# set-soft/ComfyUI-FLOAT_Optimized

Hardware: AMD Instinct MI355X
Metric: 512x512 frames/sec end-to-end audio->video @50 ODE steps (higher is better)
Workload: dtype fp16; 1 GPU; configs[1]: 10 s audio + 512x512 portrait in HBM -> 250 frames in pinned host memory; appearance encoder + wav2vec2 audio encoder + FMT sampling (50 Euler evaluations/window, CFG a=2.0 e=1.0) + decode + D2H, through InferenceAgent.infer_device (the product call); nfe=51, frames_per_clip=250, fmt_dtype=fp16, dec_dtype=fp16, decode_batch=32, hip_graph=True, parallelism=replicas x1 (one clip per GPU), stage_overlap=off

## Files before the change

comfyui-float_optimized_amd/csrc/fmt_api.hip:

```cpp
#include <math.h>
#include <stdlib.h>

#include "fmt_gemm.hpp"
#include "fmt_kernels.hpp"
#include "fmt_rb_kernels.hpp"
#include "fmt_big_kernels.hpp"
#include "fmt_launch.hpp"

namespace {

struct Blk {
  Lin qkv, proj, fc1, fc2;
};

constexpr int kMaxTok = 80;
constexpr int kMaxSteps = 1024;

}

struct float_fmt {
  float_fmt_cfg_t cfg;
  DevicePool pool;
  int D, ntok, Mpad, Kc, Ntot, Kx;
  int Bmax = 1;
  Lin x_embed, t0, t2, c_embed, adaln_all, final_lin;
  std::vector<Blk> blk;
  float* pos = nullptr;
  float* freqs = nullptr;
  u16 *cond16, *sc16, *h16, *hfin16, *qkv16, *att16, *hid16, *xin16, *tsin16, *th16;
  float *ccond, *xres, *xcur, *temb, *vout;
  unsigned long long* sat = nullptr;
  float* slab = nullptr;
  float *wa_c, *we_c, *prev_x, *prev_wa, *prev_we, *x0_c;
  float* wr_c = nullptr;
  int method = 0;
  FmtTune tune;
  int n_cu = 0;
  float* kbuf = nullptr;
  float* modall = nullptr;
  int Mmod = 0;
  size_t mod_zs = 0;
  struct GraphKey {
    int nfe, bc, we_len, method;
    int prio;
    float a, r, e;
    bool operator==(const GraphKey& o) const { return memcmp(this, &o, sizeof(GraphKey)) == 0; }
  };
  struct GraphEntry {
    GraphKey key;
    hipGraphExec_t exec[kFmtMaxClips + 1];
    uint64_t used;
  };
  std::vector<GraphEntry> graphs;
  uint64_t graph_clock = 0;
  hipStream_t cap_stream = nullptr;
  int cap_prio = 0;
  struct {
    const float *wr, *wa, *we, *noise;
    float* r_d;
    int T, we_len, nfe, include_r, next, n_chunks, B;
    int first = 0, total = 0;
    const float *hist_x = nullptr, *hist_wa = nullptr, *hist_we = nullptr;
    float a, r, e;
    std::vector<float> ts;
    bool active = false;
    bool ragged = false;
    FmtClipTab<const float*> rg_wr, rg_wa, rg_we, rg_noise;
    FmtClipTab<float*> rg_rd;
    int rg_win[kFmtMaxClips];
  } job;
};

namespace {

int dev_copy2d(float* dst, size_t dpitch, const float* src, size_t spitch, int width, int rows, hipStream_t s) {
  if (width <= 0 || rows <= 0) return FLOAT_OK;
  hipLaunchKernelGGL(fmt_copy_kernel, dim3((unsigned)(((size_t)rows * width + 255) / 256)), dim3(256), 0, s, dst, dpitch, src, spitch, width, rows);
  FH_CHECK_HIP(hipGetLastError());
  return FLOAT_OK;
}
int dev_copy(float* dst, const float* src, size_t n, hipStream_t s) { return dev_copy2d(dst, n, src, n, (int)n, 1, s); }
int dev_zero(float* dst, size_t n, hipStream_t s) { return dev_copy2d(dst, n, nullptr, n, (int)n, 1, s); }
int copy_or_zero(float* dst, const float* src, size_t n, hipStream_t s) { return src ? dev_copy(dst, src, n, s) : dev_zero(dst, n, s); }

FmtLaunch launch_ctx(const float_fmt* h, hipStream_t s) {
  return FmtLaunch{h->tune, s, h->sat, h->xres, h->slab, h->h16, h->qkv16, h->att16, h->D, h->ntok, h->Ntot, h->Mpad, h->cfg.heads,
                   h->cfg.attn_window};
}


constexpr int kScSteps = 64;

static int stream_priority(hipStream_t s) {
  int prio = 0;
  if (hipStreamGetPriority(s, &prio) != hipSuccess) {
    (void)hipGetLastError();
    prio = 0;
  }
  return prio;
}

template <class T>
int run_mod_all(float_fmt* h, int M, int e0, int n, hipStream_t s) {
  const int D = h->D;
  const FmtTune& tn = h->tune;
  FH_REQUIRE(n >= 1 && n <= kScSteps, "modulation batch of %d evaluations (max %d)", n, kScSteps);
  const int prio = (s == h->cap_stream && s) ? h->cap_prio : stream_priority(s);
  const bool big = !T::is32 && tn.wide && prio == 0 && big_shape_ok(tn, n * M, h->adaln_all.N, h->adaln_all.K, h->n_cu);
  hipLaunchKernelGGL((fmt_silu_c_kernel<T>), dim3((M * D / 8 + 255) / 256, n), dim3(256), 0, s, h->sc16, h->temb + (size_t)e0 * D,
                     h->ccond, M, D, (size_t)h->Mpad * D, big ? M : 0, h->sat);
  h->mod_zs = big ? (size_t)M * h->Ntot : (size_t)h->Mmod * h->Ntot;
  if constexpr (!T::is32) {
    if (big) return launch_big4<T>(h->sc16, h->adaln_all, h->modall, n * M, h->Ntot, h->n_cu, s);
  }
  GemmArgs g = base_args(h->sc16, h->adaln_all, M);
  g.sat = h->sat, g.out_f32 = h->modall, g.ldo = h->Ntot, g.zcount = n;
  const bool dma = (tn.wide_variant == 6 || tn.wide_variant == 7) && (M + 15) / 16 > 4 && dma_shape_ok(g, 320);
  g.zgroup = tn.zgroup > 0 ? tn.zgroup : (dma ? 2 : 4);
  g.a_zstride = (size_t)h->Mpad * D;
  g.o_zstride = (size_t)h->Mmod * h->Ntot;
  if constexpr (!T::is32) {
    if (tn.wide && g.N % 128 == 0 && g.K % 128 == 0) return launch_wide<T>(g, tn.wide_variant, s);
  }
  for (int z = 0; z < n; ++z) {
    GemmArgs gz = g;
    gz.A = g.A + (size_t)z * g.a_zstride * (sizeof(typename T::elem) / sizeof(u16));
    gz.out_f32 = g.out_f32 + (size_t)z * g.o_zstride;
    gz.zcount = 0;
    int rc = run_gemm<T, EPI_F32>(tn, gz, s);
    if (rc) return rc;
  }
  return FLOAT_OK;
}

bool split_ok(int ks, const Lin& L) { return (ks == 1 || ks == 2 || ks == 4) && L.K % (128 * ks) == 0; }

template <class T>
int run_proj(const FmtLaunch& cx, const Blk& B, int M, const float* gate, const RbPlan& rb, PendingRed* pend) {
  const FmtTune& tn = cx.tn;
  const int ks = rb.shape >= 0 ? rb.ksplit : (split_ok(tn.proj_split, B.proj) ? tn.proj_split : 0);
  int rc;
  launch_attn<T>(cx, M, (!ks && (tn.touch & 2)) ? &B.proj : nullptr);
  GemmArgs g = base_args(cx.att16, B.proj, M);
  if (rb.shape >= 0) {
    to_slab(g, cx.slab, cx.Mpad, ks);
    rc = launch_rbs<T, EPI_PARTIAL>(g, rb.shape, cx.s);
  } else if (ks) {
    rc = run_gemm_partial<T>(cx, g, ks);
  } else {
    g.sat = cx.sat, g.out_f32 = cx.xres, g.ldo = cx.D;
    g.gate = gate, g.ldg = cx.Ntot;
    if (tn.touch & 16) g.touch = make_touch(tn, B.fc1, M, 0, gemm_lanes_per_xcd(tn, M, g.N, g.K), 2);
    rc = run_gemm<T, EPI_GATE_RES>(tn, g, cx.s, false, &tn.plan_layer[RB_PROJ]);
  }
  if (!rc && ks) *pend = pending_red(cx.slab, cx.Mpad, cx.D, B.proj.b, gate, ks);
  return rc;
}

template <class T>
int run_fc2(const FmtLaunch& cx, const Blk& B, const u16* hid16, int M, const float* gate, const RbPlan& rb, const Lin& after,
            int after_nt, PendingRed* pend) {
  const FmtTune& tn = cx.tn;
  const int ks = rb.shape >= 0 ? rb.ksplit : (split_ok(tn.fc2_split, B.fc2) ? tn.fc2_split : 0);
  GemmArgs g = base_args(hid16, B.fc2, M);
  int rc;
  if (rb.shape >= 0) {
    to_slab(g, cx.slab, cx.Mpad, ks);
    rc = launch_rbs<T, EPI_PARTIAL>(g, rb.shape, cx.s);
  } else if (ks) {
    g.sat = cx.sat;
    if (tn.touch & 32) g.touch = make_touch(tn, after, M, 0, gemm_lanes_per_xcd(tn, M, g.N * ks, g.K / ks), 2, after_nt);
    rc = run_gemm_partial<T>(cx, g, ks, &tn.plan_layer[RB_FC2]);
  } else {
    g.sat = cx.sat, g.out_f32 = cx.xres, g.ldo = cx.D;
    g.gate = gate, g.ldg = cx.Ntot;
    rc = run_gemm<T, EPI_GATE_RES>(tn, g, cx.s);
  }
  if (!rc && ks) *pend = pending_red(cx.slab, cx.Mpad, cx.D, B.fc2.b, gate, ks);
  return rc;
}

template <class T>
int run_blocks(float_fmt* h, int nclip, int bc, const float* modbuf, bool euler, float dt, float a, float r, float e, hipStream_t s,
               float* vout_to = nullptr) {
  const float_fmt_cfg_t& c = h->cfg;
  const FmtTune& tn = h->tune;
  const FmtLaunch cx = launch_ctx(h, s);
  const int D = h->D, ntok = h->ntok, M = nclip * bc * ntok;
  int rc;
  {
    GemmArgs g = base_args(h->xin16, h->x_embed, nclip * ntok);
    g.sat = h->sat, g.out_f32 = h->xres, g.ldo = D;
    g.pos = h->pos, g.bc = bc, g.ntok = ntok;
    if ((rc = run_gemm<T, EPI_XEMBED>(tn, g, s))) return rc;
  }
  PendingRed pend;
  RbPlan rb_qkv, rb_proj, rb_fc1, rb_fc2;
  if constexpr (!T::is32) {
    rb_qkv = pick_rb(tn, RB_QKV, M), rb_proj = pick_rb(tn, RB_PROJ, M), rb_fc1 = pick_rb(tn, RB_FC1, M), rb_fc2 = pick_rb(tn, RB_FC2, M);
  }
  for (int b = 0; b < c.depth; ++b) {
    const float* mod = modbuf + (size_t)b * 6 * D;
    const Blk& B = h->blk[b];
    const bool last = b + 1 == c.depth;
    if ((rc = launch_lnmod<T>(cx, M, mod, mod + D, &pend, &B.qkv, nullptr, 0, 128, rb_qkv.shape))) return rc;
    {
      GemmArgs g = base_args(h->h16, B.qkv, M);
      g.sat = h->sat, g.out16 = h->qkv16, g.ldo16 = 3 * D;
      if ((tn.touch & 8) && !split_ok(tn.proj_split, B.proj)) g.touch = make_touch(tn, B.proj, M, 0, gemm_lanes_per_xcd(tn, M, g.N, g.K), 2);
      if (rb_qkv.shape >= 0) rc = launch_rbs<T, EPI_T16>(g, rb_qkv.shape, s);
      else rc = run_gemm<T, EPI_T16>(tn, g, s, false, &tn.plan_layer[RB_QKV]);
      if (rc) return rc;
    }
    if ((rc = run_proj<T>(cx, B, M, mod + 2 * D, rb_proj, &pend))) return rc;
    if ((rc = launch_lnmod<T>(cx, M, mod + 3 * D, mod + 4 * D, &pend, &B.fc1, nullptr, 0, 64, rb_fc1.shape))) return rc;
    {
      GemmArgs g = base_args(h->h16, B.fc1, M);
      g.sat = h->sat, g.out16 = h->hid16, g.ldo16 = B.fc2.K / 32;
      if ((tn.touch & 4) && rb_fc2.shape < 0)
        g.touch = make_touch(tn, B.fc2, M, split_ok(tn.fc2_split, B.fc2) ? tn.fc2_split : 0, gemm_lanes_per_xcd(tn, M, g.N, g.K), 2);
      if (rb_fc1.shape >= 0) rc = launch_rbs<T, EPI_GELU_P16>(g, rb_fc1.shape, s);
      else rc = run_gemm<T, EPI_GELU_P16>(tn, g, s, false, &tn.plan_layer[RB_FC1]);
      if (rc) return rc;
    }
    if ((rc = run_fc2<T>(cx, B, h->hid16, M, mod + 5 * D, rb_fc2, last ? h->final_lin : h->blk[b + 1].qkv, last ? 1 : 0, &pend))) return rc;
  }
  {
    const float* mod = modbuf + (size_t)c.depth * 6 * D;
    const bool tokblk = (!tn.no_tokblk || nclip > 1) && (bc == 1 || bc == 3 || bc == 4) && h->final_lin.K % 256 == 0;
    FH_REQUIRE(tokblk || nclip == 1, "batched sampling needs the token-blocked head GEMM");
    const int nblk = (ntok + 15) / 16, seqs = nclip * bc;
    if ((rc = launch_lnmod<T>(cx, M, mod, mod + D, &pend, nullptr, tokblk ? h->hfin16 : nullptr, tokblk ? seqs * 16 : 0))) return rc;
    GemmArgs g = base_args(tokblk ? h->hfin16 : h->h16, h->final_lin, tokblk ? nblk * seqs * 16 : M);
    g.sat = h->sat, g.tokblk = tokblk ? 1 : 0;
    g.nclip = nclip, g.bc = bc, g.ntok = ntok, g.n_prev = c.n_prev;
    g.a_cfg = a, g.r_cfg = r, g.e_cfg = e, g.dt = dt;
    if (euler) g.xcur = h->xcur, g.xin16 = h->xin16, g.ldx = h->Kx / 32;
    else g.vout = vout_to ? vout_to : h->vout;
    if (tokblk) rc = launch_gemm<T, EPI_CFG>(g, bc, 1, 8, s);
    else rc = run_gemm<T, EPI_CFG>(tn, g, s, true);
    if (rc) return rc;
  }
  FH_CHECK_HIP(hipGetLastError());
  return FLOAT_OK;
}

void linspace01(int n, std::vector<float>* ts) {
  ts->resize(n);
  if (n == 1) {
    (*ts)[0] = 0.f;
    return;
  }
  const float step = 1.0f / (float)(n - 1);
  const int half = n / 2;
  for (int i = 0; i < n; ++i) (*ts)[i] = (i < half) ? (0.f + step * (float)i) : (1.0f - step * (float)(n - 1 - i));
}

struct TimeSpec {
  float t;
  int nfe, stages;
  float c[4];
};
template <class T>
int prepare_time(float_fmt* h, const TimeSpec& ts, int n, hipStream_t s) {
  int rc;
  hipLaunchKernelGGL((fmt_tsin_kernel<T>), dim3(n), dim3(256), 0, s, h->tsin16, h->freqs, n, ts.t, ts.nfe, ts.stages, ts.c[0],
                     ts.c[1], ts.c[2], ts.c[3]);
  GemmArgs g = base_args(h->tsin16, h->t0, n);
  g.sat = h->sat, g.out16 = h->th16, g.ldo16 = h->t2.K / 32;
  if ((rc = launch_gemm<T, EPI_SILU_P16>(g, 4, 1, T::is32 ? 4 : pick_nw(g.K, 0), s))) return rc;
  GemmArgs g2 = base_args(h->th16, h->t2, n);
  g2.sat = h->sat, g2.out_f32 = h->temb, g2.ldo = h->D;
  if ((rc = launch_gemm<T, EPI_F32>(g2, 4, 1, T::is32 ? 4 : pick_nw(g2.K, 0), s))) return rc;
  return FLOAT_OK;
}

struct CfgMode {
  int bc;
  unsigned wr_mask, wa_mask, we_mask;
  int nclip = 1;
};

CfgMode cfg_mode(float a, float r, float e, int include_r) {
  if (a == 1.0f && r == 1.0f && e == 1.0f) return {1, 1u, 1u, 1u, 1};
  if (!include_r) return {3, 0b111u, 0b110u, 0b010u, 1};
  return {4, 0b1110u, 0b1100u, 0b0100u, 1};
}

template <class T>
int stage_window(float_fmt* h, const CfgMode& m, const float* x0, const float* wa, const float* wr, const float* we,
                 int we_len, const float* prev_x, const float* prev_wa, const float* prev_we, hipStream_t s) {
  const float_fmt_cfg_t& c = h->cfg;
  const int M = m.nclip * m.bc * h->ntok;
  hipLaunchKernelGGL((fmt_build_cond_kernel<T>), dim3(M), dim3(256), 0, s, h->cond16, h->Kc, m.bc, h->ntok, c.n_prev,
                     c.dim_w, c.dim_a, c.dim_e, wr, wa, prev_wa, we, we_len, prev_we, m.wr_mask, m.wa_mask, m.we_mask, h->sat);
  GemmArgs g = base_args(h->cond16, h->c_embed, M);
  g.sat = h->sat, g.out_f32 = h->ccond, g.ldo = h->D;
  int rc;
  if ((rc = run_gemm<T, EPI_F32>(h->tune, g, s))) return rc;
  const int n = m.nclip * h->ntok * c.dim_w;
  hipLaunchKernelGGL((fmt_init_x_kernel<T>), dim3((n + 255) / 256), dim3(256), 0, s, h->xcur, h->xin16, h->Kx / 32, x0, prev_x,
                     c.n_prev, c.n_cur, c.dim_w, m.nclip, h->sat);
  FH_CHECK_HIP(hipGetLastError());
  return FLOAT_OK;
}

int check_cfg_rows(const float_fmt* h, const CfgMode& m) {
  FH_REQUIRE(!h->tune.no_tokblk || m.bc * h->ntok <= 240,
             "%d-way CFG of %d tokens is %d rows; the all-rows CFG epilogue GEMM holds at most 240 (15 row tiles)", m.bc, h->ntok,
             m.bc * h->ntok);
  return FLOAT_OK;
}

int check_common(float_fmt* h, const void* we, int we_len, const void* prev_we) {
  FH_REQUIRE(h != nullptr, "null FMT handle");
  FH_REQUIRE(we_len == 1 || we_len == h->cfg.n_cur,
             "Dynamic emotion latent `we` time dimension (%d) does not match audio latent `wa` time dimension (%d).",
             we_len, h->cfg.n_cur);
  FH_REQUIRE(!(we_len > 1 && prev_we == nullptr),
             "`we` is dynamic (T>1), but prev_we was not provided with prev_x/prev_wa.");
  (void)we;
  return FLOAT_OK;
}

struct Tableau {
  int s;
  float c[4], a[4][3], b[4];
};
const Tableau& tableau(int method) {
  static const Tableau T[5] = {
      {1, {0.f}, {{0.f}}, {1.f}},
      {2, {0.f, 0.5f}, {{0.f}, {0.5f}}, {0.f, 1.f}},
      {4, {0.f, 1.f / 3, 2.f / 3, 1.f}, {{0.f}, {1.f / 3}, {-1.f / 3, 1.f}, {1.f, -1.f, 1.f}}, {0.125f, 0.375f, 0.375f, 0.125f}},
      {2, {0.f, 1.f}, {{0.f}, {1.f}}, {0.5f, 0.5f}},
      {3, {0.f, 1.f / 3, 2.f / 3}, {{0.f}, {1.f / 3}, {0.f, 2.f / 3}}, {0.25f, 0.f, 0.75f}},
  };
  return T[method];
}

TimeSpec time_spec(int method, int nfe) {
  const Tableau& tb = tableau(method);
  TimeSpec ts{};
  ts.nfe = nfe;
  ts.stages = tb.s;
  for (int j = 0; j < 4; ++j) ts.c[j] = tb.c[j];
  return ts;
}
int n_evals(int method, int nfe) { return (nfe - 1) * tableau(method).s; }

template <class T>
int run_window_steps(float_fmt* h, const CfgMode& m, int nfe, const std::vector<float>& ts, float a, float r, float e,
                     hipStream_t s) {
  const Tableau& tb = tableau(h->method);
  const float_fmt_cfg_t& c = h->cfg;
  const size_t kstride = (size_t)h->Bmax * kMaxTok * c.dim_w;
  const int n = m.nclip * c.n_cur * c.dim_w, rows = m.nclip * m.bc * h->ntok;
  const int nev = n_evals(h->method, nfe), batch = h->tune.hoist ? kScSteps : 1;
  const bool euler = h->method == FLOAT_ODE_EULER;
  int rc;
  for (int ev = 0; ev < nev; ++ev) {
    const int i = ev / tb.s, j = ev - i * tb.s, z = ev % batch;
    const float dt = ts[i + 1] - ts[i];
    if (z == 0 && (rc = run_mod_all<T>(h, rows, ev, std::min(batch, nev - ev), s))) return rc;
    const float* mod = h->modall + (size_t)z * h->mod_zs;
    if (euler) {
      if ((rc = run_blocks<T>(h, m.nclip, m.bc, mod, true, dt, a, r, e, s))) return rc;
      continue;
    }
    if (j > 0) {
      hipLaunchKernelGGL((fmt_rk_combine_kernel<T>), dim3((n + 255) / 256), dim3(256), 0, s, h->xcur, h->kbuf, kstride, j,
                         dt * tb.a[j][0], dt * tb.a[j][1], dt * tb.a[j][2], 0.f, 0, h->xin16, h->Kx / 32, c.n_prev, c.n_cur,
                         c.dim_w, m.nclip, h->sat);
    }
    if ((rc = run_blocks<T>(h, m.nclip, m.bc, mod, false, 0.f, a, r, e, s, h->kbuf + (size_t)j * kstride))) return rc;
    if (j == tb.s - 1) {
      hipLaunchKernelGGL((fmt_rk_combine_kernel<T>), dim3((n + 255) / 256), dim3(256), 0, s, h->xcur, h->kbuf, kstride, tb.s,
                         dt * tb.b[0], dt * tb.b[1], dt * tb.b[2], dt * tb.b[3], 1, h->xin16, h->Kx / 32, c.n_prev, c.n_cur,
                         c.dim_w, m.nclip, h->sat);
    }
  }
  FH_CHECK_HIP(hipGetLastError());
  return FLOAT_OK;
}

constexpr size_t kMaxGraphs = 8;
void destroy_graphs(float_fmt::GraphEntry& g) {
  for (hipGraphExec_t& e : g.exec)
    if (e) {
      (void)hipGraphExecDestroy(e);
      e = nullptr;
    }
}
template <class T>
int run_window_steps_graph(float_fmt* h, const CfgMode& m, int we_len, int nfe, const std::vector<float>& ts, float a,
                           float r, float e, hipStream_t s) {
  float_fmt::GraphKey key;
  memset(&key, 0, sizeof(key));
  key.nfe = nfe;
  key.method = h->method;
  key.bc = m.bc;
  key.we_len = we_len;
  key.a = a;
  key.r = r;
  key.e = e;
  key.prio = stream_priority(s);
  FH_REQUIRE(m.nclip >= 1 && m.nclip <= kFmtMaxClips, "chain of %d clips (max %d)", m.nclip, kFmtMaxClips);
  float_fmt::GraphEntry* hit = nullptr;
  for (auto& g : h->graphs)
    if (g.key == key) hit = &g;
  if (!hit || !hit->exec[m.nclip]) {
    if (!h->cap_stream) FH_CHECK_HIP(hipStreamCreateWithFlags(&h->cap_stream, hipStreamNonBlocking));
    hipGraph_t graph = nullptr;
    h->cap_prio = key.prio;
    FH_CHECK_HIP(hipStreamBeginCapture(h->cap_stream, hipStreamCaptureModeThreadLocal));
    int rc = run_window_steps<T>(h, m, nfe, ts, a, r, e, h->cap_stream);
    hipError_t ce = hipStreamEndCapture(h->cap_stream, &graph);
    if (rc) {
      if (graph) (void)hipGraphDestroy(graph);
      return rc;
    }
    FH_CHECK_HIP(ce);
    hipGraphExec_t exec = nullptr;
    FH_CHECK_HIP(hipGraphInstantiate(&exec, graph, nullptr, nullptr, 0));
    (void)hipGraphDestroy(graph);
    if (!hit) {
      if (h->graphs.size() >= kMaxGraphs) {
        size_t lru = 0;
        for (size_t i = 1; i < h->graphs.size(); ++i)
          if (h->graphs[i].used < h->graphs[lru].used) lru = i;
        hipError_t se = hipDeviceSynchronize();
        if (se != hipSuccess) {
          (void)hipGraphExecDestroy(exec);
          FH_CHECK_HIP(se);
        }
        destroy_graphs(h->graphs[lru]);
        h->graphs.erase(h->graphs.begin() + lru);
      }
      float_fmt::GraphEntry fresh;
      memset(&fresh, 0, sizeof(fresh));
      fresh.key = key;
      h->graphs.push_back(fresh);
      hit = &h->graphs.back();
    }
    hit->exec[m.nclip] = exec;
  }
  hit->used = ++h->graph_clock;
  FH_CHECK_HIP(hipGraphLaunch(hit->exec[m.nclip], s));
  return FLOAT_OK;
}

template <class T>
int window_impl(float_fmt* h, const float* x0, const float* wa, const float* wr, const float* we, int we_len,
                const float* prev_x, const float* prev_wa, const float* prev_we, int nfe, const std::vector<float>& ts,
                float a, float r, float e, int include_r, hipStream_t s, int nclip = 1) {
  CfgMode m = cfg_mode(a, r, e, include_r);
  m.nclip = nclip;
  int rc = check_cfg_rows(h, m);
  if (rc) return rc;
  if ((rc = stage_window<T>(h, m, x0, wa, wr, we, we_len, prev_x, prev_wa, prev_we, s))) return rc;
  if (nfe <= 1) return FLOAT_OK;
  hipStreamCaptureStatus cs = hipStreamCaptureStatusNone;
  if (hipStreamIsCapturing(s, &cs) != hipSuccess) {
    (void)hipGetLastError();
    cs = hipStreamCaptureStatusNone;
  }
  if (h->cfg.use_graph && !g_fh_profiling && cs == hipStreamCaptureStatusNone)
    return run_window_steps_graph<T>(h, m, we_len, nfe, ts, a, r, e, s);
  return run_window_steps<T>(h, m, nfe, ts, a, r, e, s);
}

template <class T>
int eval_impl(float_fmt* h, float t, const float* x, const float* wa, const float* wr, const float* we, int we_len,
              const float* prev_x, const float* prev_wa, const float* prev_we, float a, float r, float e, int include_r,
              float* out, hipStream_t s) {
  TimeSpec tsp{};
  tsp.t = t;
  int rc = prepare_time<T>(h, tsp, 1, s);
  if (rc) return rc;
  const CfgMode m = cfg_mode(a, r, e, include_r);
  if ((rc = check_cfg_rows(h, m))) return rc;
  if ((rc = stage_window<T>(h, m, x, wa, wr, we, we_len, prev_x, prev_wa, prev_we, s))) return rc;
  if ((rc = run_mod_all<T>(h, m.bc * h->ntok, 0, 1, s))) return rc;
  if ((rc = run_blocks<T>(h, 1, m.bc, h->modall, false, 0.f, a, r, e, s))) return rc;
  return dev_copy(out, h->vout, (size_t)h->ntok * h->cfg.dim_w, s);
}

template <class T>
int sample_window(float_fmt* h, int k, hipStream_t s) {
  const float_fmt_cfg_t& c = h->cfg;
  auto& J = h->job;
  const int L = c.n_cur, P = c.n_prev, Tn = J.T, B = J.B;
  const bool dynamic = J.we_len > 1;
  int rc;
  auto blocks = [](int n) { return dim3((n + 255) / 256); };
  if (k == J.first) {
    if ((rc = prepare_time<T>(h, time_spec(h->method, J.nfe), std::max(1, n_evals(h->method, J.nfe)), s))) return rc;
    if ((rc = copy_or_zero(h->prev_x, J.hist_x, (size_t)B * P * c.dim_w, s))) return rc;
    if ((rc = copy_or_zero(h->prev_wa, J.hist_wa, (size_t)B * P * c.dim_a, s))) return rc;
    if ((rc = copy_or_zero(h->prev_we, J.hist_we, (size_t)B * P * c.dim_e, s))) return rc;
  } else if (P > 0) {
    hipLaunchKernelGGL(fmt_tail_kernel, blocks(B * P * c.dim_w), dim3(256), 0, s, h->prev_x, h->xcur, P, L, c.dim_w, B);
    hipLaunchKernelGGL(fmt_tail_kernel, blocks(B * P * c.dim_a), dim3(256), 0, s, h->prev_wa, h->wa_c, P, L, c.dim_a, B);
    if (dynamic) hipLaunchKernelGGL(fmt_tail_kernel, blocks(B * P * c.dim_e), dim3(256), 0, s, h->prev_we, h->we_c, P, L, c.dim_e, B);
  }
  hipLaunchKernelGGL(fmt_slice_pad_kernel, blocks(B * L * c.dim_a), dim3(256), 0, s, h->wa_c, J.wa, k * L, Tn, L, c.dim_a, B);
  if (dynamic) hipLaunchKernelGGL(fmt_slice_pad_kernel, blocks(B * L * c.dim_e), dim3(256), 0, s, h->we_c, J.we, k * L, Tn, L, c.dim_e, B);
  if ((rc = dev_copy(h->x0_c, J.noise + (size_t)k * B * L * c.dim_w, (size_t)B * L * c.dim_w, s))) return rc;
  rc = window_impl<T>(h, h->x0_c, h->wa_c, J.wr, dynamic ? h->we_c : J.we, dynamic ? L : 1, h->prev_x, h->prev_wa,
                      dynamic ? h->prev_we : nullptr, J.nfe, J.ts, J.a, J.r, J.e, J.include_r, s, B);
  if (rc) return rc;
  const int rows = (k == J.total - 1) ? (Tn - k * L) : L;
  return dev_copy2d(J.r_d + (size_t)k * L * c.dim_w, (size_t)Tn * c.dim_w, h->xcur, (size_t)L * c.dim_w, rows * c.dim_w, B, s);
}

template <class T>
int sample_window_ragged(float_fmt* h, int k, hipStream_t s) {
  const float_fmt_cfg_t& c = h->cfg;
  auto& J = h->job;
  const int L = c.n_cur, P = c.n_prev;
  const bool dynamic = J.we_len > 1;
  int nact = 0;
  while (nact < J.B && J.rg_win[nact] > k) ++nact;
  int rc;
  auto blocks = [](int n) { return dim3((n + 255) / 256); };
  auto grid = [nact](int n) { return dim3((n + 255) / 256, nact); };
  if (k == 0) {
    if ((rc = prepare_time<T>(h, time_spec(h->method, J.nfe), std::max(1, n_evals(h->method, J.nfe)), s))) return rc;
    if ((rc = dev_zero(h->prev_x, (size_t)nact * P * c.dim_w, s))) return rc;
    if ((rc = dev_zero(h->prev_wa, (size_t)nact * P * c.dim_a, s))) return rc;
    if ((rc = dev_zero(h->prev_we, (size_t)nact * P * c.dim_e, s))) return rc;
    hipLaunchKernelGGL(fmt_gather_pad_kernel, grid(c.dim_w), dim3(256), 0, s, h->wr_c, J.rg_wr, 0, 1, c.dim_w);
    if (!dynamic) hipLaunchKernelGGL(fmt_gather_pad_kernel, grid(c.dim_e), dim3(256), 0, s, h->we_c, J.rg_we, 0, 1, c.dim_e);
  } else if (P > 0) {
    hipLaunchKernelGGL(fmt_tail_kernel, blocks(nact * P * c.dim_w), dim3(256), 0, s, h->prev_x, h->xcur, P, L, c.dim_w, nact);
    hipLaunchKernelGGL(fmt_tail_kernel, blocks(nact * P * c.dim_a), dim3(256), 0, s, h->prev_wa, h->wa_c, P, L, c.dim_a, nact);
    if (dynamic) hipLaunchKernelGGL(fmt_tail_kernel, blocks(nact * P * c.dim_e), dim3(256), 0, s, h->prev_we, h->we_c, P, L, c.dim_e, nact);
  }
  hipLaunchKernelGGL(fmt_gather_pad_kernel, grid(L * c.dim_a), dim3(256), 0, s, h->wa_c, J.rg_wa, k * L, L, c.dim_a);
  if (dynamic) hipLaunchKernelGGL(fmt_gather_pad_kernel, grid(L * c.dim_e), dim3(256), 0, s, h->we_c, J.rg_we, k * L, L, c.dim_e);
  hipLaunchKernelGGL(fmt_gather_pad_kernel, grid(L * c.dim_w), dim3(256), 0, s, h->x0_c, J.rg_noise, k * L, L, c.dim_w);
  FH_CHECK_HIP(hipGetLastError());
  rc = window_impl<T>(h, h->x0_c, h->wa_c, h->wr_c, h->we_c, dynamic ? L : 1, h->prev_x, h->prev_wa,
                      dynamic ? h->prev_we : nullptr, J.nfe, J.ts, J.a, J.r, J.e, J.include_r, s, nact);
  if (rc) return rc;
  hipLaunchKernelGGL(fmt_scatter_trim_kernel, grid(L * c.dim_w), dim3(256), 0, s, J.rg_rd, h->xcur, k * L, L, c.dim_w);
  FH_CHECK_HIP(hipGetLastError());
  return FLOAT_OK;
}

template <class T>
int create_impl(float_fmt* h, const TensorTable& tt) {
  const float_fmt_cfg_t& c = h->cfg;
  const int D = c.dim_h;
  int rc;
  prime_kernels<T>();
  auto pack = [&](const std::vector<std::string>& names, int N_each, int K, Lin* out) {
    return pack_linear_pool<T>(h->tune, &h->pool, tt, names, N_each, K, out);
  };
  if ((rc = pack({"x_embedder.proj"}, D, c.dim_w, &h->x_embed))) return rc;
  if ((rc = pack({"t_embedder.mlp.0"}, D, 256, &h->t0))) return rc;
  if ((rc = pack({"t_embedder.mlp.2"}, D, D, &h->t2))) return rc;
  if ((rc = pack({"c_embedder"}, D, c.dim_w + c.dim_a + c.dim_e, &h->c_embed))) return rc;
  h->blk.resize(c.depth);
  std::vector<std::string> ada;
  for (int b = 0; b < c.depth; ++b) {
    const std::string p = "blocks." + std::to_string(b) + ".";
    if ((rc = pack({p + "attn.qkv"}, 3 * D, D, &h->blk[b].qkv))) return rc;
    if ((rc = pack({p + "attn.proj"}, D, D, &h->blk[b].proj))) return rc;
    if ((rc = pack({p + "mlp.fc1"}, c.mlp_hidden, D, &h->blk[b].fc1))) return rc;
    if ((rc = pack({p + "mlp.fc2"}, D, c.mlp_hidden, &h->blk[b].fc2))) return rc;
    ada.push_back(p + "adaLN_modulation.1");
  }
  if ((rc = pack(ada, 6 * D, D, &h->adaln_all))) return rc;
  Lin tail;
  if ((rc = pack(std::vector<std::string>{"decoder.adaLN_modulation.1"}, 2 * D, D, &tail))) return rc;
  if ((rc = concat_linear_rows<T>(&h->pool, h->adaln_all, tail, &h->adaln_all))) return rc;
  if ((rc = pack({"decoder.linear"}, c.dim_w, D, &h->final_lin))) return rc;
  return FLOAT_OK;
}

}


int fmt_pack_linear(const FmtTune& tn, DevicePool* pool, int dtype, const TensorTable& tt, const std::vector<std::string>& names,
                    int N_each, int K, FmtLin* out) {
  FH_REQUIRE(dtype == FLOAT_DT_BF16 || dtype == FLOAT_DT_FP16 || dtype == FLOAT_DT_FP32, "the GEMM service: unknown dtype %d", dtype);
  return fmt_by_dtype(dtype, [&](auto t) { return pack_linear_pool<decltype(t)>(tn, pool, tt, names, N_each, K, out); });
}

int fmt_pack_linear_raw(const FmtTune& tn, DevicePool* pool, int dtype, const float* w, const float* b, int N, int K, FmtLin* out) {
  std::vector<float> zeros;
  if (!b) {
    zeros.assign(N, 0.f);
    b = zeros.data();
  }
  float_tensor_t t[2];
  memset(t, 0, sizeof(t));
  t[0].name = "raw.weight";
  t[0].data = w;
  t[0].ndim = 2;
  t[0].shape[0] = N;
  t[0].shape[1] = K;
  t[1].name = "raw.bias";
  t[1].data = b;
  t[1].ndim = 1;
  t[1].shape[0] = N;
  TensorTable tt(t, 2);
  return fmt_pack_linear(tn, pool, dtype, tt, {"raw"}, N, K, out);
}

GemmArgs fmt_gemm_args(const u16* A, const FmtLin& L, int M) { return base_args(A, L, M); }

void fmt_gemm_prime(int dtype) {
  fmt_by_dtype(dtype, [](auto t) { prime_kernels<decltype(t)>(); });
}

template <class T>
static int gemm_run_t(const FmtTune& tn, int epi, const GemmArgs& g, hipStream_t s) {
  switch (epi) {
    case EPI_F32: return run_gemm<T, EPI_F32>(tn, g, s);
    case EPI_T16: return run_gemm<T, EPI_T16>(tn, g, s);
    case EPI_SILU_P16: return run_gemm<T, EPI_SILU_P16>(tn, g, s);
    case EPI_GELU_P16: return run_gemm<T, EPI_GELU_P16>(tn, g, s);
    case EPI_GELUERF_P16: return run_gemm<T, EPI_GELUERF_P16>(tn, g, s);
    default: fh_set_error("fmt_gemm_run: epilogue %d is not exported", epi); return FLOAT_E_INVALID;
  }
}

int fmt_gemm_run(const FmtTune& tn, int dtype, int epi, GemmArgs g, hipStream_t s) {
  return fmt_by_dtype(dtype, [&](auto t) { return gemm_run_t<decltype(t)>(tn, epi, g, s); });
}

template <class T>
static int debug_impl(float_fmt* h, int what, const float* in, float* out, hipStream_t s) {
  const int D = h->D, ntok = h->ntok;
  if (what == 0) {
    return dev_copy(out, h->pos, (size_t)ntok * D, s);
  }
  if (what == 3 || what == 4) {
    FH_REQUIRE(in != nullptr, "float_fmt_debug: request %d needs an input", what);
    constexpr int Mt = 48, Kt = 1024;
    const int Nt = what == 3 ? 64 : 16;
    std::vector<float> host((size_t)(Mt + Nt) * Kt);
    FH_CHECK_HIP(hipStreamSynchronize(s));
    FH_CHECK_HIP(hipMemcpy(host.data(), in, host.size() * sizeof(float), hipMemcpyDeviceToHost));
    struct Scratch : DevicePool {
      ~Scratch() { release(); }
    } pool;
    Lin a, w;
    int rc;
    if ((rc = fmt_pack_linear_raw(h->tune, &pool, h->cfg.dtype, host.data(), nullptr, Mt, Kt, &a))) return rc;
    if ((rc = fmt_pack_linear_raw(h->tune, &pool, h->cfg.dtype, host.data() + (size_t)Mt * Kt, nullptr, Nt, Kt, &w))) return rc;
    GemmArgs g = base_args(a.W, w, Mt);
    g.out_f32 = out, g.ldo = Nt;
    if (what == 3) {
      if ((rc = launch_gemm<T, EPI_F32>(g, 3, 4, T::is32 ? 4 : 8, s))) return rc;
    } else {
      float* ones = nullptr;
      if ((rc = pool.alloc(&ones, (size_t)Mt * Nt, false))) return rc;
      const std::vector<float> one((size_t)Mt * Nt, 1.f);
      FH_CHECK_HIP(hipMemcpy(ones, one.data(), one.size() * sizeof(float), hipMemcpyHostToDevice));
      FH_CHECK_HIP(hipMemsetAsync(out, 0, (size_t)Mt * Nt * sizeof(float), s));
      g.gate = ones, g.ldg = Nt;
      if ((rc = launch_gemm<T, EPI_GATE_RES>(g, 3, 1, T::is32 ? 4 : 8, s))) return rc;
    }
    FH_CHECK_HIP(hipStreamSynchronize(s));
    return FLOAT_OK;
  }
  if (what == 5) {
    FH_REQUIRE(in != nullptr, "float_fmt_debug: request %d needs an input", what);
    hipLaunchKernelGGL(fmt_xlane_probe_kernel, dim3(kXlaneProbeVecs), dim3(64), 0, s, in, out);
    FH_CHECK_HIP(hipGetLastError());
    return FLOAT_OK;
  }
  FH_REQUIRE(what == 1 && in != nullptr, "float_fmt_debug: unknown request %d (or null input)", what);
  const int n = ntok * 3 * D;
  hipLaunchKernelGGL((fmt_dbg_to16_kernel<T>), dim3((n + 255) / 256), dim3(256), 0, s, h->qkv16, in, n);
  launch_attn<T>(launch_ctx(h, s), ntok, nullptr);
  hipLaunchKernelGGL((fmt_dbg_unpack_kernel<T>), dim3((ntok * D + 255) / 256), dim3(256), 0, s, out, h->att16, ntok, D);
  FH_CHECK_HIP(hipGetLastError());
  return FLOAT_OK;
}

static int drain_job(float_fmt_t* h, void* stream) {
  int32_t left = 1;
  while (left > 0)
    if (int rc = float_fmt_sample_next(h, stream, nullptr, &left)) return rc;
  return FLOAT_OK;
}

extern "C" {

int float_fmt_create(const float_fmt_cfg_t* cfg, const float_tensor_t* tensors, int32_t n_tensors, float_fmt_t** out) {
  FH_REQUIRE(cfg && tensors && out, "null argument to float_fmt_create");
  FH_REQUIRE(cfg->dim_h % 256 == 0 && cfg->dim_h / 256 <= 8 && ((cfg->dim_h / 256) & (cfg->dim_h / 256 - 1)) == 0,
             "dim_h=%d unsupported", cfg->dim_h);
  FH_REQUIRE(cfg->dim_h / cfg->heads == 128, "head_dim must be 128 (dim_h=%d heads=%d)", cfg->dim_h, cfg->heads);
  FH_REQUIRE(cfg->dim_w % 128 == 0 && cfg->mlp_hidden % 128 == 0, "dim_w / mlp_hidden must be multiples of 128");
  FH_REQUIRE(cfg->n_prev + cfg->n_cur <= kMaxTok, "at most %d tokens per window (got %d)", kMaxTok, cfg->n_prev + cfg->n_cur);
  FH_REQUIRE(cfg->n_prev >= 0 && cfg->n_prev <= cfg->n_cur, "n_prev must be in [0, n_cur]");
  FH_REQUIRE(cfg->dtype == FLOAT_DT_BF16 || cfg->dtype == FLOAT_DT_FP16 || cfg->dtype == FLOAT_DT_FP32, "unknown dtype %d", cfg->dtype);
  FH_REQUIRE(cfg->max_batch >= 0 && cfg->max_batch <= 16, "max_batch must be in [0, 16] (got %d)", cfg->max_batch);
  float_fmt* h = new float_fmt();
  h->tune = FmtTune::from_env();
  h->cfg = *cfg;
  h->D = cfg->dim_h;
  h->ntok = cfg->n_prev + cfg->n_cur;
  h->Bmax = cfg->max_batch > 0 ? cfg->max_batch : 1;
  h->Mpad = 16 * ((h->Bmax * 4 * h->ntok + 15) / 16 + 12);
  h->Kc = round_up(cfg->dim_w + cfg->dim_a + cfg->dim_e, 128);
  h->Kx = round_up(cfg->dim_w, 128);
  {
    int dev = 0, ncu = 0;
    if (hipGetDevice(&dev) == hipSuccess && hipDeviceGetAttribute(&ncu, hipDeviceAttributeMultiprocessorCount, dev) == hipSuccess) h->n_cu = ncu;
    else (void)hipGetLastError();
  }
  h->Ntot = cfg->depth * 6 * h->D + 2 * h->D;
  TensorTable tt(tensors, n_tensors);
  int rc = fmt_by_dtype(cfg->dtype, [&](auto t) { return create_impl<decltype(t)>(h, tt); });
  const int D = h->D, Mp = h->Mpad;
  const size_t esz = cfg->dtype == FLOAT_DT_FP32 ? 2 : 1;
  auto A = [&](auto** p, size_t n) {
    if (!rc) rc = h->pool.alloc(p, std::is_same<std::remove_reference_t<decltype(**p)>, u16>::value ? n * esz : n, true);
  };
  A(&h->pos, (size_t)kMaxTok * D);
  A(&h->freqs, 128);
  A(&h->cond16, (size_t)Mp * h->Kc);
  A(&h->sc16, (size_t)kScSteps * Mp * D + (size_t)12 * 16 * D);
  A(&h->h16, (size_t)Mp * D);
  A(&h->hfin16, (size_t)h->Bmax * 64 * ((kMaxTok + 15) / 16) * D);
  A(&h->qkv16, (size_t)Mp * 3 * D);
  A(&h->att16, (size_t)Mp * D);
  A(&h->hid16, (size_t)Mp * cfg->mlp_hidden);
  A(&h->xin16, (size_t)(h->Bmax * kMaxTok + 6 * 16) * h->Kx);
  A(&h->tsin16, (size_t)kMaxSteps * 256);
  A(&h->th16, (size_t)kMaxSteps * D);
  A(&h->ccond, (size_t)Mp * D);
  h->Mmod = 16 * ((h->Bmax * 4 * h->ntok + 15) / 16);
  if (!rc) rc = h->pool.alloc(&h->modall, (size_t)kScSteps * h->Mmod * h->Ntot, false);
  A(&h->kbuf, (size_t)4 * h->Bmax * kMaxTok * cfg->dim_w);
  A(&h->xres, (size_t)Mp * D);
  A(&h->slab, (size_t)8 * Mp * D);
  A(&h->sat, 1);
  A(&h->xcur, (size_t)h->Bmax * cfg->n_cur * cfg->dim_w);
  A(&h->temb, (size_t)kMaxSteps * D);
  A(&h->vout, (size_t)h->Bmax * kMaxTok * cfg->dim_w);
  A(&h->wa_c, (size_t)h->Bmax * cfg->n_cur * cfg->dim_a);
  A(&h->we_c, (size_t)h->Bmax * cfg->n_cur * cfg->dim_e);
  A(&h->x0_c, (size_t)h->Bmax * cfg->n_cur * cfg->dim_w);
  A(&h->wr_c, (size_t)h->Bmax * cfg->dim_w);
  A(&h->prev_x, (size_t)h->Bmax * cfg->n_cur * cfg->dim_w);
  A(&h->prev_wa, (size_t)h->Bmax * cfg->n_cur * cfg->dim_a);
  A(&h->prev_we, (size_t)h->Bmax * cfg->n_cur * cfg->dim_e);
  if (!rc) {
    std::vector<float> pos((size_t)h->ntok * D);
    const float_tensor_t* pe = tt.find("pos_embed");
    if (pe && TensorTable::numel(pe) == (int64_t)h->ntok * D) {
      memcpy(pos.data(), pe->data, pos.size() * sizeof(float));
    } else {
      for (int p = 0; p < h->ntok; ++p)
        for (int j = 0; j < D; ++j) {
          const float ang = (float)((double)p / pow(10000.0, 2.0 * (double)(j / 2) / (double)D));
          pos[(size_t)p * D + j] = (j & 1) ? cosf(ang) : sinf(ang);
        }
    }
    std::vector<float> fr(128);
    for (int k = 0; k < 128; ++k) fr[k] = expf(-logf(10000.0f) * (float)k / 128.0f);
    if (hipMemcpy(h->pos, pos.data(), pos.size() * sizeof(float), hipMemcpyHostToDevice) != hipSuccess ||
        hipMemcpy(h->freqs, fr.data(), fr.size() * sizeof(float), hipMemcpyHostToDevice) != hipSuccess) {
      fh_set_error("hipMemcpy of FMT tables failed");
      rc = FLOAT_E_HIP;
    }
  }
  if (rc) {
    float_fmt_destroy(h);
    return rc;
  }
  *out = h;
  return FLOAT_OK;
}

void float_fmt_destroy(float_fmt_t* h) {
  if (!h) return;
  for (auto& g : h->graphs) destroy_graphs(g);
  if (h->cap_stream) (void)hipStreamDestroy(h->cap_stream);
  h->pool.release();
  delete h;
}

int float_fmt_eval(float_fmt_t* h, float t, const float* x, const float* wa, const float* wr, const float* we,
                   int32_t we_len, const float* prev_x, const float* prev_wa, const float* prev_we, float a_cfg,
                   float r_cfg, float e_cfg, int32_t include_r_cfg, float* out, void* stream) {
  int rc = check_common(h, we, we_len, prev_we);
  if (rc) return rc;
  FH_REQUIRE(x && wa && wr && we && prev_x && prev_wa && out, "null tensor argument to float_fmt_eval");
  hipStream_t s = (hipStream_t)stream;
  return fmt_by_dtype(h->cfg.dtype, [&](auto tag) {
    return eval_impl<decltype(tag)>(h, t, x, wa, wr, we, we_len, prev_x, prev_wa, prev_we, a_cfg, r_cfg, e_cfg, include_r_cfg, out, s);
  });
}

int float_fmt_sample_chunk(float_fmt_t* h, const float* x0, const float* wa, const float* wr, const float* we,
                           int32_t we_len, const float* prev_x, const float* prev_wa, const float* prev_we, int32_t nfe,
                           float a_cfg, float r_cfg, float e_cfg, int32_t include_r_cfg, float* out, void* stream) {
  int rc = check_common(h, we, we_len, prev_we);
  if (rc) return rc;
  FH_REQUIRE(x0 && wa && wr && we && prev_x && prev_wa && out, "null tensor argument to float_fmt_sample_chunk");
  FH_REQUIRE(nfe >= 1 && n_evals(h->method, nfe) < kMaxSteps, "nfe=%d: too many evaluations (max %d)", nfe, kMaxSteps);
  hipStream_t s = (hipStream_t)stream;
  std::vector<float> ts;
  linspace01(nfe, &ts);
  const float_fmt_cfg_t& c = h->cfg;
  if ((rc = dev_copy(h->x0_c, x0, (size_t)c.n_cur * c.dim_w, s))) return rc;
  if ((rc = dev_copy(h->wa_c, wa, (size_t)c.n_cur * c.dim_a, s))) return rc;
  if ((rc = dev_copy(h->prev_x, prev_x, (size_t)c.n_prev * c.dim_w, s))) return rc;
  if ((rc = dev_copy(h->prev_wa, prev_wa, (size_t)c.n_prev * c.dim_a, s))) return rc;
  if (we_len > 1) {
    if ((rc = dev_copy(h->we_c, we, (size_t)c.n_cur * c.dim_e, s))) return rc;
    if ((rc = dev_copy(h->prev_we, prev_we, (size_t)c.n_prev * c.dim_e, s))) return rc;
  }
  const float* we_p = we_len > 1 ? h->we_c : we;
  const float* pwe_p = we_len > 1 ? h->prev_we : nullptr;
  const TimeSpec tsp = time_spec(h->method, nfe);
  const int nev = std::max(1, n_evals(h->method, nfe));
  rc = fmt_by_dtype(c.dtype, [&](auto t) {
    typedef decltype(t) T;
    if (int prc = prepare_time<T>(h, tsp, nev, s)) return prc;
    return window_impl<T>(h, h->x0_c, h->wa_c, wr, we_p, we_len, h->prev_x, h->prev_wa, pwe_p, nfe, ts, a_cfg, r_cfg, e_cfg,
                          include_r_cfg, s);
  });
  if (rc) return rc;
  return dev_copy(out, h->xcur, (size_t)c.n_cur * c.dim_w, s);
}

int float_fmt_debug(float_fmt_t* h, int32_t what, const float* in, float* out, void* stream) {
  FH_REQUIRE(h != nullptr && out != nullptr, "null argument to float_fmt_debug");
  return fmt_by_dtype(h->cfg.dtype, [&](auto t) { return debug_impl<decltype(t)>(h, what, in, out, (hipStream_t)stream); });
}

int float_fmt_saturation(float_fmt_t* h, uint64_t* total, int32_t reset, void* stream) {
  FH_REQUIRE(h && total, "null argument to float_fmt_saturation");
  FH_CHECK_HIP(hipStreamSynchronize((hipStream_t)stream));
  unsigned long long v = 0;
  FH_CHECK_HIP(hipMemcpy(&v, h->sat, sizeof(v), hipMemcpyDeviceToHost));
  *total = v;
  if (reset) {
    FH_CHECK_HIP(hipMemsetAsync(h->sat, 0, sizeof(v), (hipStream_t)stream));
    FH_CHECK_HIP(hipStreamSynchronize((hipStream_t)stream));
  }
  return FLOAT_OK;
}

int float_fmt_set_method(float_fmt_t* h, int32_t method) {
  FH_REQUIRE(h != nullptr, "null FMT handle");
  FH_REQUIRE(method >= FLOAT_ODE_EULER && method <= FLOAT_ODE_HEUN3, "unknown ODE method %d", method);
  h->method = method;
  return FLOAT_OK;
}

int float_fmt_sample_begin(float_fmt_t* h, const float* wr, const float* wa, int32_t T, const float* we, int32_t we_len,
                           const float* noise, int32_t nfe, float a_cfg, float r_cfg, float e_cfg, int32_t include_r_cfg,
                           float* r_d) {
  FH_REQUIRE(h != nullptr, "null FMT handle");
  FH_REQUIRE(wr && wa && we && noise && r_d, "null tensor argument to float_fmt_sample");
  FH_REQUIRE(T >= 1, "T must be >= 1 (got %d)", T);
  FH_REQUIRE(we_len == 1 || we_len == T,
             "Dynamic emotion latent `we` time dimension (%d) does not match audio latent `wa` time dimension (%d).",
             we_len, T);
  FH_REQUIRE(nfe >= 1 && n_evals(h->method, nfe) < kMaxSteps, "nfe=%d: too many evaluations (max %d)", nfe, kMaxSteps);
  auto& J = h->job;
  J.wr = wr;
  J.wa = wa;
  J.we = we;
  J.noise = noise;
  J.r_d = r_d;
  J.T = T;
  J.we_len = we_len;
  J.nfe = nfe;
  J.include_r = include_r_cfg;
  J.a = a_cfg;
  J.r = r_cfg;
  J.e = e_cfg;
  J.B = 1;
  J.ragged = false;
  J.next = 0;
  J.n_chunks = (T + h->cfg.n_cur - 1) / h->cfg.n_cur;
  J.first = 0;
  J.total = J.n_chunks;
  J.hist_x = J.hist_wa = J.hist_we = nullptr;
  linspace01(nfe, &J.ts);
  J.active = true;
  return FLOAT_OK;
}

int float_fmt_sample_begin_range(float_fmt_t* h, const float* wr, const float* wa, int32_t T, const float* we, int32_t we_len,
                                 const float* noise, int32_t nfe, float a_cfg, float r_cfg, float e_cfg, int32_t include_r_cfg,
                                 float* r_d, int32_t first_window, int32_t end_window, const float* hist_x, const float* hist_wa,
                                 const float* hist_we) {
  int rc = float_fmt_sample_begin(h, wr, wa, T, we, we_len, noise, nfe, a_cfg, r_cfg, e_cfg, include_r_cfg, r_d);
  if (rc) return rc;
  auto& J = h->job;
  J.active = false;
  FH_REQUIRE(first_window >= 0 && first_window < end_window && end_window <= J.total,
             "window range [%d, %d) outside the clip's %d windows", first_window, end_window, J.total);
  FH_REQUIRE(we_len == 1 || hist_we != nullptr || hist_x == nullptr,
             "a dynamic-emotion job that starts from a history needs hist_we too");
  J.first = J.next = first_window;
  J.n_chunks = end_window;
  J.hist_x = hist_x;
  J.hist_wa = hist_wa;
  J.hist_we = we_len > 1 ? hist_we : nullptr;
  J.active = true;
  return FLOAT_OK;
}

int float_fmt_sample_next(float_fmt_t* h, void* stream, int32_t* window_done, int32_t* windows_left) {
  FH_REQUIRE(h != nullptr && h->job.active, "float_fmt_sample_next without float_fmt_sample_begin");
  auto& J = h->job;
  hipStream_t s = (hipStream_t)stream;
  const int k = J.next;
  int rc = fmt_by_dtype(h->cfg.dtype, [&](auto t) {
    return J.ragged ? sample_window_ragged<decltype(t)>(h, k, s) : sample_window<decltype(t)>(h, k, s);
  });
  if (rc) {
    J.active = false;
    return rc;
  }
  J.next = k + 1;
  if (window_done) *window_done = k;
  if (windows_left) *windows_left = J.n_chunks - J.next;
  if (J.next >= J.n_chunks) J.active = false;
  return FLOAT_OK;
}

int float_fmt_sample_batch(float_fmt_t* h, int32_t n_clips, const float* wr, const float* wa, int32_t T, const float* we,
                           int32_t we_len, const float* noise, int32_t nfe, float a_cfg, float r_cfg, float e_cfg,
                           int32_t include_r_cfg, float* r_d, void* stream) {
  FH_REQUIRE(h != nullptr, "null FMT handle");
  FH_REQUIRE(n_clips >= 1 && n_clips <= h->Bmax, "batch of %d clips, the handle was created with max_batch = %d", n_clips, h->Bmax);
  int rc = float_fmt_sample_begin(h, wr, wa, T, we, we_len, noise, nfe, a_cfg, r_cfg, e_cfg, include_r_cfg, r_d);
  if (rc) return rc;
  h->job.B = n_clips;
  return drain_job(h, stream);
}

int float_fmt_sample_begin_ragged(float_fmt_t* h, int32_t n_clips, const int32_t* T, const float* const* wr,
                                  const float* const* wa, const float* const* we, int32_t we_dynamic,
                                  const float* const* noise, int32_t nfe, float a_cfg, float r_cfg, float e_cfg,
                                  int32_t include_r_cfg, float* const* r_d) {
  FH_REQUIRE(h != nullptr, "null FMT handle");
  FH_REQUIRE(T && wr && wa && we && noise && r_d, "null array argument to float_fmt_sample_begin_ragged");
  FH_REQUIRE(n_clips >= 1 && n_clips <= h->Bmax, "batch of %d clips, the handle was created with max_batch = %d", n_clips, h->Bmax);
  for (int i = 0; i < n_clips; ++i) {
    FH_REQUIRE(wr[i] && wa[i] && we[i] && noise[i] && r_d[i], "null tensor argument to float_fmt_sample_begin_ragged (clip %d)", i);
    FH_REQUIRE(T[i] >= 1, "T must be >= 1 (got %d for clip %d)", T[i], i);
  }
  FH_REQUIRE(nfe >= 1 && n_evals(h->method, nfe) < kMaxSteps, "nfe=%d: too many evaluations (max %d)", nfe, kMaxSteps);
  auto& J = h->job;
  J.active = false;
  const int L = h->cfg.n_cur;
  int order[kFmtMaxClips];
  for (int i = 0; i < n_clips; ++i) order[i] = i;
  std::stable_sort(order, order + n_clips, [&](int x, int y) { return (T[x] + L - 1) / L > (T[y] + L - 1) / L; });
  memset(&J.rg_wr, 0, sizeof(J.rg_wr));
  memset(&J.rg_wa, 0, sizeof(J.rg_wa));
  memset(&J.rg_we, 0, sizeof(J.rg_we));
  memset(&J.rg_noise, 0, sizeof(J.rg_noise));
  memset(&J.rg_rd, 0, sizeof(J.rg_rd));
  for (int q = 0; q < n_clips; ++q) {
    const int i = order[q], Ti = T[i], win = (Ti + L - 1) / L;
    J.rg_win[q] = win;
    J.rg_wr.p[q] = wr[i], J.rg_wr.T[q] = 1;
    J.rg_wa.p[q] = wa[i], J.rg_wa.T[q] = Ti;
    J.rg_we.p[q] = we[i], J.rg_we.T[q] = we_dynamic ? Ti : 1;
// ... 41 lines not shown
```

comfyui-float_optimized_amd/csrc/fmt_decode.hpp:

```cpp
#pragma once

#if defined(__HIPCC__)
#define FMT_HD __host__ __device__ __forceinline__
#else
#define FMT_HD inline
#endif

struct FmtDiv {
  unsigned mul, sh;
};
inline FmtDiv fmt_make_div(unsigned d) {
  unsigned l = 0;
  while ((1u << l) < d) ++l;
  FmtDiv v;
  v.sh = 28u + l;
  v.mul = (unsigned)((1ull << v.sh) / d + 1ull);
  return v;
}
FMT_HD unsigned fmt_div(unsigned n, unsigned mul, unsigned sh) { return (unsigned)(((unsigned long long)n * mul) >> sh); }
FMT_HD unsigned fmt_div(unsigned n, const FmtDiv& d) { return fmt_div(n, d.mul, d.sh); }
constexpr unsigned kFmtDivMax = 1u << 28;

struct GemmDecode {
  unsigned mblk_mul;
  unsigned nbx, nbx_mul;
  unsigned nbn, nbn_mul;
  unsigned bits;
};
enum { kDecAffine = 1u << 20, kDecKsXcd = 1u << 21 };

inline GemmDecode fmt_make_decode(int nbn, int mblk, int ksplit, bool partial) {
  GemmDecode d;
  const unsigned nbx = (unsigned)(partial ? nbn * ksplit : nbn);
  const FmtDiv dm = fmt_make_div((unsigned)mblk), dx = fmt_make_div(nbx), dn = fmt_make_div((unsigned)nbn);
  d.mblk_mul = dm.mul, d.nbx = nbx, d.nbx_mul = dx.mul, d.nbn = (unsigned)nbn, d.nbn_mul = dn.mul;
  d.bits = dm.sh | (dx.sh << 6) | (dn.sh << 12);
  if ((nbx & 7u) == 0u) {
    d.bits |= kDecAffine;
    if (partial && (8 % ksplit) == 0) {
      unsigned p = 0;
      while ((8u >> p) != (unsigned)ksplit) ++p;
      d.bits |= kDecKsXcd | (p << 18);
    }
  }
  return d;
}

struct GemmBlock {
  int bx, by, ks;
};
FMT_HD GemmBlock fmt_block_decode(const GemmDecode& d, unsigned mblk, unsigned id, bool partial) {
  unsigned bx, by, ks = 0u;
  if (d.bits & kDecAffine) {
    const unsigned slot = id >> 3, q = fmt_div(slot, d.mblk_mul, d.bits & 63u);
    by = slot - q * mblk;
    bx = q * 8u + (id & 7u);
  } else {
    by = fmt_div(id, d.nbx_mul, (d.bits >> 6) & 63u);
    bx = id - by * d.nbx;
  }
  if (partial) {
    if (d.bits & kDecKsXcd) {
      const unsigned p = (d.bits >> 18) & 3u, x = bx & 7u;
      ks = x >> p;
      bx = ((bx >> 3) << p) + (x & ((1u << p) - 1u));
    } else {
      ks = fmt_div(bx, d.nbn_mul, (d.bits >> 12) & 63u);
      bx -= ks * d.nbn;
    }
  }
  return GemmBlock{(int)bx, (int)by, (int)ks};
}
```

comfyui-float_optimized_amd/csrc/fmt_kernels.hpp:

```cpp
#pragma once
#include "common.hpp"
#include "fmt_pack.hpp"

template <class T, int MTW, int NT>
constexpr int fmt_gemm_pf() {
  return T::is32 ? 1 : ((MTW + NT <= 7) ? 4 : ((MTW + NT <= 8) ? 3 : 2));
}
template <class T, int MTW, int NT, int NW, int EPI>
constexpr bool fmt_gemm_has_flat() {
  if (T::is32) return false;
  if (EPI == EPI_XEMBED) return MTW == 4 && NT == 1 && NW == 4;
  return NW == 8 && MTW == 3 && (NT == 4 || EPI == EPI_GATE_RES || EPI == EPI_CFG);
}

template <class T, int MTW, int NT, int NW, int EPI, bool FLAT = false>
__device__ __forceinline__ void fmt_gemm_body(const GemmArgs& g) {
  const unsigned bid = blockIdx.x, nblk = gridDim.x;
  constexpr int BN = NT * 16;
  constexpr int ROWS = MTW * 16;
  constexpr bool WT = NW >= 8;
  constexpr int NTHR = NW * 64;
  constexpr int PF = fmt_gemm_pf<T, MTW, NT>();
  typedef typename T::elem E;
  typedef typename T::pack8 P8;
  extern __shared__ __attribute__((aligned(16))) float red[];
  const int lane = threadIdx.x & 63;
  const int w = threadIdx.x >> 6;
  const int r16 = lane & 15, q = lane >> 4;
  const GemmBlock blk = fmt_block_decode(g.dec, (unsigned)g.mblk, bid, EPI == EPI_PARTIAL);
  const int bx = blk.bx, by = blk.by, ks = blk.ks;
  const int nb0 = bx * NT;
  const int mt0 = by * MTW;
  const int n0 = nb0 * 16, m0 = mt0 * 16;

  f32x4 acc[MTW][NT];
#pragma unroll
  for (int i = 0; i < MTW; ++i)
#pragma unroll
    for (int j = 0; j < NT; ++j) acc[i][j] = f32x4{0.f, 0.f, 0.f, 0.f};

  const int KB = g.K >> 5;
  const int KBs = (EPI == EPI_PARTIAL) ? g.kbs : KB;
  const int KBw = FLAT ? PF : (int)((unsigned)KBs / NW);
  const E* Ap = reinterpret_cast<const E*>(g.A) + ((size_t)mt0 * KB + ks * KBs + w * KBw) * 512 + lane * 8;
  const E* Wp = reinterpret_cast<const E*>(g.W) + ((size_t)nb0 * KB + ks * KBs + w * KBw) * 512 + lane * 8;
  const size_t tstride = (size_t)KB * 512;

  P8 a[PF][MTW], b[PF][NT];
#pragma unroll
  for (int p = 0; p < PF; ++p) {
    if (FLAT || p < KBw) {
#pragma unroll
      for (int j = 0; j < NT; ++j) b[p][j] = T::load8_nt(Wp + j * tstride + (size_t)p * 512);
#pragma unroll
      for (int i = 0; i < MTW; ++i) a[p][i] = T::load8(Ap + i * tstride + (size_t)p * 512);
    }
  }
  constexpr bool kEarlyRes = (EPI == EPI_GATE_RES) && (MTW * 16 * (NT * 2) <= NW * 64);
  float4 res_pf[2], gate_pf[2];
  if constexpr (kEarlyRes) {
    const int r = threadIdx.x / (NT * 2), cg = threadIdx.x % (NT * 2);
    int row = m0 + r;
    const int nb = n0 + cg * 8;
    if constexpr (FLAT) row = min(m0 + min(r, ROWS - 1), g.M - 1);
    if (FLAT || (r < ROWS && row < g.M)) {
      const float* o = g.out_f32 + (size_t)row * g.ldo + nb;
      const float* gt = g.gate + (size_t)row * g.ldg + nb;
      res_pf[0] = fh_load_f4(o);
      res_pf[1] = fh_load_f4(o + 4);
      gate_pf[0] = fh_load_f4_stream(gt);
      gate_pf[1] = fh_load_f4_stream(gt + 4);
    }
  }
  constexpr bool kTouch = (EPI == EPI_GELU_P16 || EPI == EPI_T16 || EPI == EPI_GATE_RES || EPI == EPI_PARTIAL);
  unsigned touched[2] = {0u, 0u};
  if constexpr (kTouch && FLAT) {
    __builtin_amdgcn_sched_barrier(0);
    fmt_touch_always(g.touch, Wp, bid & 7, (bid >> 3) * NTHR + threadIdx.x, (nblk >> 3) * NTHR, touched);
  } else if constexpr (kTouch) {
    if (g.touch.W) fmt_touch(g.touch, bid & 7, (bid >> 3) * NTHR + threadIdx.x, (nblk >> 3) * NTHR, touched);
  }
  if constexpr (FLAT) {
#pragma unroll
    for (int p = 0; p < PF; ++p) {
      __builtin_amdgcn_sched_barrier(0);
#pragma unroll
      for (int i = 0; i < MTW; ++i)
#pragma unroll
        for (int j = 0; j < NT; ++j) acc[i][j] = T::mfma(a[p][i], b[p][j], acc[i][j]);
    }
    __builtin_amdgcn_sched_barrier(0);
  } else
  for (int kb0 = 0; kb0 < KBw; kb0 += PF) {
#pragma unroll
    for (int p = 0; p < PF; ++p) {
      const int kb = kb0 + p;
      if (kb < KBw) {
#pragma unroll
        for (int i = 0; i < MTW; ++i)
#pragma unroll
          for (int j = 0; j < NT; ++j) acc[i][j] = T::mfma(a[p][i], b[p][j], acc[i][j]);
        if (kb + PF < KBw) {
#pragma unroll
          for (int j = 0; j < NT; ++j)
            b[p][j] = T::load8_nt(Wp + j * tstride + (size_t)(kb + PF) * 512);
#pragma unroll
          for (int i = 0; i < MTW; ++i) a[p][i] = T::load8(Ap + i * tstride + (size_t)(kb + PF) * 512);
        }
      }
    }
  }

  if constexpr (kTouch && !FLAT) {
    if (g.touch.W) fmt_touch_retire(touched);
  }
  float* my = red + w * (ROWS * BN);
#pragma unroll
  for (int i = 0; i < MTW; ++i)
#pragma unroll
    for (int j = 0; j < NT; ++j)
#pragma unroll
      for (int r = 0; r < 4; ++r) my[(i * 16 + q * 4 + r) * BN + j * 16 + r16] = acc[i][j][r];
  __syncthreads();

  constexpr int S = ROWS * BN;
  constexpr int CG = BN / 8;
  unsigned rm = 0u;
  auto slab_sum = [&](int o) {
    float a = red[o];
#pragma unroll
    for (int ww = 1; ww < NW; ++ww) a += red[ww * S + o];
    return a;
  };
  if constexpr (EPI == EPI_CFG) {
    const int nclip = g.nclip > 1 ? g.nclip : 1;
    const int tb = g.tokblk ? by / nclip : 0, q = g.tokblk ? by - tb * nclip : 0;
    const int ni = g.tokblk ? 16 : g.ntok, i0 = tb * 16, rstride = g.tokblk ? 16 : g.ntok;
    float* const vout_q = g.vout ? g.vout + (size_t)q * g.ntok * g.N : nullptr;
    float* const xcur_q = g.xcur ? g.xcur + (size_t)q * (g.ntok - g.n_prev) * g.N : nullptr;
    for (int idx = threadIdx.x; idx < ni * BN; idx += NTHR) {
      const int il = idx / BN, i = i0 + il, c = idx % BN, n = n0 + c;
      if (i >= g.ntok) break;
      const float bias = g.bias[n];
      float v[4];
#pragma unroll
      for (int b2 = 0; b2 < 4; ++b2) {
        if (b2 < g.bc) {
          const int o = (b2 * rstride + il) * BN + c;
          v[b2] = slab_sum(o) + bias;
        } else {
          v[b2] = 0.f;
        }
      }
      float out;
      if (g.bc == 1) {
        out = v[0];
      } else if (g.bc == 3) {
        out = v[0] + g.a_cfg * (v[2] - v[0]) + g.e_cfg * (v[1] - v[2]);
      } else {
        out = v[0] + g.r_cfg * (v[1] - v[0]) + g.a_cfg * (v[3] - v[1]) + g.e_cfg * (v[2] - v[3]);
      }
      if (vout_q) vout_q[(size_t)i * g.N + n] = out;
      if (xcur_q && i >= g.n_prev) {
        const size_t xo = (size_t)(i - g.n_prev) * g.N + n;
        const float xn = xcur_q[xo] + g.dt * out;
        xcur_q[xo] = xn;
        reinterpret_cast<E*>(g.xin16)[fmt_pack_off(q * g.ntok + i, n, g.ldx)] = fh_cvt<T>(xn, rm);
      }
    }
  } else {
    for (int idx = threadIdx.x; idx < ROWS * CG; idx += NTHR) {
      const int r = idx / CG, cg = idx % CG;
      const int row = m0 + r, nb = n0 + cg * 8;
      if (row >= g.M) continue;
      float v[8];
      {
        const float* p0 = red + r * BN + cg * 8;
#pragma unroll
        for (int e = 0; e < 8; e += 4) {
          float4 a4 = *reinterpret_cast<const float4*>(p0 + e);
#pragma unroll
          for (int ww = 1; ww < NW; ++ww) {
            const float4 t4 = *reinterpret_cast<const float4*>(p0 + ww * S + e);
            a4.x += t4.x;
            a4.y += t4.y;
            a4.z += t4.z;
            a4.w += t4.w;
          }
          float4 bb = float4{0.f, 0.f, 0.f, 0.f};
          if constexpr (EPI != EPI_PARTIAL) bb = *reinterpret_cast<const float4*>(g.bias + nb + e);
          v[e + 0] = a4.x + bb.x;
          v[e + 1] = a4.y + bb.y;
          v[e + 2] = a4.z + bb.z;
          v[e + 3] = a4.w + bb.w;
        }
      }
      if constexpr (EPI == EPI_F32 || EPI == EPI_PARTIAL) {
        float* o = g.out_f32 + (size_t)ks * g.slab_stride + (size_t)row * g.ldo + nb;
        fh_store_f4_wt<4, WT>(o, float4{v[0], v[1], v[2], v[3]});
        fh_store_f4_wt<4, WT>(o + 4, float4{v[4], v[5], v[6], v[7]});
      } else if constexpr (EPI == EPI_T16 || EPI == EPI_SILU_P16 || EPI == EPI_GELU_P16 || EPI == EPI_GELUERF_P16) {
        P8 u;
#pragma unroll
        for (int i = 0; i < 8; ++i) {
          float x = v[i];
          if constexpr (EPI == EPI_SILU_P16) x = fh_silu(x);
          if constexpr (EPI == EPI_GELU_P16) x = fh_gelu_tanh(x);
          if constexpr (EPI == EPI_GELUERF_P16) x = fh_gelu_erf(x);
          T::set(u, i, x);
        }
        fh_track_pack<T>(rm, u);
        E* const o16 = reinterpret_cast<E*>(g.out16);
        if constexpr (EPI == EPI_T16) T::template store8_wt<8, WT>(o16 + (size_t)row * g.ldo16 + nb, u);
        else T::template store8_wt<8, WT>(o16 + fmt_pack_off(row, nb, g.ldo16), u);
      } else if constexpr (EPI == EPI_GATE_RES) {
        float* o = g.out_f32 + (size_t)row * g.ldo + nb;
        const float* gt = g.gate + (size_t)row * g.ldg + nb;
#pragma unroll
        for (int e = 0; e < 8; e += 4) {
          float4 x, gg;
          if constexpr (kEarlyRes) {
            x = res_pf[e / 4];
            gg = gate_pf[e / 4];
          } else {
            x = fh_load_f4(o + e);
            gg = fh_load_f4_stream(gt + e);
          }
          x.x += gg.x * v[e + 0];
          x.y += gg.y * v[e + 1];
          x.z += gg.z * v[e + 2];
          x.w += gg.w * v[e + 3];
          fh_store_f4_wt<16, WT>(o + e, x);
        }
      } else if constexpr (EPI == EPI_XEMBED) {
        const int q = row / g.ntok, tok = row - q * g.ntok;
        const float* ps = g.pos + (size_t)tok * g.N + nb;
#pragma unroll
        for (int i = 0; i < 8; ++i) v[i] += ps[i];
        for (int b2 = 0; b2 < g.bc; ++b2) {
          float* o = g.out_f32 + (size_t)((q * g.bc + b2) * g.ntok + tok) * g.ldo + nb;
          fh_store_f4_wt<32, WT>(o, float4{v[0], v[1], v[2], v[3]});
          fh_store_f4_wt<32, WT>(o + 4, float4{v[4], v[5], v[6], v[7]});
        }
      }
    }
  }
  if constexpr (EPI == EPI_CFG || EPI == EPI_T16 || EPI == EPI_SILU_P16 || EPI == EPI_GELU_P16 || EPI == EPI_GELUERF_P16) fh_range_flush<T>(g.sat, rm);
  if constexpr (kTouch && FLAT) fmt_touch_retire_last(touched);
}

template <class T, int MTW, int NT, int NW, int EPI>
__global__ __launch_bounds__(NW * 64) void fmt_gemm_kernel(const u16* A, const u16* W, int K, int kbs, int ksplit, int mblk,
                                                           unsigned mblk_mul, unsigned nbx, unsigned nbx_mul, unsigned nbn,
                                                           unsigned nbn_mul, unsigned bits, GemmTail t) {
  GemmArgs g;
  static_cast<GemmHead&>(g) = GemmHead{A, W, K, kbs, ksplit, mblk, GemmDecode{mblk_mul, nbx, nbx_mul, nbn, nbn_mul, bits}};
  static_cast<GemmTail&>(g) = t;
  if constexpr (fmt_gemm_has_flat<T, MTW, NT, NW, EPI>()) {
    if ((EPI == EPI_PARTIAL ? kbs : (K >> 5)) == NW * fmt_gemm_pf<T, MTW, NT>()) {
      fmt_gemm_body<T, MTW, NT, NW, EPI, true>(g);
      return;
    }
  }
  fmt_gemm_body<T, MTW, NT, NW, EPI>(g);
}
template <class K>
void fmt_gemm_launch(int prof, K kern, dim3 grid, dim3 block, size_t smem, hipStream_t s, const GemmArgs& g) {
  const GemmTail& t = g;
  fh_launch_prof(prof, kern, grid, block, smem, s, g.A, g.W, g.K, g.kbs, g.ksplit, g.mblk, g.dec.mblk_mul, g.dec.nbx, g.dec.nbx_mul,
                 g.dec.nbn, g.dec.nbn_mul, g.dec.bits, t);
}

template <class T, int MTW, int KCH , int NWV = 4>
__global__ __launch_bounds__(NWV * 64) void fmt_gemm_wide_kernel(GemmArgs g) {
  constexpr int EPI = EPI_F32;
  constexpr int NF = MTW * KCH;
  constexpr int NFW = (NF + NWV - 1) / NWV;
  constexpr int WR = NWV / 4, MTR = MTW / WR;
  static_assert(MTW % WR == 0, "row tiles must split evenly over the wave rows");
  extern __shared__ __attribute__((aligned(16))) unsigned char sA[];
  const int lane = threadIdx.x & 63, w = threadIdx.x >> 6, wc = w & 3, wr = w >> 2;
  const int r16 = lane & 15, q = lane >> 4;
  const int nbn = g.N >> 7;
  const int nbx = (EPI == EPI_PARTIAL) ? nbn * g.ksplit : nbn;
  int bx, by, bz = 0, ks = 0;
  {
    const int id = blockIdx.x;
    const int nz = g.zcount > 1 ? g.zcount : 1;
    if (nz > 1 && (nbx & 7) == 0 && g.zgroup > 1) {
      const int slot = id >> 3, G = g.zgroup, ncx = nbx >> 3, rows = g.mblk * nz;
      const int full = ncx / G, per_grp = G * rows;
      int grp = slot / per_grp, rem = slot - grp * per_grp, gw = G;
      if (grp >= full) {
        grp = full;
        rem = slot - full * per_grp;
        gw = ncx - full * G;
      }
      const int zy = rem / gw;
      bz = zy / g.mblk;
      by = zy - bz * g.mblk;
// ... 245 lines not shown
      _Pragma("unroll") for (int j = 0; j < 5; ++j) acc[i][j] = T::mfma(BC[j], AC[i], acc[i][j]); \
    __builtin_amdgcn_sched_barrier(0);                                                         \
  } while (0)

  const bool g1 = wr == 1;
#ifdef DMA_CLK
  const unsigned long long c0 = clock64(), w0 = wall_clock64();
#endif
#pragma unroll
  for (int s = 0; s < NS; ++s) issue(s);
  if constexpr (STG) DMA_WAIT(NS - 2);
  else DMA_WAIT(NS - 1);
  __builtin_amdgcn_s_barrier();
  DMA_READ(0, a0, b0);
  asm volatile("s_waitcnt lgkmcnt(0)" ::: "memory");
  __builtin_amdgcn_sched_barrier(0);
  if constexpr (STG) {
    if (g1) __builtin_amdgcn_s_barrier();
    for (int s = 0; s < KB; s += 2) {
      DMA_STEP_STG(s, a0, b0, a1, b1);
      DMA_STEP_STG(s + 1, a1, b1, a0, b0);
    }
    if (!g1) __builtin_amdgcn_s_barrier();
  } else {
    for (int s = 0; s < KB; s += 2) {
      DMA_STEP(s, a0, b0, a1, b1);
      DMA_STEP(s + 1, a1, b1, a0, b0);
    }
  }
#ifdef DMA_CLK
  if ((blockIdx.x == 3000 || blockIdx.x == 6001) && threadIdx.x == 0) {
    const unsigned long long c1 = clock64(), w1 = wall_clock64();
    printf("tile loop: %llu core clocks, %llu wall ticks\n", c1 - c0, w1 - w0);
  }
#endif
#undef DMA_STEP_STG
#undef DMA_WAIT_UPTO
#undef DMA_STEP
#undef DMA_READ
#undef DMA_WAIT
  float* const outz = g.out_f32 + (size_t)bz * g.o_zstride;
  constexpr int OW = CT * 16, OSTR = OW + 4, C4 = OW / 4, NTHR = NW * 64;
  static_assert(96 * OSTR * 4 <= NS * STAGE, "output staging does not fit the ring");
  float* const so = reinterpret_cast<float*>(ring);
  float4 bb[5];
#pragma unroll
  for (int j = 0; j < 5; ++j) bb[j] = *reinterpret_cast<const float4*>(g.bias + (bx * CT + wc * 5 + j) * 16 + q * 4);
#pragma unroll
  for (int p = 0; p < 2; ++p) {
    if (wr == p) {
#pragma unroll
      for (int i = 0; i < 6; ++i)
#pragma unroll
        for (int j = 0; j < 5; ++j)
          *reinterpret_cast<float4*>(so + (i * 16 + r16) * OSTR + (wc * 5 + j) * 16 + q * 4) =
              float4{acc[i][j][0] + bb[j].x, acc[i][j][1] + bb[j].y, acc[i][j][2] + bb[j].z, acc[i][j][3] + bb[j].w};
    }
    __syncthreads();
    {
#pragma unroll
      for (int k = 0; k < (96 * C4) / NTHR; ++k) {
        const int idx = k * NTHR + threadIdx.x, rl = idx / C4, c4 = idx - rl * C4;
        const int row = by * (RT * 16) + p * 96 + rl;
        if (row < g.M)
          *reinterpret_cast<float4*>(outz + (size_t)row * g.ldo + bx * OW + c4 * 4) = *reinterpret_cast<const float4*>(so + rl * OSTR + c4 * 4);
      }
    }
    if (p == 0) __syncthreads();
  }
}

struct LnRed {
  const float* slab;
  size_t slab_stride;
  const float* bias;
  const float* gate;
};

constexpr int kLnTouch = 6;

template <class T, int NV, int KS, bool TOUCH, bool WT>
__device__ __forceinline__ void fmt_lnmod_body(float* __restrict__ x, int M, const float* __restrict__ shift,
                                               const float* __restrict__ scale, int ldm, u16* __restrict__ out, const LnRed& red,
                                               const TouchSpec& pf, int ntok, int perm, unsigned long long* sat, const int wpb) {
  constexpr int D = NV * 256;
  const unsigned bid = blockIdx.x, nblk = gridDim.x;
  const int lane = threadIdx.x & 63;
  int row = bid * wpb + (threadIdx.x >> 6);
  unsigned touched[kLnTouch] = {};
  const bool touch = TOUCH && wpb == 1;
  auto touch_lines = [&]() { fmt_touch(pf, bid & 7, (bid >> 3) * 64 + lane, (nblk >> 3) * 64, touched); };
  if (wpb == 1) {
    const int x = bid & 7, j = bid >> 3;
    row = (((j >> 3) * 8 + x) << 3) + (j & 7);
  }
  if (row >= M) {
    if (touch) {
      touch_lines();
      fmt_touch_retire(touched);
    }
    return;
  }
  float* xr = x + (size_t)row * D;
#ifdef FMT_DIAG_HOTMOD
  const size_t mrow = 0;
#else
  const size_t mrow = (size_t)row;
#endif
  const float* sh = shift + mrow * ldm;
  const float* sc = scale + mrow * ldm;
  float4 v[NV], a[NV], b[NV];
  float s = 0.f;
#pragma unroll
  for (int i = 0; i < NV; ++i) {
    const int c = i * 256 + lane * 4;
    v[i] = fh_load_f4(xr + c);
    a[i] = fh_load_f4_stream(sh + c);
    b[i] = fh_load_f4_stream(sc + c);
  }
  if (KS == 0 && touch) touch_lines();
  if constexpr (KS > 0) {
    float4 p[KS][NV], gt[NV], bi[NV];
#pragma unroll
    for (int i = 0; i < NV; ++i) {
      const int c = i * 256 + lane * 4;
#pragma unroll
      for (int k = 0; k < KS; ++k) {
        const float* ps = red.slab + k * red.slab_stride + (size_t)row * D + c;
        p[k][i] = fh_load_f4_stream(ps);
      }
      gt[i] = fh_load_f4_stream(red.gate + mrow * ldm + c);
    }
#pragma unroll
    for (int i = 0; i < NV; ++i) bi[i] = *reinterpret_cast<const float4*>(red.bias + i * 256 + lane * 4);
    if (touch) touch_lines();
#pragma unroll
    for (int i = 0; i < NV; ++i) {
      float4 t = p[0][i];
#pragma unroll
      for (int k = 1; k < KS; ++k) {
        t.x += p[k][i].x;
        t.y += p[k][i].y;
        t.z += p[k][i].z;
        t.w += p[k][i].w;
      }
      v[i].x += gt[i].x * (t.x + bi[i].x);
      v[i].y += gt[i].y * (t.y + bi[i].y);
      v[i].z += gt[i].z * (t.z + bi[i].z);
      v[i].w += gt[i].w * (t.w + bi[i].w);
      fh_store_f4_wt<1, WT>(xr + i * 256 + lane * 4, v[i]);
    }
  }
#pragma unroll
  for (int i = 0; i < NV; ++i) s += (v[i].x + v[i].y) + (v[i].z + v[i].w);
  const float mu = wave_sum(s) * (1.f / D);
  float s2 = 0.f;
#pragma unroll
  for (int i = 0; i < NV; ++i) {
    const float d0 = v[i].x - mu, d1 = v[i].y - mu, d2 = v[i].z - mu, d3 = v[i].w - mu;
    s2 += (d0 * d0 + d1 * d1) + (d2 * d2 + d3 * d3);
  }
  const float rstd = rsqrtf(wave_sum(s2) * (1.f / D) + 1e-6f);
  unsigned rm = 0u;
  int orow = row;
  if (perm) {
    const int b = row / ntok, i = row - b * ntok;
    orow = (i >> 4) * perm + b * 16 + (i & 15);
  }
#pragma unroll
  for (int i = 0; i < NV; ++i) {
    const int c = i * 256 + lane * 4;
    fh_store4_wt<T, 1, WT>(reinterpret_cast<typename T::elem*>(out) + fmt_pack_off(orow, c, D / 32),
              (v[i].x - mu) * rstd * (1.f + b[i].x) + a[i].x, (v[i].y - mu) * rstd * (1.f + b[i].y) + a[i].y,
              (v[i].z - mu) * rstd * (1.f + b[i].z) + a[i].z, (v[i].w - mu) * rstd * (1.f + b[i].w) + a[i].w, rm);
  }
  fh_range_flush<T>(sat, rm);
  if (touch) fmt_touch_retire(touched);
}

template <class T, int NV, int KS, bool TOUCH, bool WT>
__global__ __launch_bounds__(256) void fmt_lnmod_kernel(float* __restrict__ x, const float* __restrict__ shift,
                                                        const float* __restrict__ scale, const float* __restrict__ slab,
                                                        const float* __restrict__ gate, int M, int ldm, int wpb, unsigned slab_stride,
                                                        u16* __restrict__ out, const float* __restrict__ red_bias, TouchSpec pf,
                                                        int ntok, int perm, unsigned long long* sat) {
  const LnRed red{slab, (size_t)slab_stride, red_bias, gate};
  fmt_lnmod_body<T, NV, KS, TOUCH, WT>(x, M, shift, scale, ldm, out, red, pf, ntok, perm, sat, wpb);
}

template <class T, int LPQ, bool TOUCH, bool WT>
__device__ __forceinline__ void fmt_attn_body(const u16* __restrict__ qkv, int ld, u16* __restrict__ out, int ntok, int M, int D,
                                              int window, const FmtDiv ntok_div, const TouchSpec& pf, unsigned long long* sat,
                                              const int h, const int run, const int nthr, const unsigned lin, const unsigned nwg) {
  constexpr int HD = 128, PD = HD / LPQ, NU = PD / 8;
  const int row_ = run * (nthr / LPQ) + threadIdx.x / LPQ, part = threadIdx.x % LPQ;
  unsigned touched[2] = {0u, 0u};
  auto touch = [&]() {
    if constexpr (TOUCH) {
      fmt_touch(pf, lin & 7, (lin >> 3) * nthr + threadIdx.x, (nwg >> 3) * nthr, touched);
    }
  };
  if (row_ >= M) {
    touch();
    if constexpr (TOUCH) fmt_touch_retire(touched);
    return;
  }
  const int b = (int)fmt_div((unsigned)row_, ntok_div), qi = row_ - b * ntok;
  const int d0 = h * HD + part * PD;
  const float scale = rsqrtf((float)HD);
  typedef typename T::elem E;
  typedef typename T::pack8 P8;
  const E* base = reinterpret_cast<const E*>(qkv) + (size_t)(b * ntok) * ld + d0;
  float qf[PD], o[PD];
  P8 qq[NU];
#pragma unroll
  for (int u = 0; u < NU; ++u) qq[u] = T::load8(base + (size_t)qi * ld + u * 8);
  auto scale_q = [&]() {
#pragma unroll
    for (int u = 0; u < NU; ++u) {
#pragma unroll
      for (int j = 0; j < 8; ++j) qf[u * 8 + j] = T::get(qq[u], j) * scale;
    }
  };
#pragma unroll
  for (int i = 0; i < PD; ++i) o[i] = 0.f;
  float m = -INFINITY, l = 0.f;
  auto score = [&](const P8* k) {
    float dot = 0.f;
#pragma unroll
    for (int u = 0; u < NU; ++u) {
#pragma unroll
      for (int j = 0; j < 8; ++j) dot += qf[u * 8 + j] * T::get(k[u], j);
    }
    return group_sum<LPQ>(dot);
  };
  auto fold = [&](float dot, const P8* v) {
    const float mn = fmaxf(m, dot);
    const float alpha = __expf(m - mn), p = __expf(dot - mn);
    l = l * alpha + p;
    m = mn;
#pragma unroll
    for (int u = 0; u < NU; ++u) {
#pragma unroll
      for (int j = 0; j < 8; ++j) o[u * 8 + j] = o[u * 8 + j] * alpha + p * T::get(v[u], j);
    }
  };
  if (window <= 2) {
    P8 kk[5][NU], vv[5][NU];
#pragma unroll
    for (int t = 0; t < 5; ++t) {
      const int kj = min(max(qi + t - 2, 0), ntok - 1);
      const E* kp = base + (size_t)kj * ld + D;
#pragma unroll
      for (int u = 0; u < NU; ++u) {
        kk[t][u] = T::load8(kp + u * 8);
        vv[t][u] = T::load8(kp + D + u * 8);
      }
    }
    touch();
    scale_q();
#pragma unroll
    for (int t = 0; t < 5; ++t) {
      const int kj = qi + t - 2;
      const float dot = score(kk[t]);
      if (kj >= 0 && kj < ntok && (t - 2 >= -window) && (t - 2 <= window)) fold(dot, vv[t]);
    }
  } else {
    touch();
    scale_q();
    for (int kj = qi - window; kj <= qi + window; ++kj) {
// ... 27 lines not shown
template <class T, int LPQ, bool TOUCH, bool WT>
__global__ __launch_bounds__(512) void fmt_attn_kernel(const u16* __restrict__ qkv, u16* __restrict__ out, int ld, int ntok, int M,
                                                       int D, int window, int nthr, unsigned ntok_mul, unsigned ntok_sh, int heads,
                                                       int nrun, unsigned long long* sat, TouchSpec pf) {
  fmt_attn_body<T, LPQ, TOUCH, WT>(qkv, ld, out, ntok, M, D, window, FmtDiv{ntok_mul, ntok_sh}, pf, sat, blockIdx.x, blockIdx.y,
                                   nthr, blockIdx.x + (unsigned)heads * blockIdx.y, (unsigned)(heads * nrun));
}

constexpr int kXlaneProbeVecs = 64, kXlaneProbeSums = 5;
__global__ __launch_bounds__(64) void fmt_xlane_probe_kernel(const float* __restrict__ in, float* __restrict__ out) {
  const int lane = threadIdx.x;
  const float v = in[blockIdx.x * 64 + lane];
  float* o = out + (size_t)blockIdx.x * kXlaneProbeSums * 2 * 64 + lane;
  o[0 * 64] = wave_sum(v), o[1 * 64] = wave_sum_shfl(v);
  o[2 * 64] = wave_max(v), o[3 * 64] = wave_max_shfl(v);
  o[4 * 64] = group_sum<16>(v), o[5 * 64] = group_sum_shfl<16>(v);
  o[6 * 64] = group_sum<8>(v), o[7 * 64] = group_sum_shfl<8>(v);
  o[8 * 64] = group_sum<4>(v), o[9 * 64] = group_sum_shfl<4>(v);
}

template <class T>
__global__ void fmt_build_cond_kernel(u16* __restrict__ out, int ld, int bc, int ntok, int n_prev, int dim_w, int dim_a,
                                      int dim_e, const float* __restrict__ wr, const float* __restrict__ wa,
                                      const float* __restrict__ prev_wa, const float* __restrict__ we, int we_len,
                                      const float* __restrict__ prev_we, unsigned wr_mask, unsigned wa_mask,
                                      unsigned we_mask, unsigned long long* sat) {
  const int row = blockIdx.x;
  const int s = row / ntok, i = row % ntok, q = s / bc, b = s - q * bc, n_cur = ntok - n_prev;
  const bool on_r = (wr_mask >> b) & 1, on_a = (wa_mask >> b) & 1, on_e = (we_mask >> b) & 1;
  wr += (size_t)q * dim_w;
  wa += (size_t)q * n_cur * dim_a;
  prev_wa += (size_t)q * n_prev * dim_a;
  we += (size_t)q * we_len * dim_e;
  if (prev_we) prev_we += (size_t)q * n_prev * dim_e;
  unsigned rm = 0u;
  for (int c = threadIdx.x; c < ld; c += blockDim.x) {
    float v = 0.f;
    if (c < dim_w) {
      v = on_r ? wr[c] : 0.f;
    } else if (c < dim_w + dim_a) {
      const int k = c - dim_w;
      if (i < n_prev) v = prev_wa[i * dim_a + k];
      else if (on_a) v = wa[(i - n_prev) * dim_a + k];
    } else if (c < dim_w + dim_a + dim_e) {
      const int k = c - dim_w - dim_a;
      if (on_e) {
        if (we_len == 1) v = we[k];
        else v = (i < n_prev) ? prev_we[i * dim_e + k] : we[(i - n_prev) * dim_e + k];
      }
    }
    reinterpret_cast<typename T::elem*>(out)[fmt_pack_off(row, c, ld / 32)] = fh_cvt<T>(v, rm);
  }
  fh_range_flush<T>(sat, rm);
}

__device__ __forceinline__ float fmt_linspace01(int i, int n) {
  if (n <= 1) return 0.f;
  const float step = __fdiv_rn(1.0f, (float)(n - 1));
  return (i < n / 2) ? __fmul_rn(step, (float)i) : __fsub_rn(1.0f, __fmul_rn(step, (float)(n - 1 - i)));
}
template <class T>
__global__ void fmt_tsin_kernel(u16* __restrict__ out, const float* __restrict__ freqs, int n_steps, float t0, int nfe,
                                int stages, float c0, float c1, float c2, float c3) {
  const int s = blockIdx.x;
  if (s >= n_steps) return;
  float t = t0;
  if (nfe > 0) {
    const int i = s / stages, j = s - i * stages;
    const float gi = fmt_linspace01(i, nfe);
    t = gi;
    if (j > 0) {
      const float cj = j == 1 ? c1 : (j == 2 ? c2 : c3);
      t = __fadd_rn(gi, __fmul_rn(__fsub_rn(fmt_linspace01(i + 1, nfe), gi), cj));
    }
  }
  (void)c0;
  const int k = threadIdx.x;
  const float arg = t * freqs[k & 127];
  reinterpret_cast<typename T::elem*>(out)[fmt_pack_off(s, k, 8)] = T::from_float(k < 128 ? cosf(arg) : sinf(arg));
}

template <class T>
__global__ void fmt_silu_c_kernel(u16* __restrict__ out, const float* __restrict__ temb, const float* __restrict__ ccond,
                                  int M, int D, size_t step_stride, int dense_rows, unsigned long long* sat) {
  const int idx = (blockIdx.x * blockDim.x + threadIdx.x) * 8;
  if (idx >= M * D) return;
  const int c = idx % D, row = idx / D + (int)blockIdx.y * dense_rows;
  typename T::elem* const o = reinterpret_cast<typename T::elem*>(out) + (dense_rows ? (size_t)0 : (size_t)blockIdx.y * step_stride);
  temb += (size_t)blockIdx.y * D;
  typename T::pack8 u;
#pragma unroll
  for (int h = 0; h < 2; ++h) {
    const float4 a = *reinterpret_cast<const float4*>(ccond + idx + 4 * h);
    const float4 t = *reinterpret_cast<const float4*>(temb + c + 4 * h);
    T::set(u, 4 * h + 0, fh_silu(a.x + t.x));
    T::set(u, 4 * h + 1, fh_silu(a.y + t.y));
    T::set(u, 4 * h + 2, fh_silu(a.z + t.z));
    T::set(u, 4 * h + 3, fh_silu(a.w + t.w));
  }
  unsigned rm = 0u;
  fh_track_pack<T>(rm, u);
  fh_range_flush<T>(sat, rm);
  T::store8(o + fmt_pack_off(row, c, D / 32), u);
}

template <class T>
__global__ void fmt_init_x_kernel(float* __restrict__ xcur, u16* __restrict__ xin16, int ldx, const float* __restrict__ x0,
                                  const float* __restrict__ prev_x, int n_prev, int n_cur, int dim_w, int nclip,
                                  unsigned long long* sat) {
  const int idx = blockIdx.x * blockDim.x + threadIdx.x;
  const int ntok = n_prev + n_cur;
  if (idx >= nclip * ntok * dim_w) return;
  const int q = idx / (ntok * dim_w), r = idx - q * ntok * dim_w;
  const int i = r / dim_w, c = r % dim_w;
  float v;
  if (i < n_prev) {
    v = prev_x[((size_t)q * n_prev + i) * dim_w + c];
  } else {
    v = x0[((size_t)q * n_cur + (i - n_prev)) * dim_w + c];
    xcur[((size_t)q * n_cur + (i - n_prev)) * dim_w + c] = v;
  }
  unsigned rm = 0u;
  reinterpret_cast<typename T::elem*>(xin16)[fmt_pack_off(q * ntok + i, c, ldx)] = fh_cvt<T>(v, rm);
  fh_range_flush<T>(sat, rm);
}

template <class T>
__global__ void fmt_rk_combine_kernel(float* __restrict__ xcur, const float* __restrict__ kbuf, size_t kstride, int nk, float c0,
                                      float c1, float c2, float c3, int final, u16* __restrict__ xin16, int ldx, int n_prev,
                                      int n_cur, int W, int nclip, unsigned long long* sat) {
  const int idx = blockIdx.x * blockDim.x + threadIdx.x;
  if (idx >= nclip * n_cur * W) return;
  const int q = idx / (n_cur * W), r = idx - q * n_cur * W;
  const int i = r / W, c = r % W, ntok = n_prev + n_cur;
  const float cf[4] = {c0, c1, c2, c3};
  float y = xcur[idx];
  for (int m = 0; m < nk; ++m) y += cf[m] * kbuf[(size_t)m * kstride + ((size_t)q * ntok + n_prev + i) * W + c];
  if (final) xcur[idx] = y;
  unsigned rm = 0u;
  reinterpret_cast<typename T::elem*>(xin16)[fmt_pack_off(q * ntok + n_prev + i, c, ldx)] = fh_cvt<T>(y, rm);
  fh_range_flush<T>(sat, rm);
}

__global__ void fmt_slice_pad_kernel(float* __restrict__ dst, const float* __restrict__ src, int t0, int T, int n, int dim,
                                     int nclip) {
  const int idx = blockIdx.x * blockDim.x + threadIdx.x;
  if (idx >= nclip * n * dim) return;
  const int q = idx / (n * dim), r = idx - q * n * dim;
  const int i = r / dim, c = r % dim;
  const int t = min(t0 + i, T - 1);
  dst[idx] = src[((size_t)q * T + t) * dim + c];
}

__global__ void fmt_tail_kernel(float* __restrict__ dst, const float* __restrict__ src, int n_prev, int n_cur, int dim, int nclip) {
  const int idx = blockIdx.x * blockDim.x + threadIdx.x;
  if (idx >= nclip * n_prev * dim) return;
  const int q = idx / (n_prev * dim), r = idx - q * n_prev * dim;
  dst[idx] = src[((size_t)q * n_cur + (n_cur - n_prev)) * dim + r];
}

constexpr int kFmtMaxClips = 16;
template <class P>
struct FmtClipTab {
  P p[kFmtMaxClips];
  int T[kFmtMaxClips];
};

__global__ void fmt_gather_pad_kernel(float* __restrict__ dst, const FmtClipTab<const float*> src, int t0, int n, int dim) {
  const int r = blockIdx.x * blockDim.x + threadIdx.x, q = blockIdx.y;
  if (r >= n * dim) return;
// ... 21 lines not shown
```

comfyui-float_optimized_amd/csrc/fmt_launch.hpp:

```cpp
#pragma once
#include <type_traits>

#include "fmt_weights.hpp"

namespace {

constexpr int kLdsMax = 160 * 1024;
constexpr int kWtRows = 256;

typedef void (*GemmKernel)(GemmArgs);
typedef void (*GemmHeadKernel)(const u16*, const u16*, int, int, int, int, unsigned, unsigned, unsigned, unsigned, unsigned, unsigned, GemmTail);

template <class K>
void raise_lds(K kern, int bytes) {
  if (hipFuncSetAttribute(reinterpret_cast<const void*>(kern), hipFuncAttributeMaxDynamicSharedMemorySize, bytes) != hipSuccess)
    (void)hipGetLastError();
}

template <int... Vs, class F>
bool with_const(int v, F&& f) {
  return ((v == Vs && (f(std::integral_constant<int, Vs>{}), true)) || ...);
}

struct FmtLaunch {
  const FmtTune& tn;
  hipStream_t s;
  unsigned long long* sat;
  float *xres, *slab;
  u16 *h16, *qkv16, *att16;
  int D, ntok, Ntot, Mpad, heads, attn_window;
};


template <int MTW, int NT>
struct Tile {};
template <class T, int EPI, int NW, class F, int... MTW, int... NT>
void gemm_tiles(F& f, Tile<MTW, NT>...) {
  (f(fmt_gemm_kernel<T, MTW, NT, NW, EPI>, MTW, NT, NW, NW * MTW * 16 * NT * 16 * (int)sizeof(float)), ...);
}
template <class T, int EPI, int NW, class F>
void gemm_split_tiles(F& f) {
  gemm_tiles<T, EPI, NW>(f, Tile<3, 1>{}, Tile<3, 2>{}, Tile<3, 4>{}, Tile<5, 1>{}, Tile<5, 2>{}, Tile<5, 4>{}, Tile<4, 1>{},
                         Tile<4, 2>{}, Tile<6, 2>{}, Tile<2, 1>{}, Tile<1, 1>{});
}
template <class T, int EPI, class F>
void for_each_gemm(F&& f) {
  if constexpr (T::is32) {
    gemm_tiles<T, EPI, 4>(f, Tile<1, 1>{}, Tile<2, 1>{}, Tile<3, 1>{}, Tile<4, 1>{}, Tile<5, 1>{});
    if constexpr (EPI == EPI_CFG) gemm_tiles<T, EPI, 8>(f, Tile<1, 1>{}, Tile<3, 1>{}, Tile<4, 1>{});
  } else {
    gemm_split_tiles<T, EPI, 4>(f);
    gemm_split_tiles<T, EPI, 8>(f);
    gemm_split_tiles<T, EPI, 16>(f);
    if constexpr (EPI == EPI_F32 || EPI == EPI_CFG) {
      gemm_tiles<T, EPI, 4>(f, Tile<12, 2>{}, Tile<15, 2>{}, Tile<12, 1>{}, Tile<15, 1>{});
      gemm_tiles<T, EPI, 8>(f, Tile<12, 1>{}, Tile<15, 1>{});
    }
  }
}
template <int MTW, int KCH, int NWV>
struct WideTile {};
template <class T, class F, int... MTW, int... KCH, int... NWV>
void wide_tiles(F& f, WideTile<MTW, KCH, NWV>...) {
  (f(fmt_gemm_wide_kernel<T, MTW, KCH, NWV>, MTW, KCH, NWV, 2 * MTW * KCH * 1024), ...);
}
template <class T, class F>
void for_each_wide(F&& f) {
  wide_tiles<T>(f, WideTile<4, 4, 4>{}, WideTile<5, 4, 4>{}, WideTile<6, 4, 4>{}, WideTile<6, 2, 4>{}, WideTile<12, 2, 4>{},
                WideTile<12, 4, 4>{}, WideTile<12, 2, 8>{}, WideTile<12, 4, 8>{});
}
template <class T, int NWC, int NS, int STG, class F>
void dma_tile(F& f) {
  f(fmt_gemm_dma_kernel<T, NWC, NS, STG>, NWC, NS, STG, NS * (12 + 5 * NWC) * 1024);
}
template <class T, class F>
void for_each_dma(F&& f) {
  dma_tile<T, 4, 4, 0>(f);
  dma_tile<T, 4, 4, 1>(f);
}
template <class T, int EPI, int MI, int NJ, int KPS, int NS, class F>
void rbs_tile(F& f, int shape) {
  f(fmt_gemm_rbs_kernel<T, MI, NJ, KPS, NS, EPI>, shape, 32 * MI, 32 * NJ, KPS, fmt_rb_smem(MI, NJ, KPS, NS));
}
template <class T, int EPI, class F>
void for_each_rbs(F&& f) {
  rbs_tile<T, EPI, 3, 2, 2, 4>(f, 0);
  rbs_tile<T, EPI, 3, 4, 2, 4>(f, 1);
  rbs_tile<T, EPI, 6, 4, 2, 3>(f, 2);
}

constexpr int kBigSmem = 4 * 28 * 1024 + 4 * 4096;

template <class T>
void prime_kernels() {
  auto raise = [](auto kern, int, int, int, int smem) {
    if (smem <= kLdsMax) raise_lds(kern, smem);
  };
  for_each_gemm<T, EPI_F32>(raise);
  for_each_gemm<T, EPI_T16>(raise);
  for_each_gemm<T, EPI_SILU_P16>(raise);
  for_each_gemm<T, EPI_GELU_P16>(raise);
  for_each_gemm<T, EPI_GATE_RES>(raise);
  for_each_gemm<T, EPI_XEMBED>(raise);
  for_each_gemm<T, EPI_CFG>(raise);
  for_each_gemm<T, EPI_PARTIAL>(raise);
  for_each_gemm<T, EPI_GELUERF_P16>(raise);
  if constexpr (!T::is32) {
    auto raise_rb = [](GemmKernel kern, int, int, int, int, int smem) { raise_lds(kern, smem); };
    raise_lds(fmt_gemm_big4_kernel<T, 4>, kBigSmem);
    for_each_dma<T>(raise);
    for_each_wide<T>(raise);
    for_each_rbs<T, EPI_T16>(raise_rb);
    for_each_rbs<T, EPI_GELU_P16>(raise_rb);
// ... 100 lines not shown
    for_each_rbs<T, EPI>([&](GemmKernel k, int sh, int r, int c, int kp, int bytes) {
      if (sh == want) kern = k, rows = r, bn = c, kps = kp, smem = bytes;
    });
    if (EPI != EPI_PARTIAL || g.ksplit < 1) g.ksplit = 1;
    FH_REQUIRE(g.N % bn == 0 && (g.K / 32) % (g.ksplit * kps) == 0 && g.K / 32 / g.ksplit / kps >= 1,
               "row-blocked GEMM: N=%d K=%d not tileable by %d columns / %d K slices of %d-k-block stages", g.N, g.K, bn, g.ksplit, kps);
    g.mblk = (g.M + rows - 1) / rows;
    g.touch.W = nullptr;
    const dim3 grid((unsigned)((g.N / bn) * g.mblk * g.ksplit));
    fh_launch_prof(3, kern, grid, dim3(512), smem, s, g);
    FH_CHECK_HIP(hipGetLastError());
    return FLOAT_OK;
  }
}
constexpr int kRbMinRows = 300;
struct RbPlan {
  int shape = -1, ksplit = 1;
};
RbPlan pick_rb(const FmtTune& tn, int layer, int M) {
  RbPlan p;
  if (!tn.rb || M < kRbMinRows) return p;
  const int tier = M < 540 ? 0 : (M < 1100 ? 1 : (M < 2200 ? 2 : 3));
  static const int shapes[4][4] = { {0, 1, 0, 2},  {-1, 0, 0, 2},  {0, 1, 2, 2},  {0, 1, 2, 2}};
  p.shape = shapes[layer][tier];
  p.ksplit = layer == RB_PROJ ? 2 : (layer == RB_FC2 ? (tier == 3 ? 2 : 4) : 1);
  const FmtTune::Rb& o = tn.rb_layer[layer];
  if (o.n >= 1) {
    p.shape = o.shape;
    const int ks = o.ksplit;
    if (o.n >= 2 && (layer == RB_PROJ || layer == RB_FC2) && (ks == 1 || ks == 2 || ks == 4 || ks == 8)) p.ksplit = ks;
  }
  return p;
}

struct Tiling {
  int mtw, nt, nw;
};
int pick_nw(int K, int forced) {
  const int KB = K / 32;
  if (forced && KB % forced == 0) return forced;
  if (KB >= 128 && KB % 16 == 0) return 16;
  if (KB >= 32 && KB % 8 == 0) return 8;
  return 4;
}
Tiling pick_tiling(const FmtTune& tn, int M, int N, int K, bool need_full_rows) {
  const int mt = (M + 15) / 16;
  if (need_full_rows) {
    if (mt <= 4) return {4, 1, pick_nw(K, 0)};
    return {mt <= 12 ? 12 : 15, 1, (tn.full_nw == 8 && (K / 32) % 8 == 0) ? 8 : 4};
  }
  int split = mt <= 4 ? 4 : (mt <= 12 ? 3 : 5);
  if (mt <= 2) split = mt;
  const int blocks = (mt + split - 1) / split;
  const bool wide = N >= 16384;
  if (mt >= 12) {
    const int* o = tn.plan + (wide ? 3 : 0);
    if (o[0]) {
      int nw = o[0] >= 12 ? 4 : pick_nw(K, o[2]);
      while (nw > 4 && nw * o[0] * 16 * o[1] * 16 * 4 > kLdsMax) nw >>= 1;
      return {o[0], o[1], nw};
    }
  }
  if (wide) return {mt <= 4 ? 4 : 6, 2, std::min(8, pick_nw(K, 0))};
  if (mt > 15 && N % 64 == 0) return {3, 4, 4};
  int nt = 1;
  if (mt >= 5) {
    if ((N / 64) * blocks >= 192 && N % 64 == 0) nt = 4;
    else if ((N / 32) * blocks >= 192 && N % 32 == 0) nt = 2;
  } else if ((N / 16) * blocks > 512) {
    nt = 2;
  }
  return {split, nt, pick_nw(K, 0)};
}
Tiling pick_tiling32(int M) {
  const int mt = (M + 15) / 16;
  return {mt <= 5 ? mt : (mt <= 12 ? 3 : 5), 1, 4};
}

GemmArgs base_args(const u16* A, const Lin& L, int M) {
  GemmArgs g;
  memset(&g, 0, sizeof(g));
  g.A = A, g.W = L.W, g.bias = L.b;
  g.K = L.K, g.N = L.N, g.M = M;
  return g;
}

template <class T, int EPI>
int run_gemm(const FmtTune& tn, GemmArgs g, hipStream_t s, bool need_full_rows = false, const LayerPlan* plan = nullptr) {
  if constexpr (T::is32) {
    FH_REQUIRE(!need_full_rows, "the fp32 mode has no all-rows CFG epilogue tiling (token-blocked head only)");
    const Tiling t = pick_tiling32(g.M);
    g.touch.W = nullptr;
    return launch_gemm<T, EPI>(g, t.mtw, t.nt, t.nw, s);
  }
  if (plan && plan->on() && (g.M + 15) / 16 <= 15) {
    g.touch.W = nullptr;
    return launch_gemm<T, EPI>(g, plan->v[0], plan->v[1], plan->v[2], s);
  }
  const Tiling t = pick_tiling(tn, g.M, g.N, g.K, need_full_rows);
  return launch_gemm<T, EPI>(g, t.mtw, t.nt, t.nw, s);
}

struct PendingRed {
  int ks = 0;
  LnRed red{};
};
void to_slab(GemmArgs& g, float* slab, int Mpad, int ks) {
  g.ksplit = ks, g.out_f32 = slab, g.ldo = g.N, g.slab_stride = (size_t)Mpad * g.N;
}
PendingRed pending_red(float* slab, int Mpad, int D, const float* bias, const float* gate, int ks) {
  return PendingRed{ks, LnRed{slab, (size_t)Mpad * D, bias, gate}};
}
template <class T>
int run_gemm_partial(const FmtLaunch& cx, GemmArgs g, int ksplit, const LayerPlan* plan = nullptr) {
  to_slab(g, cx.slab, cx.Mpad, ksplit);
  if (plan && plan->on() && !T::is32 && (g.M + 15) / 16 <= 15) {
    g.touch.W = nullptr;
    return launch_gemm<T, EPI_PARTIAL>(g, plan->v[0], plan->v[1], plan->v[2], cx.s);
  }
  Tiling t = T::is32 ? pick_tiling32(g.M) : pick_tiling(cx.tn, g.M, g.N * ksplit, g.K / ksplit, false);
  while (t.nt > 1 && g.N % (t.nt * 16)) t.nt >>= 1;
  if (T::is32) g.touch.W = nullptr;
  return launch_gemm<T, EPI_PARTIAL>(g, t.mtw, t.nt, t.nw, cx.s);
}

int log2_exact(unsigned v) {
  int n = 0;
  while ((1u << n) < v) ++n;
  return (1u << n) == v ? n : -1;
}

TouchSpec make_touch(const FmtTune& tn, const Lin& L, int M, int ksplit, unsigned lanes, unsigned per_lane, int force_nt = 0) {
  TouchSpec t{};
  Tiling tl = ksplit ? pick_tiling(tn, M, L.N * ksplit, L.K / ksplit, false) : pick_tiling(tn, M, L.N, L.K, false);
  if (force_nt) tl.nt = force_nt;
  if (ksplit)
    while (tl.nt > 1 && L.N % (tl.nt * 16)) tl.nt >>= 1;
  const int ks = ksplit ? ksplit : 1;
  if (L.N % (tl.nt * 16) || L.K % (32 * ks) || 8 % ks) return t;
  const int nbn = L.N / (tl.nt * 16);
  if ((nbn * ks) % 8) return t;
  const unsigned P = 8 / ks, run_lines = (unsigned)(L.K / 32 / ks) * 8u;
  if (log2_exact(run_lines) < 0 || log2_exact((unsigned)tl.nt) < 0) return t;
  t.run_shift = (unsigned)log2_exact(run_lines);
  t.nt_shift = (unsigned)log2_exact((unsigned)tl.nt);
  t.p_shift = (unsigned)log2_exact(P);
  t.tile_bytes = (unsigned)(L.K / 32) * 1024u;
  t.total = ((unsigned)nbn / P) * (unsigned)tl.nt * run_lines;
  if ((size_t)t.total > (size_t)lanes * per_lane) return t;
  t.W = reinterpret_cast<const char*>(L.W);
  return t;
}

TouchSpec make_touch_rb(const Lin& L, int shape, int kb, unsigned lanes, unsigned per_lane) {
  TouchSpec t{};
  const int ct = shape == 0 ? 4 : 8;
  if (kb <= 0 || (kb & (kb - 1)) || L.N % (ct * 16) || (L.N / (ct * 16)) % 8 || L.K / 32 < kb) return t;
  const unsigned run_lines = (unsigned)kb * 8u;
  t.run_shift = (unsigned)log2_exact(run_lines);
  t.nt_shift = (unsigned)log2_exact((unsigned)ct);
  t.p_shift = 3;
  t.tile_bytes = (unsigned)(L.K / 32) * 1024u;
  t.total = (unsigned)(L.N / (ct * 16) / 8) * (unsigned)ct * run_lines;
  if ((size_t)t.total > (size_t)lanes * per_lane) return t;
  t.W = reinterpret_cast<const char*>(L.W);
  return t;
}

unsigned gemm_lanes_per_xcd(const FmtTune& tn, int M, int N, int K) {
  const Tiling t = pick_tiling(tn, M, N, K, false);
  const int mblk = ((M + 15) / 16 + t.mtw - 1) / t.mtw;
  return (unsigned)((N / (t.nt * 16)) * mblk / 8) * (unsigned)(t.nw * 64);
}


template <class T>
int launch_lnmod(const FmtLaunch& cx, int M, const float* shift, const float* scale, PendingRed* pend = nullptr,
                 const Lin* next = nullptr, u16* out = nullptr, int perm = 0, int touch_bit = 1, int rb_shape = -1) {
  const int rpw = cx.tn.ln_rows;
  dim3 grid(rpw == 1 ? ((M + 63) / 64) * 64 : (M + rpw - 1) / rpw), block(64 * rpw);
  const int ks = pend ? pend->ks : 0;
  const bool wt = M <= kWtRows;
  LnRed red{};
  if (ks) red = pend->red;
  TouchSpec pf{};
  if (next && (cx.tn.touch & (1 | touch_bit)) && rpw == 1 && !T::is32)
    pf = rb_shape >= 0 ? make_touch_rb(*next, rb_shape, cx.tn.rb_touch, (grid.x / 8) * 64, 6)
                       : make_touch(cx.tn, *next, M, 0, (grid.x / 8) * 64, 6);
  decltype(&fmt_lnmod_kernel<T, 1, 0, false, false>) kern = nullptr;
  with_const<1, 2, 4, 8>(cx.D / 256, [&](auto NV) {
    with_const<0, 1, 2, 4, 8>((ks == 0 || ks == 1 || ks == 2 || ks == 4) ? ks : 8, [&](auto KS) {
      with_const<0, 1>(pf.W != nullptr, [&](auto TOUCH) {
        with_const<0, 1>(wt, [&](auto WT) {
          kern = fmt_lnmod_kernel<T, decltype(NV)::value, decltype(KS)::value, decltype(TOUCH)::value != 0, decltype(WT)::value != 0>;
        });
      });
    });
  });
  FH_REQUIRE(kern, "dim_h %d unsupported (must be 256*{1,2,4,8})", cx.D);
  FH_REQUIRE(red.slab_stride <= 0xffffffffull, "split-K slab of %zu elements is beyond the LayerNorm kernel's 32-bit stride", red.slab_stride);
  hipLaunchKernelGGL(kern, grid, block, 0, cx.s, cx.xres, shift, scale, red.slab, red.gate, M, cx.Ntot, rpw, (unsigned)red.slab_stride,
                     out ? out : cx.h16, red.bias, pf, cx.ntok, perm, cx.sat);
  if (pend) pend->ks = 0;
  FH_CHECK_HIP(hipGetLastError());
  return FLOAT_OK;
}

template <class T>
void launch_attn(const FmtLaunch& cx, int M, const Lin* pull) {
  const int qpw = cx.tn.attn_qpw, lpq = cx.tn.attn_lpq;
  dim3 grid(cx.heads, (M + qpw - 1) / qpw), block(qpw * lpq);
  TouchSpec pf{};
  if (pull && !T::is32) pf = make_touch(cx.tn, *pull, M, 0, (grid.x * grid.y / 8) * block.x, 2);
  decltype(&fmt_attn_kernel<T, 8, false, false>) kern = nullptr;
  with_const<16, 8>(lpq == 16 ? 16 : 8, [&](auto LPQ) {
    with_const<0, 1>(pf.W != nullptr, [&](auto TOUCH) {
      with_const<0, 1>(M <= kWtRows, [&](auto WT) {
        kern = fmt_attn_kernel<T, decltype(LPQ)::value, decltype(TOUCH)::value != 0, decltype(WT)::value != 0>;
      });
    });
  });
  const FmtDiv nd = fmt_make_div((unsigned)cx.ntok);
  hipLaunchKernelGGL(kern, grid, block, 0, cx.s, cx.qkv16, cx.att16, 3 * cx.D, cx.ntok, M, cx.D, cx.attn_window, (int)block.x, nd.mul, nd.sh,
                     (int)grid.x, (int)grid.y, cx.sat, pf);
}

}
```

comfyui-float_optimized_amd/csrc/fmt_pack.hpp:

```cpp
#pragma once
#include "common.hpp"
#include "fmt_decode.hpp"

enum {
  EPI_F32 = 0,
  EPI_T16 = 1,
  EPI_SILU_P16 = 2,
  EPI_GELU_P16 = 3,
  EPI_GATE_RES = 4,
  EPI_XEMBED = 5,
  EPI_CFG = 6,
  EPI_PARTIAL = 7,
  EPI_GELUERF_P16 = 8
};

__host__ __device__ __forceinline__ size_t fmt_pack_off(int row, int k, int KB) {
  return ((size_t)((row >> 4) * KB + (k >> 5)) * 64 + (row & 15) + 16 * ((k >> 3) & 3)) * 8 + (k & 7);
}

template <class T>
__global__ void fmt_dbg_to16_kernel(u16* __restrict__ dst, const float* __restrict__ src, int n) {
  const int i = blockIdx.x * blockDim.x + threadIdx.x;
  if (i < n) reinterpret_cast<typename T::elem*>(dst)[i] = T::from_float(src[i]);
}
template <class T>
__global__ void fmt_dbg_unpack_kernel(float* __restrict__ dst, const u16* __restrict__ src, int rows, int D) {
  const int i = blockIdx.x * blockDim.x + threadIdx.x;
  if (i >= rows * D) return;
  const int r = i / D, c = i - r * D;
  dst[i] = T::to_float(reinterpret_cast<const typename T::elem*>(src)[fmt_pack_off(r, c, D / 32)]);
}

struct TouchSpec {
  const char* W;
  unsigned run_shift;
  unsigned nt_shift;
  unsigned p_shift;
  unsigned tile_bytes;
  unsigned total;
};

__device__ __forceinline__ unsigned fmt_touch_line(const TouchSpec& t, unsigned xcd, unsigned l) {
  if (l >= t.total) return 0u;
  const unsigned r = l >> t.run_shift, off = l & ((1u << t.run_shift) - 1u);
  const unsigned cb = r >> t.nt_shift, jn = r & ((1u << t.nt_shift) - 1u);
  const unsigned ks = xcd >> t.p_shift, bx = (cb << t.p_shift) + (xcd & ((1u << t.p_shift) - 1u));
  return *reinterpret_cast<const unsigned*>(t.W + (size_t)((bx << t.nt_shift) + jn) * t.tile_bytes +
                                            ((size_t)((ks << t.run_shift) + off) << 7));
}
template <int N>
__device__ __forceinline__ void fmt_touch(const TouchSpec& t, unsigned xcd, unsigned first, unsigned stride, unsigned (&v)[N]) {
#pragma unroll
  for (int i = 0; i < N; ++i) v[i] = fmt_touch_line(t, xcd, first + (unsigned)i * stride);
}
template <int N>
__device__ __forceinline__ void fmt_touch_always(const TouchSpec& t, const void* idle, unsigned xcd, unsigned first, unsigned stride,
                                                 unsigned (&v)[N]) {
#pragma unroll
  for (int i = 0; i < N; ++i) {
    unsigned l = first + (unsigned)i * stride;
    const bool on = t.W != nullptr && l < t.total;
    l = on ? l : 0u;
    const unsigned r = l >> t.run_shift, off = l & ((1u << t.run_shift) - 1u);
    const unsigned cb = r >> t.nt_shift, jn = r & ((1u << t.nt_shift) - 1u);
    const unsigned ks = xcd >> t.p_shift, bx = (cb << t.p_shift) + (xcd & ((1u << t.p_shift) - 1u));
    const char* p = t.W + (size_t)((bx << t.nt_shift) + jn) * t.tile_bytes + ((size_t)((ks << t.run_shift) + off) << 7);
    v[i] = *reinterpret_cast<const unsigned*>(on ? p : reinterpret_cast<const char*>(idle));
  }
}
template <int N>
__device__ __forceinline__ void fmt_touch_retire(const unsigned (&v)[N]) {
  unsigned o = 0u;
#pragma unroll
  for (int i = 0; i < N; ++i) o |= v[i];
  asm volatile("" ::"v"(o));
}
template <int N>
__device__ __forceinline__ void fmt_touch_retire_last(const unsigned (&v)[N]) {
  unsigned o = 0u;
#pragma unroll
  for (int i = 0; i < N; ++i) o |= v[i];
  asm volatile("" ::"v"(o) : "memory");
}

struct GemmHead {
  const u16* A;
  const u16* W;
  int K;
  int kbs;
  int ksplit;
  int mblk;
  GemmDecode dec;
};
struct GemmTail {
  const float* bias;
  int M, N;
  float* out_f32;
  int ldo;
  u16* out16;
  int ldo16;
  const float* gate;
  int ldg;
  const float* pos;
  int bc, ntok, n_prev;
  int nclip;
  float a_cfg, r_cfg, e_cfg, dt;
  float* vout;
  float* xcur;
  u16* xin16;
  int ldx;
  size_t slab_stride;
  TouchSpec touch;
  int zcount, zgroup;
  size_t a_zstride, o_zstride;
  int tokblk;
  unsigned long long* sat;
};
struct GemmArgs : GemmHead, GemmTail {};
static_assert(sizeof(GemmHead) == 14 * 4, "the head is what the dispatch can preload: 14 dwords");

inline void fmt_gemm_head(GemmArgs& g, int bn, bool partial) {
  g.kbs = (g.K >> 5) / (partial ? g.ksplit : 1);
  g.dec = fmt_make_decode(g.N / bn, g.mblk, g.ksplit, partial);
}
```

comfyui-float_optimized_amd/csrc/tuning.hpp:

```cpp
#pragma once
#include <stdio.h>
#include <stdlib.h>
#include <string.h>

#include <algorithm>
#include <string>

inline int env_int(const char* name, int dflt, int lo, int hi) {
  const char* v = getenv(name);
  if (!v || !*v) return dflt;
  char* end = nullptr;
  const long x = strtol(v, &end, 10);
  return (end && *end == 0 && x >= lo && x <= hi) ? (int)x : dflt;
}
inline int env_atoi(const char* name, int dflt) {
  const char* v = getenv(name);
  return v ? atoi(v) : dflt;
}
inline bool env_set(const char* name) { return getenv(name) != nullptr; }
inline int env_scan(const char* s, int* v) { int n = 0; return sscanf(s, "%d%n", v, &n) == 1 ? n : 0; }
inline int env_scan(const char* s, double* v) { int n = 0; return sscanf(s, "%lf%n", v, &n) == 1 ? n : 0; }
template <class V>
int env_list(const char* name, V* v, int n, char sep = ',') {
  const char* s = getenv(name);
  int got = 0;
  while (s && got < n) {
    const int used = env_scan(s, v + got);
    if (!used) break;
    ++got;
    s += used;
    if (sep == ',' && *s++ != ',') break;
  }
  return got;
}

struct LayerPlan {
  int v[3] = {0, 0, 0};
  bool on() const { return v[0] > 0; }
};

enum { RB_QKV = 0, RB_PROJ, RB_FC1, RB_FC2 };

struct FmtTune {
  bool wide = true;
  int wide_variant = 7;
  bool big = true;
  bool rb = true;
  int rb_touch = 16;
  struct Rb {
    int n = 0, shape = -1, ksplit = 1;
  } rb_layer[4];
  int full_nw = 8;
  int plan[6] = {0, 0, 0, 0, 0, 0};
  LayerPlan plan_layer[4];
  int fc2_split = 4;
  int proj_split = 0;
  int touch = 230;
  bool hoist = true;
  int zgroup = 0;
  int ln_rows = 1;
  int attn_qpw = 8, attn_lpq = 16;
  bool no_tokblk = false;
  bool pack_host = false;

  static FmtTune from_env() {
    FmtTune t;
    t.wide = env_atoi("FLOAT_FMT_WIDE", 1) != 0;
    t.wide_variant = env_atoi("FLOAT_FMT_WIDE_VARIANT", t.wide_variant);
    t.big = env_atoi("FLOAT_FMT_BIG", 1) != 0;
    t.rb = env_atoi("FLOAT_FMT_RB", 1) != 0;
    t.rb_touch = env_atoi("FLOAT_FMT_RB_TOUCH", t.rb_touch);
    static const char* const layers[4] = {"QKV", "PROJ", "FC1", "FC2"};
    for (int l = 0; l < 4; ++l) {
      const std::string s = layers[l];
      int rb[2] = {-1, 1};
      t.rb_layer[l].n = env_list(("FLOAT_FMT_RB_" + s).c_str(), rb, 2);
      t.rb_layer[l].shape = rb[0];
      t.rb_layer[l].ksplit = rb[1];
      env_list(("FLOAT_FMT_PLAN_" + s).c_str(), t.plan_layer[l].v, 3);
    }
    t.full_nw = env_atoi("FLOAT_FMT_FULL_NW", t.full_nw);
    env_list("FLOAT_FMT_PLAN", t.plan, 6);
    t.fc2_split = env_atoi("FLOAT_FMT_FC2_SPLIT", t.fc2_split);
    t.proj_split = env_atoi("FLOAT_FMT_PROJ_SPLIT", t.proj_split);
    t.touch = env_atoi("FLOAT_FMT_TOUCH", t.touch);
    t.hoist = env_atoi("FLOAT_FMT_HOIST", 1) != 0;
    t.zgroup = std::max(0, env_atoi("FLOAT_FMT_ZGROUP", 0));
    t.ln_rows = std::max(1, std::min(4, env_atoi("FLOAT_FMT_LN_ROWS", 1)));
    int attn[2] = {t.attn_qpw, t.attn_lpq};
    env_list("FLOAT_FMT_ATTN", attn, 2);
    t.attn_lpq = attn[1] == 16 ? 16 : 8;
    t.attn_qpw = std::max(1, std::min(512 / t.attn_lpq, attn[0]));
    t.no_tokblk = env_set("FLOAT_FMT_NO_TOKBLK");
    t.pack_host = env_atoi("FLOAT_PACK_HOST", 0) != 0;
    return t;
  }
};

struct DecTune {
  int lds_pad = 0;
  unsigned ride_wgs = 16;
  int ride_min_res = 64;
  unsigned ride_pace = 3;
  double ride_w[4][3] = {{170, 140, 50}, {170, 155, 100}, {220, 200, 180}, {300, 250, 120}};
  bool cb_order = true;
  int conv_bn = 64, conv_bn_lo = 32;
  int tpw = 0;
  bool no_zfuse = false;
  int zblur_min = 64;
  int flow_pix = 0;
  int flow_wgs = 2048;
  bool flow_epi = true;
  bool yuv_fused = true;
  bool write_pyr = false;
  bool copy_memcpy = false;
  bool style_norm = true;

  static DecTune from_env() {
    DecTune t;
    t.lds_pad = env_int("FLOAT_DEC_LDS_PAD", 0, 0, 160 * 1024);
    t.ride_wgs = (unsigned)env_int("FLOAT_DEC_RIDE_WGS", 16, 0, 64) / 8 * 8;
    t.ride_min_res = env_int("FLOAT_DEC_RIDE_MIN_RES", 64, 64, 512);
    t.ride_pace = (unsigned)env_int("FLOAT_DEC_RIDE_PACE", 3, 0, 64);
    double w[12];
    if (env_list("FLOAT_DEC_RIDE_W", w, 12, ' ') == 12)
      for (int i = 0; i < 12; ++i)
        if (w[i] > 0.0 && w[i] < 1e6) t.ride_w[i / 3][i % 3] = w[i];
    t.cb_order = env_atoi("FLOAT_DEC_CB_ORDER", 1) != 0;
    t.conv_bn = env_int("FLOAT_DEC_CONV_BN", 64, 32, 64);
    t.conv_bn_lo = env_int("FLOAT_DEC_CONV_BN_LO", 32, 32, 64);
    t.tpw = env_int("FLOAT_DEC_TPW", 0, 0, 4096);
    t.no_zfuse = env_set("FLOAT_DEC_NO_ZFUSE");
    t.zblur_min = env_int("FLOAT_DEC_ZBLUR_MIN", 64, 16, 4096);
    t.flow_pix = env_int("FLOAT_DEC_FLOW_PIX", 0, 0, 4);
    t.flow_wgs = env_int("FLOAT_DEC_FLOW_WGS", 2048, 8, 1 << 20);
    t.flow_epi = env_int("FLOAT_DEC_FLOW_EPI", 1, 0, 1) != 0;
    t.yuv_fused = env_int("FLOAT_DEC_YUV_FUSED", 1, 0, 1) != 0;
    t.write_pyr = env_set("FLOAT_DEC_WRITE_PYR");
    const char* copy = getenv("FLOAT_DEC_COPY");
    t.copy_memcpy = copy && !strcmp(copy, "memcpy");
    t.style_norm = env_int("FLOAT_DEC_STYLE_NORM", 1, 0, 1) != 0;
    return t;
  }
};

struct EncTune {
  bool no_tiles = false;
  static EncTune from_env() { return EncTune{env_set("FLOAT_ENC_NO_TILES")}; }
};

struct AudTune {
  bool attn_mfma = true;
  static AudTune from_env() { return AudTune{env_atoi("FLOAT_AUD_ATTN_MFMA", 1) != 0}; }
};
```

comfyui-float_optimized_amd/fmt.py:

```python
import ctypes as C
import math

import torch

from . import native
from .config import FmtConfig


@native.rebuildable
class FlowMatchingTransformerHIP:

    def __init__(self, state_dict, cfg: FmtConfig = None, device="cuda:0", dtype="fp16", use_graph=2, max_batch=1):
        self.cfg = cfg or FmtConfig()
        self.device = torch.device(device)
        self.dtype = dtype = native.canon_dtype(dtype)
        self.max_batch = max(1, int(max_batch))
        L = native.lib()
        c = self.cfg
        ncfg = native.FmtCfg(c.dim_w, c.dim_a, c.dim_e, c.dim_h, c.fmt_depth, c.num_heads,
                             int(c.dim_h * c.mlp_ratio), c.num_prev_frames, c.num_frames_for_clip,
                             c.attention_window, native.DTYPES[dtype], int(use_graph), self.max_batch)
        sd = {k[4:] if k.startswith("fmt.") else k: v for k, v in state_dict.items()
              if k not in ("alignment_mask", "fmt.alignment_mask")}
        arr, keep = native.tensor_table(sd)
        h = C.c_void_p()
        with torch.cuda.device(self.device):
            native.check(L.float_fmt_create(C.byref(ncfg), arr, len(sd), C.byref(h)))
        self._h = h
        del keep

    def set_method(self, name):
        if name not in native.ODE_METHODS:
            raise ValueError("unknown fixed-step ODE method %r (known: %s)" % (name, ", ".join(native.ODE_METHODS)))
        native.check(native.lib().float_fmt_set_method(self._h, native.ODE_METHODS[name]))
        self.method = name

    @torch.no_grad()
    def pos_embed_in_use(self):
        out = torch.empty(self.cfg.n_tokens, self.cfg.dim_h, device=self.device, dtype=torch.float32)
        with torch.cuda.device(self.device):
            native.check(native.lib().float_fmt_debug(self._h, 0, None, native.dev_ptr(out), native.stream_ptr(self.device)))
        return out

    @torch.no_grad()
    def attention_probe(self, qkv):
        qkv = self._f(qkv)
        if qkv.shape != (self.cfg.n_tokens, 3 * self.cfg.dim_h):
            raise ValueError("qkv must be (%d,%d)" % (self.cfg.n_tokens, 3 * self.cfg.dim_h))
        out = torch.empty(self.cfg.n_tokens, self.cfg.dim_h, device=self.device, dtype=torch.float32)
        with torch.cuda.device(self.device):
            native.check(native.lib().float_fmt_debug(self._h, 1, native.dev_ptr(qkv), native.dev_ptr(out),
                                                      native.stream_ptr(self.device)))
        return out

    @torch.no_grad()
    def gemm_tile_probe(self, a, w):
        a, w = self._f(a), self._f(w)
        if a.shape != (48, 1024) or w.shape not in ((64, 1024), (16, 1024)):
            raise ValueError("a must be (48,1024) and w (64,1024) or (16,1024)")
        buf = torch.cat([a, w]).contiguous()
        out = torch.empty(48, w.shape[0], device=self.device, dtype=torch.float32)
        with torch.cuda.device(self.device):
            native.check(native.lib().float_fmt_debug(self._h, 3 if w.shape[0] == 64 else 4, native.dev_ptr(buf), native.dev_ptr(out),
                                                      native.stream_ptr(self.device)))
        return out

    @torch.no_grad()
    def xlane_probe(self, v):
        v = self._f(v)
        if v.dim() != 2 or v.shape[1] != 64:
            raise ValueError("v must be (n,64)")
        n, per = v.shape[0], native.XLANE_PROBE_VECS
        buf = torch.zeros(-(-n // per) * per, 64, device=self.device, dtype=torch.float32)
        buf[:n] = v
        out = torch.empty(buf.shape[0], 5, 2, 64, device=self.device, dtype=torch.float32)
        with torch.cuda.device(self.device):
            for i in range(0, buf.shape[0], per):
                native.check(native.lib().float_fmt_debug(self._h, 5, native.dev_ptr(buf[i:i + per]), native.dev_ptr(out[i:i + per]),
                                                          native.stream_ptr(self.device)))
        return out[:n]

    def saturation(self, reset=False):
        with torch.cuda.device(self.device):
            return native.saturation("float_fmt_saturation", self._h, self.device, reset)

    def close(self):
        if getattr(self, "_h", None) and native is not None:
            native.lib().float_fmt_destroy(self._h)
            self._h = None

    __del__ = close

    def _f(self, t):
        return None if t is None else t.to(self.device, torch.float32).contiguous()

    def _check_shapes(self, x, wa, wr, we, prev_x, prev_wa, prev_we):
        c = self.cfg
        B = x.shape[0]
        if x.shape != (B, c.num_frames_for_clip, c.dim_w):
            raise ValueError("x must be (B,%d,%d), got %s" % (c.num_frames_for_clip, c.dim_w, tuple(x.shape)))
        if wa.shape != (B, c.num_frames_for_clip, c.dim_a):
            raise ValueError("wa must be (B,%d,%d), got %s" % (c.num_frames_for_clip, c.dim_a, tuple(wa.shape)))
        if wr.shape != (B, c.dim_w):
            raise ValueError("wr must be (B,%d), got %s" % (c.dim_w, tuple(wr.shape)))
        if prev_x is None or prev_wa is None:
            raise ValueError("prev_x was provided, but prev_wa was not." if prev_x is not None
                             else "prev_x / prev_wa are required")
        if we.dim() != 3 or we.shape[2] != c.dim_e:
            raise ValueError("we must be (B,1|%d,%d)" % (c.num_frames_for_clip, c.dim_e))
        if we.shape[1] > 1 and prev_we is None:
            raise ValueError("`we` is dynamic (T>1), but prev_we was not provided with prev_x/prev_wa.")
        if we.shape[1] not in (1, c.num_frames_for_clip):
            raise ValueError("Dynamic emotion latent `we` time dimension (%d) does not match audio latent `wa` "
                             "time dimension (%d)." % (we.shape[1] + c.num_prev_frames,
                                                       c.num_frames_for_clip + c.num_prev_frames))

    @torch.no_grad()
    def forward_with_cfv(self, t, x, wa, wr, we, prev_x, prev_wa, prev_we=None, a_cfg_scale=1.0, r_cfg_scale=1.0,
                         e_cfg_scale=1.0, include_r_cfg=False, **kwargs):
        x, wa, wr, we, prev_x, prev_wa, prev_we = map(self._f, (x, wa, wr, we, prev_x, prev_wa, prev_we))
        self._check_shapes(x, wa, wr, we, prev_x, prev_wa, prev_we)
        c, L = self.cfg, native.lib()
        tval = float(torch.as_tensor(t).reshape(-1)[0])
        B = x.shape[0]
        out = torch.empty(B, c.n_tokens, c.dim_w, device=self.device, dtype=torch.float32)
        dynamic = we.shape[1] > 1
        with torch.cuda.device(self.device):
            s = native.stream_ptr(self.device)
            for b in range(B):
                native.check(L.float_fmt_eval(
                    self._h, tval, native.dev_ptr(x[b]), native.dev_ptr(wa[b]), native.dev_ptr(wr[b]),
                    native.dev_ptr(we[b]), we.shape[1], native.dev_ptr(prev_x[b]), native.dev_ptr(prev_wa[b]),
                    native.dev_ptr(prev_we[b]) if dynamic else None, a_cfg_scale, r_cfg_scale, e_cfg_scale,
                    1 if include_r_cfg else 0, native.dev_ptr(out[b]), s))
        return out

    @torch.no_grad()
    def sample_chunk(self, x0, wa, wr, we, prev_x, prev_wa, prev_we=None, nfe=10, a_cfg_scale=1.0, r_cfg_scale=1.0,
                     e_cfg_scale=1.0, include_r_cfg=False):
        x0, wa, wr, we, prev_x, prev_wa, prev_we = map(self._f, (x0, wa, wr, we, prev_x, prev_wa, prev_we))
        self._check_shapes(x0, wa, wr, we, prev_x, prev_wa, prev_we)
        c, L = self.cfg, native.lib()
        B = x0.shape[0]
        out = torch.empty(B, c.num_frames_for_clip, c.dim_w, device=self.device, dtype=torch.float32)
        dynamic = we.shape[1] > 1
        with torch.cuda.device(self.device):
            s = native.stream_ptr(self.device)
            for b in range(B):
                native.check(L.float_fmt_sample_chunk(
                    self._h, native.dev_ptr(x0[b]), native.dev_ptr(wa[b]), native.dev_ptr(wr[b]),
                    native.dev_ptr(we[b]), we.shape[1], native.dev_ptr(prev_x[b]), native.dev_ptr(prev_wa[b]),
                    native.dev_ptr(prev_we[b]) if dynamic else None, int(nfe), a_cfg_scale, r_cfg_scale, e_cfg_scale,
                    1 if include_r_cfg else 0, native.dev_ptr(out[b]), s))
        return out

    @torch.no_grad()
    def sample(self, r_s, wa, we, noise, nfe=10, a_cfg_scale=2.0, r_cfg_scale=1.0, e_cfg_scale=1.0,
               include_r_cfg=False):
        r_s, wa, we, noise = map(self._f, (r_s, wa, we, noise))
        c, L = self.cfg, native.lib()
        B, T = wa.shape[0], wa.shape[1]
        n_chunks = int(math.ceil(T / c.num_frames_for_clip))
        if noise.shape != (n_chunks, B, c.num_frames_for_clip, c.dim_w):
# ... 112 lines not shown
```

comfyui-float_optimized_amd/native.py:

```python
import ctypes as C
import os

import torch

_HERE = os.path.dirname(os.path.abspath(__file__))
LIB_PATH = os.path.join(_HERE, "csrc", "libfloat_hip.so")

FLOAT_DT_BF16, FLOAT_DT_FP16, FLOAT_DT_FP32 = 0, 1, 2
AUD_FRONT_NORMALIZE = 1
AUD_SEG_NORMALIZE = 1
IMG_RGBA_MODES = {"discard_alpha": 0, "blend_with_color": 1, "replace_with_color": 2}
IMG_OUT_NCHW_PM1, IMG_OUT_HWC_U8 = 0, 1
MATRIX_BT601_LIMITED = 0
IMG_MATRIX_BT601_LIMITED = 0
MATRIX_BT709_LIMITED, MATRIX_BT601_FULL, MATRIX_BT709_FULL = 2, 4, 6
IMG_FILTER_BICUBIC, IMG_FILTER_LANCZOS = 0, 1
ODE_METHODS = {"euler": 0, "midpoint": 1, "rk4": 2, "heun2": 3, "heun3": 4}
DTYPES = {"bf16": FLOAT_DT_BF16, "bfloat16": FLOAT_DT_BF16, "fp16": FLOAT_DT_FP16, "float16": FLOAT_DT_FP16,
          "fp32": FLOAT_DT_FP32, "float32": FLOAT_DT_FP32}
DTYPE_NAMES = {FLOAT_DT_BF16: "bf16", FLOAT_DT_FP16: "fp16", FLOAT_DT_FP32: "fp32"}
DEC_SAT_SITES = 40
XLANE_PROBE_VECS = 64
ABI_VERSION = 6

# ... 31 lines not shown
    _fields_ = [(n, C.c_int32) for n in ("size", "dim", "dim_motion", "dtype")]


class SfdCfg(C.Structure):
    _fields_ = [(n, C.c_int32) for n in ("dtype", "max_h", "max_w", "max_candidates", "max_boxes")]


class AudCfg(C.Structure):
    _fields_ = [("n_conv", C.c_int32), ("conv_dim", C.c_int32 * 8), ("conv_kernel", C.c_int32 * 8), ("conv_stride", C.c_int32 * 8)] + \
               [(n, C.c_int32) for n in ("hidden", "layers", "heads", "intermediate", "pos_k", "pos_groups", "dim_w", "only_last",
                                         "dtype")] + [("ln_eps", C.c_float)] + \
               [(n, C.c_int32) for n in ("feat_norm_layer", "stable_ln", "conv_bias", "num_labels")]


_F = C.POINTER(C.c_float)
_SIGNATURES = {
    "float_hip_abi_version": (C.c_int, []),
    "float_last_error": (C.c_char_p, []),
    "float_yuv_matrix": (C.c_int, [C.c_int32, C.POINTER(C.c_int32)]),
    "float_set_profiling": (C.c_int, [C.c_int32]),
    "float_probe_peaks": (C.c_int, [C.POINTER(C.c_float)] * 4 + [C.POINTER(C.c_int32)]),
    "float_profile_ms": (C.c_double, [C.c_int32, C.POINTER(C.c_int64)]),
    "float_stream_create_cu_range": (C.c_int, [C.c_int32, C.c_int32, C.POINTER(C.c_void_p)]),
    "float_stream_destroy": (C.c_int, [C.c_void_p]),
    "float_fmt_create": (C.c_int, [C.POINTER(FmtCfg), C.POINTER(FloatTensor), C.c_int32, C.POINTER(C.c_void_p)]),
    "float_fmt_destroy": (None, [C.c_void_p]),
    "float_fmt_set_method": (C.c_int, [C.c_void_p, C.c_int32]),
    "float_fmt_debug": (C.c_int, [C.c_void_p, C.c_int32, C.c_void_p, C.c_void_p, C.c_void_p]),
    "float_fmt_eval": (C.c_int, [C.c_void_p, C.c_float] + [C.c_void_p] * 4 + [C.c_int32] + [C.c_void_p] * 3 +
                       [C.c_float] * 3 + [C.c_int32, C.c_void_p, C.c_void_p]),
    "float_fmt_sample_chunk": (C.c_int, [C.c_void_p] + [C.c_void_p] * 4 + [C.c_int32] + [C.c_void_p] * 3 +
                               [C.c_int32] + [C.c_float] * 3 + [C.c_int32, C.c_void_p, C.c_void_p]),
    "float_fmt_sample": (C.c_int, [C.c_void_p, C.c_void_p, C.c_void_p, C.c_int32, C.c_void_p, C.c_int32, C.c_void_p,
                                   C.c_int32] + [C.c_float] * 3 + [C.c_int32, C.c_void_p, C.c_void_p]),
    "float_fmt_sample_batch": (C.c_int, [C.c_void_p, C.c_int32, C.c_void_p, C.c_void_p, C.c_int32, C.c_void_p, C.c_int32,
                                         C.c_void_p, C.c_int32] + [C.c_float] * 3 + [C.c_int32, C.c_void_p, C.c_void_p]),
    "float_fmt_sample_begin_ragged": (C.c_int, [C.c_void_p, C.c_int32, C.POINTER(C.c_int32)] + [C.POINTER(C.c_void_p)] * 3 +
                                      [C.c_int32, C.POINTER(C.c_void_p), C.c_int32] + [C.c_float] * 3 +
                                      [C.c_int32, C.POINTER(C.c_void_p)]),
    "float_fmt_sample_batch_ragged": (C.c_int, [C.c_void_p, C.c_int32, C.POINTER(C.c_int32)] + [C.POINTER(C.c_void_p)] * 3 +
                                      [C.c_int32, C.POINTER(C.c_void_p), C.c_int32] + [C.c_float] * 3 +
                                      [C.c_int32, C.POINTER(C.c_void_p), C.c_void_p]),
    "float_fmt_sample_begin": (C.c_int, [C.c_void_p, C.c_void_p, C.c_void_p, C.c_int32, C.c_void_p, C.c_int32, C.c_void_p,
                                         C.c_int32] + [C.c_float] * 3 + [C.c_int32, C.c_void_p]),
    "float_fmt_sample_next": (C.c_int, [C.c_void_p, C.c_void_p, C.POINTER(C.c_int32), C.POINTER(C.c_int32)]),
    "float_fmt_sample_begin_range": (C.c_int, [C.c_void_p, C.c_void_p, C.c_void_p, C.c_int32, C.c_void_p, C.c_int32, C.c_void_p,
                                               C.c_int32] + [C.c_float] * 3 + [C.c_int32, C.c_void_p, C.c_int32, C.c_int32] +
                                     [C.c_void_p] * 3),
    "float_dec_create": (C.c_int, [C.POINTER(DecCfg), C.POINTER(FloatTensor), C.c_int32, C.POINTER(C.c_void_p)]),
    "float_dec_destroy": (None, [C.c_void_p]),
    "float_dec_set_feats": (C.c_int, [C.c_void_p, C.POINTER(C.c_void_p), C.c_int32, C.c_void_p]),
    "float_dec_frames": (C.c_int, [C.c_void_p, C.c_void_p, C.c_void_p, C.c_int32, C.c_void_p, C.c_void_p]),
    "float_dec_frames_host": (C.c_int, [C.c_void_p, C.c_void_p, C.c_void_p, C.c_int32, C.c_void_p, C.c_void_p, C.c_void_p,
                                        C.c_void_p]),
    "float_dec_frames_u8": (C.c_int, [C.c_void_p, C.c_void_p, C.c_void_p, C.c_int32, C.c_void_p, C.c_void_p]),
    "float_dec_frames_host_u8": (C.c_int, [C.c_void_p, C.c_void_p, C.c_void_p, C.c_int32, C.c_void_p, C.c_void_p, C.c_void_p,
                                           C.c_void_p]),
    "float_dec_frames_i420": (C.c_int, [C.c_void_p, C.c_void_p, C.c_void_p, C.c_int32, C.c_int32, C.c_void_p, C.c_void_p]),
    "float_dec_frames_host_i420": (C.c_int, [C.c_void_p, C.c_void_p, C.c_void_p, C.c_int32, C.c_int32, C.c_void_p, C.c_void_p,
                                             C.c_void_p, C.c_void_p]),
    "float_dec_feat_shape": (C.c_int, [C.c_void_p, C.c_int32, C.POINTER(C.c_int32), C.POINTER(C.c_int32)]),
    "float_dec_frames_raw": (C.c_int, [C.c_void_p, C.c_void_p, C.c_void_p, C.c_int32, C.c_void_p, C.c_void_p]),
    "float_dec_direction": (C.c_int, [C.c_void_p, C.c_void_p, C.c_void_p, C.c_void_p]),
    "float_dec_saturation": (C.c_int, [C.c_void_p, C.POINTER(C.c_uint64), C.POINTER(C.c_uint64), C.c_int32, C.c_void_p]),
    "float_dec_debug_styled_conv": (C.c_int, [C.POINTER(DecUnit), C.POINTER(FloatTensor), C.c_int32, C.c_void_p, C.c_void_p,
                                              C.c_void_p, C.POINTER(C.c_uint64), C.c_void_p]),
    "float_dec_debug_flow_level": (C.c_int, [C.POINTER(DecUnit), C.POINTER(FloatTensor), C.c_int32] + [C.c_void_p] * 9),
    "float_dec_set_feats16": (C.c_int, [C.c_void_p, C.POINTER(C.c_void_p), C.c_int32, C.c_int32, C.c_void_p]),
    "float_enc_create": (C.c_int, [C.POINTER(EncCfg), C.POINTER(FloatTensor), C.c_int32, C.POINTER(C.c_void_p)]),
    "float_enc_destroy": (None, [C.c_void_p]),
    "float_enc_forward": (C.c_int, [C.c_void_p] * 5 + [C.POINTER(C.c_void_p), C.c_int32, C.c_void_p]),
    "float_aud_create": (C.c_int, [C.POINTER(AudCfg), C.POINTER(FloatTensor), C.c_int32, C.POINTER(C.c_void_p)]),
    "float_aud_destroy": (None, [C.c_void_p]),
    "float_aud_reserve": (C.c_int, [C.c_void_p, C.c_int32, C.c_int32, C.c_void_p]),
    "float_aud_classify": (C.c_int, [C.c_void_p, C.c_void_p, C.c_int32, C.c_void_p, C.c_void_p]),
    "float_aud_inference": (C.c_int, [C.c_void_p, C.c_void_p, C.c_int32, C.c_int32, C.c_void_p, C.c_void_p]),
    "float_aud_debug": (C.c_int, [C.c_void_p, C.c_int32, C.c_void_p, C.c_int32, C.c_void_p, C.c_void_p]),
    "float_aud_reserve_segments": (C.c_int, [C.c_void_p, C.c_int32, C.c_int32, C.c_void_p]),
    "float_aud_classify_segments": (C.c_int, [C.c_void_p, C.c_void_p, C.c_int32, C.c_int32, C.c_int64, C.c_int32, C.c_void_p, C.c_void_p,
                                              C.c_int32, C.c_float, C.c_void_p]),
    "float_aud_expand_rows": (C.c_int, [C.c_void_p, C.c_int32, C.c_int32, C.c_void_p, C.c_int32, C.c_float, C.c_void_p]),
    "float_enc_feats16": (C.c_int, [C.c_void_p, C.POINTER(C.c_void_p), C.POINTER(C.c_int32), C.c_int32, C.POINTER(C.c_int32)]),
    "float_enc_export_feats16": (C.c_int, [C.c_void_p, C.POINTER(C.c_void_p), C.c_int32, C.c_void_p]),
    "float_fmt_saturation": (C.c_int, [C.c_void_p, C.POINTER(C.c_uint64), C.c_int32, C.c_void_p]),
    "float_enc_saturation": (C.c_int, [C.c_void_p, C.POINTER(C.c_uint64), C.c_int32, C.c_void_p]),
    "float_aud_saturation": (C.c_int, [C.c_void_p, C.POINTER(C.c_uint64), C.c_int32, C.c_void_p]),
    "float_cmp_segments": (C.c_int, [C.c_void_p, C.c_void_p, C.c_int32, C.c_int64, C.c_float, C.c_void_p, C.c_void_p, C.c_size_t,
                                     C.c_void_p]),
    "float_cmp_work_bytes": (C.c_size_t, [C.c_int32, C.c_int64]),
    "float_aud_front_len": (C.c_int64, [C.c_int64, C.c_int32, C.c_int32]),
    "float_aud_front_work_bytes": (C.c_size_t, [C.c_int64, C.c_int32, C.c_int32]),
    "float_aud_front": (C.c_int, [C.c_void_p, C.c_int32, C.c_int64, C.c_int64, C.c_int32, C.c_int32, C.c_int32, C.c_float, C.c_int32,
                                  C.c_void_p, C.c_int64, C.c_void_p, C.c_size_t, C.c_void_p]),
    "float_img_front_work_bytes": (C.c_size_t, [C.c_int32] * 4),
    "float_img_front": (C.c_int, [C.c_void_p] + [C.c_int32] * 14 + [C.c_void_p, C.c_int32, C.c_int32, C.c_void_p, C.c_size_t, C.c_void_p]),
    "float_img_paste": (C.c_int, [C.c_void_p, C.c_int32, C.c_int32, C.c_void_p] + [C.c_int32] * 8 + [C.c_void_p, C.c_void_p]),
    "float_img_paste_i420": (C.c_int, [C.c_void_p, C.c_int32, C.c_int32, C.c_void_p] + [C.c_int32] * 9 + [C.c_void_p, C.c_void_p]),
    "float_img_resample_plan_ints": (C.c_size_t, [C.c_int32] * 4),
    "float_img_resample_plan": (C.c_int, [C.c_int32] * 5 + [C.POINTER(C.c_int32), C.c_size_t]),
    "float_img_resample_work_bytes": (C.c_size_t, [C.c_int32] * 10),
    "float_img_resample": (C.c_int, [C.c_void_p] + [C.c_int32] * 10 + [C.c_void_p, C.c_void_p, C.c_void_p, C.c_size_t, C.c_void_p, C.c_void_p]),
    "float_jpg_work_bytes": (C.c_size_t, [C.c_int32] * 4),
    "float_jpg_encode": (C.c_int, [C.c_void_p] + [C.c_int32] * 5 + [C.c_void_p, C.c_size_t, C.c_void_p, C.c_void_p, C.c_size_t, C.c_void_p]),
    "float_jpg_work_bytes_padded": (C.c_size_t, [C.c_int32] * 4),
    "float_jpg_encode_padded": (C.c_int, [C.c_void_p] + [C.c_int32] * 5 + [C.c_void_p, C.c_size_t, C.c_void_p, C.c_void_p, C.c_size_t, C.c_void_p]),
    "float_png_work_bytes": (C.c_size_t, [C.c_int32] * 4),
    "float_png_encode": (C.c_int, [C.c_void_p] + [C.c_int32] * 4 + [C.c_void_p, C.c_size_t, C.c_void_p, C.c_void_p, C.c_void_p, C.c_size_t,
                                   C.c_void_p]),
    "float_png_tables": (C.c_int, [C.POINTER(C.c_int32)]),
    "float_sfd_create": (C.c_int, [C.POINTER(SfdCfg), C.POINTER(FloatTensor), C.c_int32, C.POINTER(C.c_void_p)]),
    "float_sfd_destroy": (None, [C.c_void_p]),
    "float_sfd_detect": (C.c_int, [C.c_void_p, C.c_void_p, C.c_int32, C.c_int32, C.c_float, C.c_float, C.c_void_p, C.c_void_p, C.c_void_p]),
    "float_sfd_maps": (C.c_int, [C.c_void_p, C.c_void_p, C.c_int32, C.c_int32, C.c_void_p, C.c_void_p]),
    "float_sfd_post": (C.c_int, [C.c_void_p, C.c_void_p, C.c_int32, C.c_int32, C.c_float, C.c_float, C.c_void_p, C.c_void_p, C.c_void_p]),
    "float_sfd_dense": (C.c_int, [C.c_void_p, C.c_void_p, C.c_void_p]),
    "float_sfd_saturation": (C.c_int, [C.c_void_p, C.POINTER(C.c_uint64), C.c_int32, C.c_void_p]),
    "float_sfd_reserve_batch": (C.c_int, [C.c_void_p, C.c_int32, C.c_int32, C.c_int32]),
    "float_sfd_maps_batch": (C.c_int, [C.c_void_p, C.c_void_p, C.c_int32, C.c_int32, C.c_int32, C.c_void_p, C.c_void_p]),
    "float_sfd_post_batch": (C.c_int, [C.c_void_p, C.c_void_p, C.c_int32, C.c_int32, C.c_int32, C.c_float, C.c_float, C.c_void_p, C.c_void_p,
                                       C.c_void_p]),
    "float_sfd_detect_batch": (C.c_int, [C.c_void_p, C.c_void_p, C.c_int32, C.c_int32, C.c_int32, C.c_float, C.c_float, C.c_void_p, C.c_void_p,
                                         C.c_void_p]),
    "float_sfd_dense_batch": (C.c_int, [C.c_void_p, C.c_void_p, C.c_void_p]),
}
EXPORTS = tuple(_SIGNATURES)

_lib = None


def lib():
    global _lib
    if _lib is not None:
        return _lib
    if not os.path.exists(LIB_PATH):
        raise NativeLibraryError(
            "libfloat_hip.so not built: run `python -c 'import __graft_entry__ as g; g.build()'` or "
            "`make -C comfyui-float_optimized_amd/csrc` (there is no CPU fallback)")
    try:
        L = C.CDLL(LIB_PATH)
    except OSError as e:
        raise NativeLibraryError("cannot load %s: %s" % (LIB_PATH, e)) from e
    for name, (res, args) in _SIGNATURES.items():
        try:
            fn = getattr(L, name)
        except AttributeError as e:
            raise NativeLibraryError("libfloat_hip.so does not export %s" % name) from e
        fn.restype = res
        fn.argtypes = args
    if L.float_hip_abi_version() != ABI_VERSION:
        raise NativeLibraryError("libfloat_hip.so ABI version mismatch")
    _lib = L
    return L


_ERR_TYPES = {1: ValueError, 2: KeyError, 3: RuntimeError, 4: MemoryError}


def check(rc):
    if rc != 0:
        msg = lib().float_last_error().decode("utf-8", "replace")
        raise _ERR_TYPES.get(rc, RuntimeError)(msg)


def tensor_table(state):
    keep = []
    arr = (FloatTensor * len(state))()
# ... 110 lines not shown
```

include/float_hip.h:

```cpp
#ifndef FLOAT_HIP_H
#define FLOAT_HIP_H

#include <stddef.h>
#include <stdint.h>

#ifdef __cplusplus
extern "C" {
#endif

#define FLOAT_HIP_ABI_VERSION 6

enum {
  FLOAT_OK = 0,
  FLOAT_E_INVALID = 1,
  FLOAT_E_MISSING = 2,
  FLOAT_E_HIP = 3,
  FLOAT_E_NOMEM = 4
};

enum { FLOAT_DT_BF16 = 0, FLOAT_DT_FP16 = 1, FLOAT_DT_FP32 = 2 };

typedef struct {
  const char* name;
  const float* data;
// ... 102 lines not shown

#define FLOAT_DEC_SAT_SITES 40
int float_dec_saturation(float_dec_t* h, uint64_t* total, uint64_t* per_site, int32_t reset, void* stream);

typedef struct {
  int32_t dtype;
  int32_t cin, cout;
  int32_t res;
  int32_t upsample;
  int32_t n_frames;
  int32_t style_dim;
  int32_t flags;
} float_dec_unit_t;
int float_dec_debug_styled_conv(const float_dec_unit_t* u, const float_tensor_t* tensors, int32_t n_tensors, const float* x,
                                const float* style, float* out, uint64_t* saturated, void* stream);
int float_dec_debug_flow_level(const float_dec_unit_t* u, const float_tensor_t* tensors, int32_t n_tensors, const float* x,
                               const float* feat, const float* style, const float* prev_flow, const float* prev_rgb,
                               float* out_flow, float* out_blend, float* out_rgb, void* stream);

int float_dec_direction(float_dec_t* h, const float* lam, float* r_s, void* stream);

int float_dec_set_feats16(float_dec_t* h, const void* const* feats16, int32_t n_feats, int32_t dtype,
                          void* stream);

typedef struct {
  int32_t size;
  int32_t dim;
  int32_t dim_motion;
  int32_t dtype;
} float_enc_cfg_t;

typedef struct float_enc float_enc_t;

int float_enc_create(const float_enc_cfg_t* cfg, const float_tensor_t* tensors, int32_t n_tensors,
                     float_enc_t** out);
void float_enc_destroy(float_enc_t* h);

int float_enc_forward(float_enc_t* h, const float* img, float* s_r, float* lam, float* r_s,
                      float* const* feats, int32_t n_feats, void* stream);

int float_enc_saturation(float_enc_t* h, uint64_t* total, int32_t reset, void* stream);
int float_enc_feats16(float_enc_t* h, const void** feats16, int32_t* channels, int32_t max_feats,
                      int32_t* n_out);
int float_enc_export_feats16(float_enc_t* h, void* const* dst, int32_t n_feats, void* stream);

typedef struct {
  int32_t n_conv;
  int32_t conv_dim[8], conv_kernel[8], conv_stride[8];
  int32_t hidden, layers, heads, intermediate;
  int32_t pos_k, pos_groups;
  int32_t dim_w;
  int32_t only_last;
  int32_t dtype;
  float ln_eps;
  int32_t feat_norm_layer;
  int32_t stable_ln;
  int32_t conv_bias;
  int32_t num_labels;
} float_aud_cfg_t;

typedef struct float_aud float_aud_t;

int float_aud_create(const float_aud_cfg_t* cfg, const float_tensor_t* tensors, int32_t n_tensors,
                     float_aud_t** out);
void float_aud_destroy(float_aud_t* h);

int float_aud_reserve(float_aud_t* h, int32_t n_samples, int32_t seq_len, void* stream);
int float_aud_saturation(float_aud_t* h, uint64_t* total, int32_t reset, void* stream);

int float_aud_inference(float_aud_t* h, const float* a, int32_t n_samples, int32_t seq_len, float* wa,
                        void* stream);

int float_aud_classify(float_aud_t* h, const float* a, int32_t n_samples, float* scores, void* stream);

int float_aud_debug(float_aud_t* h, int32_t what, const float* in, int32_t Tn, float* out, void* stream);

enum { FLOAT_AUD_SEG_NORMALIZE = 1 };
int float_aud_reserve_segments(float_aud_t* h, int32_t n_seg, int32_t seg_len, void* stream);
int float_aud_classify_segments(float_aud_t* h, const float* a, int32_t n_seg, int32_t seg_len, int64_t seg_stride, int32_t flags,
                                float* scores , float* frames , int32_t T,
                                float scale, void* stream);
int float_aud_expand_rows(const float* rows, int32_t n, int32_t c, float* frames, int32_t T, float scale, void* stream);

int float_hip_abi_version(void);
const char* float_last_error(void);
int float_yuv_matrix(int32_t matrix, int32_t table[15]);
int float_stream_create_cu_range(int32_t cu_begin, int32_t cu_end, void** stream_out);
int float_stream_destroy(void* stream);
int float_set_profiling(int32_t on);
double float_profile_ms(int32_t which, int64_t* n_launches);
int float_probe_peaks(float* hbm_read_gbps, float* hbm_copy_gbps, float* mfma16_tflops, float* mfma32_tflops, int32_t* n_cu);

int float_cmp_segments(const float* a, const float* b, int32_t n_seg, int64_t seg_len, float thr, double* stats, void* work,
                       size_t work_bytes, void* stream);
size_t float_cmp_work_bytes(int32_t n_seg, int64_t seg_len);

enum { FLOAT_AUD_FRONT_NORMALIZE = 1 };
int64_t float_aud_front_len(int64_t n_in, int32_t rate_in, int32_t rate_out);
size_t float_aud_front_work_bytes(int64_t n_in, int32_t rate_in, int32_t rate_out);
int float_aud_front(const float* w, int32_t channels, int64_t ch_stride, int64_t n_in, int32_t rate_in, int32_t rate_out,
                    int32_t zeros, float rolloff, int32_t flags, float* a, int64_t n_out, void* work, size_t work_bytes,
                    void* stream);

enum { FLOAT_IMG_RGBA_DISCARD = 0, FLOAT_IMG_RGBA_BLEND = 1, FLOAT_IMG_RGBA_REPLACE = 2 };
enum { FLOAT_IMG_OUT_NCHW_PM1 = 0, FLOAT_IMG_OUT_HWC_U8 = 1 };
size_t float_img_front_work_bytes(int32_t src_h, int32_t src_w, int32_t dst_h, int32_t dst_w);
int float_img_front(const float* img, int32_t src_h, int32_t src_w, int32_t channels, int32_t rect_x, int32_t rect_y, int32_t rect_w,
                    int32_t rect_h, int32_t scale_num, int32_t scale_den, int32_t rgba_mode, int32_t bkg_r, int32_t bkg_g, int32_t bkg_b,
                    int32_t out_mode, void* out, int32_t dst_h, int32_t dst_w, void* work, size_t work_bytes, void* stream);

int float_img_paste(const uint8_t* src8, int32_t src_h, int32_t src_w, const uint8_t* frames8, int32_t n_frames, int32_t fr_h,
                    int32_t fr_w, int32_t rect_x, int32_t rect_y, int32_t rect_w, int32_t rect_h, int32_t feather, uint8_t* out,
                    void* stream);

enum { FLOAT_IMG_MATRIX_BT601_LIMITED = 0 };
enum { FLOAT_IMG_MATRIX_BT709_LIMITED = 2, FLOAT_IMG_MATRIX_BT601_FULL = 4, FLOAT_IMG_MATRIX_BT709_FULL = 6 };
int float_img_paste_i420(const uint8_t* src8, int32_t src_h, int32_t src_w, const uint8_t* frames8, int32_t n_frames, int32_t fr_h,
                         int32_t fr_w, int32_t rect_x, int32_t rect_y, int32_t rect_w, int32_t rect_h, int32_t feather, int32_t matrix,
                         uint8_t* out, void* stream);

enum { FLOAT_IMG_FILTER_BICUBIC = 0, FLOAT_IMG_FILTER_LANCZOS = 1 };
size_t float_img_resample_plan_ints(int32_t n_in, int32_t n_out, int32_t filter, int32_t count);
int float_img_resample_plan(int32_t n_in, int32_t n_out, int32_t filter, int32_t first, int32_t count, int32_t* table,
                            size_t table_ints);
size_t float_img_resample_work_bytes(int32_t n_frames, int32_t fr_h, int32_t fr_w, int32_t box_h, int32_t box_w, int32_t filter,
                                     int32_t win_x, int32_t win_y, int32_t win_w, int32_t win_h);
int float_img_resample(const uint8_t* frames8, int32_t n_frames, int32_t fr_h, int32_t fr_w, int32_t box_h, int32_t box_w,
                       int32_t filter, int32_t win_x, int32_t win_y, int32_t win_w, int32_t win_h, const int32_t* tab_x,
                       const int32_t* tab_y, void* work, size_t work_bytes, uint8_t* out, void* stream);

size_t float_jpg_work_bytes(int32_t n_frames, int32_t h, int32_t w, int32_t restart);
int float_jpg_encode(const uint8_t* rgb8, int32_t n_frames, int32_t h, int32_t w, int32_t quality, int32_t restart, uint8_t* out, size_t out_cap,
                     int64_t* offsets, void* work, size_t work_bytes, void* stream);

size_t float_jpg_work_bytes_padded(int32_t n_frames, int32_t h, int32_t w, int32_t restart);
int float_jpg_encode_padded(const uint8_t* rgb8, int32_t n_frames, int32_t h, int32_t w, int32_t quality, int32_t restart, uint8_t* out,
                            size_t out_cap, int64_t* offsets, void* work, size_t work_bytes, void* stream);

size_t float_png_work_bytes(int32_t n_frames, int32_t h, int32_t w, int32_t band);
int float_png_encode(const uint8_t* rgb8, int32_t n_frames, int32_t h, int32_t w, int32_t band, uint8_t* out, size_t out_cap, int64_t* offsets,
                     uint32_t* crcs, void* work, size_t work_bytes, void* stream);
int float_png_tables(int32_t lengths[8 * 257]);

typedef struct {
  int32_t dtype;
  int32_t max_h, max_w;
  int32_t max_candidates;
  int32_t max_boxes;
} float_sfd_cfg_t;

typedef struct float_sfd float_sfd_t;

int float_sfd_create(const float_sfd_cfg_t* cfg, const float_tensor_t* tensors, int32_t n_tensors, float_sfd_t** out);
void float_sfd_destroy(float_sfd_t* h);
int float_sfd_detect(float_sfd_t* h, const void* rgb8, int32_t H, int32_t W, float score_thr, float iou_thr, float* boxes, int32_t* counts,
                     void* stream);
int float_sfd_maps(float_sfd_t* h, const void* rgb8, int32_t H, int32_t W, float* maps12, void* stream);
int float_sfd_post(float_sfd_t* h, const float* maps12, int32_t H, int32_t W, float score_thr, float iou_thr, float* boxes, int32_t* counts,
                   void* stream);
int float_sfd_dense(float_sfd_t* h, float* scores_boxes, void* stream);
int float_sfd_saturation(float_sfd_t* h, uint64_t* total, int32_t reset, void* stream);

int float_sfd_reserve_batch(float_sfd_t* h, int32_t n, int32_t H, int32_t W);
int float_sfd_maps_batch(float_sfd_t* h, const void* rgb8, int32_t n, int32_t H, int32_t W, float* maps12, void* stream);
int float_sfd_post_batch(float_sfd_t* h, const float* maps12, int32_t n, int32_t H, int32_t W, float score_thr, float iou_thr, float* boxes,
                         int32_t* counts, void* stream);
// ... 9 lines not shown
```

Before: 2638 frames/s.

## Compute only distinct adaLN modulation rows and reuse previous window's rows via row map

Adds a row-deduplication plan for the per-evaluation adaLN modulation GEMM. Only the distinct conditioning rows across CFG branches and tokens are computed, and rows identical to the previous window's are read from a double-buffered slab. LayerNorm and gated-residual kernels index modulation through a packed row map. This shrinks the modulation GEMM's M dimension, at the cost of extra graph variants, per-row index arithmetic in hot kernels and more state tracked across windows.

```diff
diff --git a/comfyui-float_optimized_amd/csrc/fmt_api.hip b/comfyui-float_optimized_amd/csrc/fmt_api.hip
--- a/comfyui-float_optimized_amd/csrc/fmt_api.hip
+++ b/comfyui-float_optimized_amd/csrc/fmt_api.hip
@@ -15,6 +15,8 @@
 
 constexpr int kMaxTok = 80;
 constexpr int kMaxSteps = 1024;
+constexpr int kScSteps = 64;
+constexpr int kRowsVariants = 5;
 
 }
 
@@ -40,6 +42,15 @@
   float* modall = nullptr;
   int Mmod = 0;
   size_t mod_zs = 0;
+  int Mmod1 = 0;
+  struct {
+    bool valid = false;
+    int par = 0, zs = 0, window = 0, nev = 0, method = 0, bc = 0;
+    uint64_t job = 0;
+    bool first = false;
+    ModLayout lay;
+  } rows_prev;
+  uint64_t job_serial = 0;
   struct GraphKey {
     int nfe, bc, we_len, method;
     int prio;
@@ -48,7 +59,7 @@
   };
   struct GraphEntry {
     GraphKey key;
-    hipGraphExec_t exec[kFmtMaxClips + 1];
+    hipGraphExec_t exec[kRowsVariants][kFmtMaxClips + 1];
     uint64_t used;
   };
   std::vector<GraphEntry> graphs;
@@ -89,8 +100,16 @@
 }
 
 
-constexpr int kScSteps = 64;
-
+
+struct RowsPlan {
+  bool on = false;
+  int variant = 0;
+  int par = 0;
+  bool first = true;
+  bool big = false;
+  int zs = 0, prev_zs = 0, prev_par = 0;
+  ModLayout lay, prev_lay;
+};
 static int stream_priority(hipStream_t s) {
   int prio = 0;
   if (hipStreamGetPriority(s, &prio) != hipSuccess) {
@@ -100,25 +119,36 @@
   return prio;
 }
 
-template <class T>
-int run_mod_all(float_fmt* h, int M, int e0, int n, hipStream_t s) {
+float* rows_slab(const float_fmt* h, int par) { return h->modall + (size_t)par * kScSteps * h->Mmod1 * h->Ntot; }
+
+template <class T>
+int run_mod_all(float_fmt* h, int M, int e0, int n, hipStream_t s, const RowsPlan* rp = nullptr) {
   const int D = h->D;
+  const bool rows = rp && rp->on;
+  ModSegs segs = ModSegs();
+  float* const modall = rows ? rows_slab(h, rp->par) : h->modall;
+  const int Mmod = rows ? h->Mmod1 : h->Mmod;
+  if (rows) {
+    FH_REQUIRE(e0 == 0, "distinct modulation rows: one batch of evaluations per window");
+    M = rp->lay.rows, segs = rp->lay.segs;
+  }
   const FmtTune& tn = h->tune;
   FH_REQUIRE(n >= 1 && n <= kScSteps, "modulation batch of %d evaluations (max %d)", n, kScSteps);
   const int prio = (s == h->cap_stream && s) ? h->cap_prio : stream_priority(s);
   const bool big = !T::is32 && tn.wide && prio == 0 && big_shape_ok(tn, n * M, h->adaln_all.N, h->adaln_all.K, h->n_cu);
+  FH_REQUIRE(!rows || (big == rp->big && rp->zs == (big ? M : Mmod)), "distinct modulation rows: the plan and the launch disagree");
   hipLaunchKernelGGL((fmt_silu_c_kernel<T>), dim3((M * D / 8 + 255) / 256, n), dim3(256), 0, s, h->sc16, h->temb + (size_t)e0 * D,
-                     h->ccond, M, D, (size_t)h->Mpad * D, big ? M : 0, h->sat);
-  h->mod_zs = big ? (size_t)M * h->Ntot : (size_t)h->Mmod * h->Ntot;
+                     h->ccond, M, D, (size_t)h->Mpad * D, big ? M : 0, h->sat, segs);
+  h->mod_zs = big ? (size_t)M * h->Ntot : (size_t)Mmod * h->Ntot;
   if constexpr (!T::is32) {
-    if (big) return launch_big4<T>(h->sc16, h->adaln_all, h->modall, n * M, h->Ntot, h->n_cu, s);
+    if (big) return launch_big4<T>(h->sc16, h->adaln_all, modall, n * M, h->Ntot, h->n_cu, s);
   }
   GemmArgs g = base_args(h->sc16, h->adaln_all, M);
-  g.sat = h->sat, g.out_f32 = h->modall, g.ldo = h->Ntot, g.zcount = n;
+  g.sat = h->sat, g.out_f32 = modall, g.ldo = h->Ntot, g.zcount = n;
   const bool dma = (tn.wide_variant == 6 || tn.wide_variant == 7) && (M + 15) / 16 > 4 && dma_shape_ok(g, 320);
   g.zgroup = tn.zgroup > 0 ? tn.zgroup : (dma ? 2 : 4);
   g.a_zstride = (size_t)h->Mpad * D;
-  g.o_zstride = (size_t)h->Mmod * h->Ntot;
+  g.o_zstride = (size_t)Mmod * h->Ntot;
   if constexpr (!T::is32) {
     if (tn.wide && g.N % 128 == 0 && g.K % 128 == 0) return launch_wide<T>(g, tn.wide_variant, s);
   }
@@ -149,7 +179,7 @@
     rc = run_gemm_partial<T>(cx, g, ks);
   } else {
     g.sat = cx.sat, g.out_f32 = cx.xres, g.ldo = cx.D;
-    g.gate = gate, g.ldg = cx.Ntot;
+    g.gate = gate, g.ldg = cx.Ntot, g.mr = cx.mr;
     if (tn.touch & 16) g.touch = make_touch(tn, B.fc1, M, 0, gemm_lanes_per_xcd(tn, M, g.N, g.K), 2);
     rc = run_gemm<T, EPI_GATE_RES>(tn, g, cx.s, false, &tn.plan_layer[RB_PROJ]);
   }
@@ -173,7 +203,7 @@
     rc = run_gemm_partial<T>(cx, g, ks, &tn.plan_layer[RB_FC2]);
   } else {
     g.sat = cx.sat, g.out_f32 = cx.xres, g.ldo = cx.D;
-    g.gate = gate, g.ldg = cx.Ntot;
+    g.gate = gate, g.ldg = cx.Ntot, g.mr = cx.mr;
     rc = run_gemm<T, EPI_GATE_RES>(tn, g, cx.s);
   }
   if (!rc && ks) *pend = pending_red(cx.slab, cx.Mpad, cx.D, B.fc2.b, gate, ks);
@@ -182,10 +212,11 @@
 
 template <class T>
 int run_blocks(float_fmt* h, int nclip, int bc, const float* modbuf, bool euler, float dt, float a, float r, float e, hipStream_t s,
-               float* vout_to = nullptr) {
+               float* vout_to = nullptr, const ModRows* mr = nullptr) {
   const float_fmt_cfg_t& c = h->cfg;
   const FmtTune& tn = h->tune;
-  const FmtLaunch cx = launch_ctx(h, s);
+  FmtLaunch cx = launch_ctx(h, s);
+  if (mr) cx.mr = *mr;
   const int D = h->D, ntok = h->ntok, M = nclip * bc * ntok;
   int rc;
   {
@@ -350,7 +381,7 @@
 
 template <class T>
 int run_window_steps(float_fmt* h, const CfgMode& m, int nfe, const std::vector<float>& ts, float a, float r, float e,
-                     hipStream_t s) {
+                     hipStream_t s, const RowsPlan& rp) {
   const Tableau& tb = tableau(h->method);
   const float_fmt_cfg_t& c = h->cfg;
   const size_t kstride = (size_t)h->Bmax * kMaxTok * c.dim_w;
@@ -361,10 +392,16 @@
   for (int ev = 0; ev < nev; ++ev) {
     const int i = ev / tb.s, j = ev - i * tb.s, z = ev % batch;
     const float dt = ts[i + 1] - ts[i];
-    if (z == 0 && (rc = run_mod_all<T>(h, rows, ev, std::min(batch, nev - ev), s))) return rc;
-    const float* mod = h->modall + (size_t)z * h->mod_zs;
+    if (z == 0 && (rc = run_mod_all<T>(h, rows, ev, std::min(batch, nev - ev), s, &rp))) return rc;
+    const float* mod = (rp.on ? rows_slab(h, rp.par) : h->modall) + (size_t)z * h->mod_zs;
+    ModRows mrz, *mr = nullptr;
+    if (rp.on) {
+      const int other = (rp.prev_par - rp.par) * kScSteps * h->Mmod1 + z * (rp.prev_zs - rp.zs);
+      FH_REQUIRE(fmt_make_mod_rows(rp.lay, rp.prev_lay, other, m.bc, h->ntok, c.n_prev, &mrz), "distinct modulation rows: the map does not fit its fields");
+      mr = &mrz;
+    }
     if (euler) {
-      if ((rc = run_blocks<T>(h, m.nclip, m.bc, mod, true, dt, a, r, e, s))) return rc;
+      if ((rc = run_blocks<T>(h, m.nclip, m.bc, mod, true, dt, a, r, e, s, nullptr, mr))) return rc;
       continue;
     }
     if (j > 0) {
@@ -372,7 +409,7 @@
                          dt * tb.a[j][0], dt * tb.a[j][1], dt * tb.a[j][2], 0.f, 0, h->xin16, h->Kx / 32, c.n_prev, c.n_cur,
                          c.dim_w, m.nclip, h->sat);
     }
-    if ((rc = run_blocks<T>(h, m.nclip, m.bc, mod, false, 0.f, a, r, e, s, h->kbuf + (size_t)j * kstride))) return rc;
+    if ((rc = run_blocks<T>(h, m.nclip, m.bc, mod, false, 0.f, a, r, e, s, h->kbuf + (size_t)j * kstride, mr))) return rc;
     if (j == tb.s - 1) {
       hipLaunchKernelGGL((fmt_rk_combine_kernel<T>), dim3((n + 255) / 256), dim3(256), 0, s, h->xcur, h->kbuf, kstride, tb.s,
                          dt * tb.b[0], dt * tb.b[1], dt * tb.b[2], dt * tb.b[3], 1, h->xin16, h->Kx / 32, c.n_prev, c.n_cur,
@@ -385,15 +422,17 @@
 
 constexpr size_t kMaxGraphs = 8;
 void destroy_graphs(float_fmt::GraphEntry& g) {
-  for (hipGraphExec_t& e : g.exec)
-    if (e) {
-      (void)hipGraphExecDestroy(e);
-      e = nullptr;
-    }
+  for (auto& form : g.exec)
+    for (hipGraphExec_t& e : form)
+      if (e) {
+        (void)hipGraphExecDestroy(e);
+        e = nullptr;
+      }
 }
 template <class T>
 int run_window_steps_graph(float_fmt* h, const CfgMode& m, int we_len, int nfe, const std::vector<float>& ts, float a,
-                           float r, float e, hipStream_t s) {
+                           float r, float e, hipStream_t s, const RowsPlan& rp) {
+  const int v = rp.on ? rp.variant : 0;
   float_fmt::GraphKey key;
   memset(&key, 0, sizeof(key));
   key.nfe = nfe;
@@ -408,12 +447,12 @@
   float_fmt::GraphEntry* hit = nullptr;
   for (auto& g : h->graphs)
     if (g.key == key) hit = &g;
-  if (!hit || !hit->exec[m.nclip]) {
+  if (!hit || !hit->exec[v][m.nclip]) {
     if (!h->cap_stream) FH_CHECK_HIP(hipStreamCreateWithFlags(&h->cap_stream, hipStreamNonBlocking));
     hipGraph_t graph = nullptr;
     h->cap_prio = key.prio;
     FH_CHECK_HIP(hipStreamBeginCapture(h->cap_stream, hipStreamCaptureModeThreadLocal));
-    int rc = run_window_steps<T>(h, m, nfe, ts, a, r, e, h->cap_stream);
+    int rc = run_window_steps<T>(h, m, nfe, ts, a, r, e, h->cap_stream, rp);
     hipError_t ce = hipStreamEndCapture(h->cap_stream, &graph);
     if (rc) {
       if (graph) (void)hipGraphDestroy(graph);
@@ -442,21 +481,22 @@
       h->graphs.push_back(fresh);
       hit = &h->graphs.back();
     }
-    hit->exec[m.nclip] = exec;
+    hit->exec[v][m.nclip] = exec;
   }
   hit->used = ++h->graph_clock;
-  FH_CHECK_HIP(hipGraphLaunch(hit->exec[m.nclip], s));
+  FH_CHECK_HIP(hipGraphLaunch(hit->exec[v][m.nclip], s));
   return FLOAT_OK;
 }
 
 template <class T>
 int window_impl(float_fmt* h, const float* x0, const float* wa, const float* wr, const float* we, int we_len,
                 const float* prev_x, const float* prev_wa, const float* prev_we, int nfe, const std::vector<float>& ts,
-                float a, float r, float e, int include_r, hipStream_t s, int nclip = 1) {
+                float a, float r, float e, int include_r, hipStream_t s, int nclip = 1, const RowsPlan& rp = RowsPlan()) {
   CfgMode m = cfg_mode(a, r, e, include_r);
   m.nclip = nclip;
   int rc = check_cfg_rows(h, m);
   if (rc) return rc;
+  if (!rp.on) h->rows_prev.valid = false;
   if ((rc = stage_window<T>(h, m, x0, wa, wr, we, we_len, prev_x, prev_wa, prev_we, s))) return rc;
   if (nfe <= 1) return FLOAT_OK;
   hipStreamCaptureStatus cs = hipStreamCaptureStatusNone;
@@ -465,8 +505,8 @@
     cs = hipStreamCaptureStatusNone;
   }
   if (h->cfg.use_graph && !g_fh_profiling && cs == hipStreamCaptureStatusNone)
-    return run_window_steps_graph<T>(h, m, we_len, nfe, ts, a, r, e, s);
-  return run_window_steps<T>(h, m, nfe, ts, a, r, e, s);
+    return run_window_steps_graph<T>(h, m, we_len, nfe, ts, a, r, e, s, rp);
+  return run_window_steps<T>(h, m, nfe, ts, a, r, e, s, rp);
 }
 
 template <class T>
@@ -480,9 +520,36 @@
   const CfgMode m = cfg_mode(a, r, e, include_r);
   if ((rc = check_cfg_rows(h, m))) return rc;
   if ((rc = stage_window<T>(h, m, x, wa, wr, we, we_len, prev_x, prev_wa, prev_we, s))) return rc;
+  h->rows_prev.valid = false;
   if ((rc = run_mod_all<T>(h, m.bc * h->ntok, 0, 1, s))) return rc;
   if ((rc = run_blocks<T>(h, 1, m.bc, h->modall, false, 0.f, a, r, e, s))) return rc;
   return dev_copy(out, h->vout, (size_t)h->ntok * h->cfg.dim_w, s);
+}
+
+template <class T>
+RowsPlan rows_plan(float_fmt* h, int k, hipStream_t s) {
+  RowsPlan p;
+  const auto& J = h->job;
+  const FmtTune& tn = h->tune;
+  const float_fmt_cfg_t& c = h->cfg;
+  const CfgMode m = cfg_mode(J.a, J.r, J.e, J.include_r);
+  const int nev = n_evals(h->method, J.nfe);
+  if (T::is32 || !tn.mod_rows || !tn.hoist || J.ragged || J.B != 1 || (m.bc != 3 && m.bc != 4) || nev < 1 || nev > kScSteps ||
+      stream_priority(s) != 0)
+    return p;
+  const auto& R = h->rows_prev;
+  p.first = !(k > J.first && R.valid && R.job == h->job_serial && R.window == k - 1 && R.nev == nev && R.method == h->method && R.bc == m.bc);
+  p.lay = fmt_mod_layout(m.bc, h->ntok, c.n_prev, m.wr_mask, m.wa_mask, m.we_mask, p.first);
+  if (!p.first) p.prev_lay = R.lay, p.prev_zs = R.zs, p.prev_par = R.par;
+  p.par = p.first ? 0 : (R.par ^ 1);
+  p.variant = p.first ? 1 : (R.first ? 2 : 3 + p.par);
+  p.big = tn.wide && big_shape_ok(tn, nev * p.lay.rows, h->adaln_all.N, h->adaln_all.K, h->n_cu);
+  p.zs = p.big ? p.lay.rows : h->Mmod1;
+  ModRows probe;
+  p.on = p.lay.rows <= h->Mmod1 &&
+         fmt_make_mod_rows(p.lay, p.prev_lay, (p.prev_par - p.par) * kScSteps * h->Mmod1 + (nev - 1) * (p.prev_zs - p.zs), m.bc, h->ntok,
+                           c.n_prev, &probe);
+  return p;
 }
 
 template <class T>
@@ -506,9 +573,18 @@
   hipLaunchKernelGGL(fmt_slice_pad_kernel, blocks(B * L * c.dim_a), dim3(256), 0, s, h->wa_c, J.wa, k * L, Tn, L, c.dim_a, B);
   if (dynamic) hipLaunchKernelGGL(fmt_slice_pad_kernel, blocks(B * L * c.dim_e), dim3(256), 0, s, h->we_c, J.we, k * L, Tn, L, c.dim_e, B);
   if ((rc = dev_copy(h->x0_c, J.noise + (size_t)k * B * L * c.dim_w, (size_t)B * L * c.dim_w, s))) return rc;
+  const RowsPlan rp = rows_plan<T>(h, k, s);
   rc = window_impl<T>(h, h->x0_c, h->wa_c, J.wr, dynamic ? h->we_c : J.we, dynamic ? L : 1, h->prev_x, h->prev_wa,
-                      dynamic ? h->prev_we : nullptr, J.nfe, J.ts, J.a, J.r, J.e, J.include_r, s, B);
-  if (rc) return rc;
+                      dynamic ? h->prev_we : nullptr, J.nfe, J.ts, J.a, J.r, J.e, J.include_r, s, B, rp);
+  if (rc) {
+    h->rows_prev.valid = false;
+    return rc;
+  }
+  if (rp.on) {
+    auto& R = h->rows_prev;
+    R.valid = true, R.par = rp.par, R.zs = rp.zs, R.window = k, R.nev = n_evals(h->method, J.nfe), R.method = h->method;
+    R.bc = cfg_mode(J.a, J.r, J.e, J.include_r).bc, R.job = h->job_serial, R.first = rp.first, R.lay = rp.lay;
+  }
   const int rows = (k == J.total - 1) ? (Tn - k * L) : L;
   return dev_copy2d(J.r_d + (size_t)k * L * c.dim_w, (size_t)Tn * c.dim_w, h->xcur, (size_t)L * c.dim_w, rows * c.dim_w, B, s);
 }
@@ -673,6 +749,13 @@
     FH_CHECK_HIP(hipGetLastError());
     return FLOAT_OK;
   }
+  if (what == 6) {
+    const auto& R = h->rows_prev;
+    const float v[4] = {R.valid ? 1.f : 0.f, (float)R.par, (float)R.lay.rows, R.first ? 1.f : 0.f};
+    FH_CHECK_HIP(hipStreamSynchronize(s));
+    FH_CHECK_HIP(hipMemcpy(out, v, sizeof(v), hipMemcpyHostToDevice));
+    return FLOAT_OK;
+  }
   FH_REQUIRE(what == 1 && in != nullptr, "float_fmt_debug: unknown request %d (or null input)", what);
   const int n = ntok * 3 * D;
   hipLaunchKernelGGL((fmt_dbg_to16_kernel<T>), dim3((n + 255) / 256), dim3(256), 0, s, h->qkv16, in, n);
@@ -737,7 +820,9 @@
   A(&h->th16, (size_t)kMaxSteps * D);
   A(&h->ccond, (size_t)Mp * D);
   h->Mmod = 16 * ((h->Bmax * 4 * h->ntok + 15) / 16);
-  if (!rc) rc = h->pool.alloc(&h->modall, (size_t)kScSteps * h->Mmod * h->Ntot, false);
+  h->Mmod1 = 16 * ((4 * h->ntok + 15) / 16);
+  const size_t mod_rows = std::max((size_t)kScSteps * h->Mmod, h->tune.mod_rows ? (size_t)2 * kScSteps * h->Mmod1 : (size_t)0);
+  if (!rc) rc = h->pool.alloc(&h->modall, mod_rows * h->Ntot, false);
   A(&h->kbuf, (size_t)4 * h->Bmax * kMaxTok * cfg->dim_w);
   A(&h->xres, (size_t)Mp * D);
   A(&h->slab, (size_t)8 * Mp * D);
@@ -851,6 +936,22 @@
   return FLOAT_OK;
 }
 
+int float_fmt_mod_rows(float a_cfg, float r_cfg, float e_cfg, int32_t include_r_cfg, int32_t ntok, int32_t n_prev, int32_t first,
+                       int32_t prev_first, int32_t other, int32_t* n_rows, int32_t* src, int32_t* map) {
+  FH_REQUIRE(n_rows && src && map, "float_fmt_mod_rows: null argument");
+  FH_REQUIRE(ntok >= 1 && ntok <= kMaxTok && n_prev >= 0 && 2 * n_prev <= ntok, "float_fmt_mod_rows: %d tokens, %d of them previous frames", (int)ntok, (int)n_prev);
+  const CfgMode m = cfg_mode(a_cfg, r_cfg, e_cfg, include_r_cfg);
+  const ModLayout L = fmt_mod_layout(m.bc, ntok, n_prev, m.wr_mask, m.wa_mask, m.we_mask, first != 0);
+  const ModLayout P = fmt_mod_layout(m.bc, ntok, n_prev, m.wr_mask, m.wa_mask, m.we_mask, prev_first != 0);
+  ModRows mr;
+  FH_REQUIRE(fmt_make_mod_rows(L, P, other, m.bc, ntok, n_prev, &mr), "float_fmt_mod_rows: the map does not fit its fields (other = %d)", (int)other);
+  *n_rows = L.rows;
+  for (int k = 0; k < L.segs.n; ++k)
+    for (int j = 0; j < L.segs.len[k]; ++j) src[L.segs.dst[k] + j] = L.segs.src[k] + j;
+  for (int r = 0; r < m.bc * ntok; ++r) map[r] = fmt_mod_row(mr, r);
+  return FLOAT_OK;
+}
+
 int float_fmt_set_method(float_fmt_t* h, int32_t method) {
   FH_REQUIRE(h != nullptr, "null FMT handle");
   FH_REQUIRE(method >= FLOAT_ODE_EULER && method <= FLOAT_ODE_HEUN3, "unknown ODE method %d", method);
@@ -890,6 +991,7 @@
   J.hist_x = J.hist_wa = J.hist_we = nullptr;
   linspace01(nfe, &J.ts);
   J.active = true;
+  ++h->job_serial;
   return FLOAT_OK;
 }
 
diff --git a/comfyui-float_optimized_amd/csrc/fmt_decode.hpp b/comfyui-float_optimized_amd/csrc/fmt_decode.hpp
--- a/comfyui-float_optimized_amd/csrc/fmt_decode.hpp
+++ b/comfyui-float_optimized_amd/csrc/fmt_decode.hpp
@@ -71,3 +71,87 @@
   }
   return GemmBlock{(int)bx, (int)by, (int)ks};
 }
+
+struct ModRows {
+  unsigned a;
+  unsigned br[4];
+};
+constexpr int kModPrevMax = (1 << 17) - 1;
+inline ModRows fmt_mod_identity() { return ModRows{0u, {1u << 13, 0u, 0u, 0u}}; }
+FMT_HD int fmt_mod_row(unsigned a, unsigned b0, unsigned b1, unsigned b2, unsigned b3, int row) {
+  const unsigned mul = a & 0xffffu, ntok = (a >> 16) & 0x7fu;
+  const int np = (int)((a >> 23) & 0x3fu);
+  const unsigned b = ((unsigned)row * mul) >> 16;
+  const int i = row - (int)(b * ntok);
+  const unsigned e = b == 0u ? b0 : (b == 1u ? b1 : (b == 2u ? b2 : b3));
+  const int cur = (int)(e & 0x1fffu) + (int)((e >> 13) & 1u) * (i - np);
+  const int prv = ((int)e >> 14) + i;
+  return i < np ? prv : cur;
+}
+FMT_HD int fmt_mod_row(const ModRows& m, int row) { return fmt_mod_row(m.a, m.br[0], m.br[1], m.br[2], m.br[3], row); }
+
+constexpr int kModBranches = 4, kModSegs = 8;
+struct ModSegs {
+  int n;
+  int dst[kModSegs], src[kModSegs], len[kModSegs];
+};
+struct ModLayout {
+  int rows;
+  int cur[kModBranches];
+  int step[kModBranches];
+  int prev[kModBranches];
+  int owner[kModBranches];
+  ModSegs segs;
+};
+inline ModLayout fmt_mod_layout(int bc, int ntok, int n_prev, unsigned wr_mask, unsigned wa_mask, unsigned we_mask, bool first) {
+  ModLayout L = ModLayout();
+  const int n_cur = ntok - n_prev;
+  auto seg = [&L](int src, int len) {
+    if (len <= 0) return;
+    L.segs.dst[L.segs.n] = L.rows, L.segs.src[L.segs.n] = src, L.segs.len[L.segs.n] = len;
+    ++L.segs.n;
+    L.rows += len;
+  };
+  for (int b = 0; b < bc && b < kModBranches; ++b) {
+    const bool on_a = (wa_mask >> b) & 1u, on_e = (we_mask >> b) & 1u;
+    L.owner[b] = b, L.prev[b] = -1;
+    if (!on_a && !on_e) {
+      L.step[b] = 0, L.cur[b] = L.rows;
+      seg(b * ntok + n_prev, 1);
+      int partner = -1;
+      for (int p = 0; p < bc && p < kModBranches; ++p)
+        if (((wa_mask >> p) & 1u) && !((we_mask >> p) & 1u) && ((wr_mask >> p) & 1u) == ((wr_mask >> b) & 1u)) partner = p;
+      if (partner >= 0) {
+        L.owner[b] = partner;
+      } else if (n_prev > 0) {
+        L.prev[b] = L.rows;
+        seg(b * ntok, n_prev);
+      }
+    } else {
+      L.step[b] = 1;
+      if ((first || !on_a) && n_prev > 0) {
+        L.prev[b] = L.rows;
+        seg(b * ntok, n_prev);
+      }
+      L.cur[b] = L.rows;
+      seg(b * ntok + n_prev, n_cur);
+    }
+  }
+  return L;
+}
+inline bool fmt_make_mod_rows(const ModLayout& L, const ModLayout& P, int other, int bc, int ntok, int n_prev, ModRows* out) {
+  ModRows m = ModRows{0u, {0u, 0u, 0u, 0u}};
+  const unsigned mul = 65535u / (unsigned)ntok + 1u;
+  if (ntok < 1 || ntok > 127 || n_prev < 0 || n_prev > 63 || bc < 1 || bc > kModBranches || mul > 0xffffu) return false;
+  for (int r = 0; r < bc * ntok; ++r)
+    if ((int)(((unsigned)r * mul) >> 16) != r / ntok) return false;
+  m.a = mul | ((unsigned)ntok << 16) | ((unsigned)n_prev << 23);
+  for (int b = 0; b < bc; ++b) {
+    const int o = L.owner[b];
+    const int p = L.prev[o] >= 0 ? L.prev[o] : other + P.cur[o] + (ntok - n_prev) - n_prev;
+    if (L.cur[b] < 0 || L.cur[b] > 0x1fff || p < -kModPrevMax || p > kModPrevMax) return false;
+    m.br[b] = (unsigned)L.cur[b] | ((unsigned)L.step[b] << 13) | ((unsigned)p << 14);
+  }
+  *out = m;
+  return true;
+}
diff --git a/comfyui-float_optimized_amd/csrc/fmt_kernels.hpp b/comfyui-float_optimized_amd/csrc/fmt_kernels.hpp
--- a/comfyui-float_optimized_amd/csrc/fmt_kernels.hpp
+++ b/comfyui-float_optimized_amd/csrc/fmt_kernels.hpp
@@ -65,7 +65,7 @@
     if constexpr (FLAT) row = min(m0 + min(r, ROWS - 1), g.M - 1);
     if (FLAT || (r < ROWS && row < g.M)) {
       const float* o = g.out_f32 + (size_t)row * g.ldo + nb;
-      const float* gt = g.gate + (size_t)row * g.ldg + nb;
+      const float* gt = g.gate + (ptrdiff_t)fmt_mod_row(g.mr, row) * g.ldg + nb;
       res_pf[0] = fh_load_f4(o);
       res_pf[1] = fh_load_f4(o + 4);
       gate_pf[0] = fh_load_f4_stream(gt);
@@ -215,7 +215,7 @@
         else T::template store8_wt<8, WT>(o16 + fmt_pack_off(row, nb, g.ldo16), u);
       } else if constexpr (EPI == EPI_GATE_RES) {
         float* o = g.out_f32 + (size_t)row * g.ldo + nb;
-        const float* gt = g.gate + (size_t)row * g.ldg + nb;
+        const float* gt = kEarlyRes ? nullptr : g.gate + (ptrdiff_t)fmt_mod_row(g.mr, row) * g.ldg + nb;
 #pragma unroll
         for (int e = 0; e < 8; e += 4) {
           float4 x, gg;
@@ -627,7 +627,8 @@
 template <class T, int NV, int KS, bool TOUCH, bool WT>
 __device__ __forceinline__ void fmt_lnmod_body(float* __restrict__ x, int M, const float* __restrict__ shift,
                                                const float* __restrict__ scale, int ldm, u16* __restrict__ out, const LnRed& red,
-                                               const TouchSpec& pf, int ntok, int perm, unsigned long long* sat, const int wpb) {
+                                               const TouchSpec& pf, int ntok, int perm, unsigned long long* sat, const int wpb,
+                                               const ModRows& mr) {
   constexpr int D = NV * 256;
   const unsigned bid = blockIdx.x, nblk = gridDim.x;
   const int lane = threadIdx.x & 63;
@@ -647,35 +648,37 @@
     return;
   }
   float* xr = x + (size_t)row * D;
+  float4 v[NV], a[NV], b[NV];
+  float s = 0.f;
+#pragma unroll
+  for (int i = 0; i < NV; ++i) v[i] = fh_load_f4(xr + i * 256 + lane * 4);
+  float4 p[KS > 0 ? KS : 1][NV];
+  if constexpr (KS > 0) {
+#pragma unroll
+    for (int i = 0; i < NV; ++i)
+#pragma unroll
+      for (int k = 0; k < KS; ++k) p[k][i] = fh_load_f4_stream(red.slab + k * red.slab_stride + (size_t)row * D + i * 256 + lane * 4);
+  }
+  asm volatile("" ::: "memory");
+  __builtin_amdgcn_sched_barrier(0);
 #ifdef FMT_DIAG_HOTMOD
-  const size_t mrow = 0;
+  const ptrdiff_t mrow = 0;
 #else
-  const size_t mrow = (size_t)row;
+  const ptrdiff_t mrow = fmt_mod_row(mr, __builtin_amdgcn_readfirstlane(row));
 #endif
   const float* sh = shift + mrow * ldm;
   const float* sc = scale + mrow * ldm;
-  float4 v[NV], a[NV], b[NV];
-  float s = 0.f;
 #pragma unroll
   for (int i = 0; i < NV; ++i) {
     const int c = i * 256 + lane * 4;
-    v[i] = fh_load_f4(xr + c);
     a[i] = fh_load_f4_stream(sh + c);
     b[i] = fh_load_f4_stream(sc + c);
   }
   if (KS == 0 && touch) touch_lines();
   if constexpr (KS > 0) {
-    float4 p[KS][NV], gt[NV], bi[NV];
-#pragma unroll
-    for (int i = 0; i < NV; ++i) {
-      const int c = i * 256 + lane * 4;
-#pragma unroll
-      for (int k = 0; k < KS; ++k) {
-        const float* ps = red.slab + k * red.slab_stride + (size_t)row * D + c;
-        p[k][i] = fh_load_f4_stream(ps);
-      }
-      gt[i] = fh_load_f4_stream(red.gate + mrow * ldm + c);
-    }
+    float4 gt[NV], bi[NV];
+#pragma unroll
+    for (int i = 0; i < NV; ++i) gt[i] = fh_load_f4_stream(red.gate + mrow * ldm + i * 256 + lane * 4);
 #pragma unroll
     for (int i = 0; i < NV; ++i) bi[i] = *reinterpret_cast<const float4*>(red.bias + i * 256 + lane * 4);
     if (touch) touch_lines();
@@ -725,12 +728,14 @@
 
 template <class T, int NV, int KS, bool TOUCH, bool WT>
 __global__ __launch_bounds__(256) void fmt_lnmod_kernel(float* __restrict__ x, const float* __restrict__ shift,
-                                                        const float* __restrict__ scale, const float* __restrict__ slab,
-                                                        const float* __restrict__ gate, int M, int ldm, int wpb, unsigned slab_stride,
+                                                        const float* __restrict__ slab, int M, int ldm, unsigned slab_stride,
+                                                        unsigned mr_a, unsigned mr0, unsigned mr1, unsigned mr2, unsigned mr3,
                                                         u16* __restrict__ out, const float* __restrict__ red_bias, TouchSpec pf,
                                                         int ntok, int perm, unsigned long long* sat) {
-  const LnRed red{slab, (size_t)slab_stride, red_bias, gate};
-  fmt_lnmod_body<T, NV, KS, TOUCH, WT>(x, M, shift, scale, ldm, out, red, pf, ntok, perm, sat, wpb);
+  constexpr int D = NV * 256;
+  const LnRed red{slab, (size_t)slab_stride, red_bias, shift - D};
+  const ModRows mr{mr_a, {mr0, mr1, mr2, mr3}};
+  fmt_lnmod_body<T, NV, KS, TOUCH, WT>(x, M, shift, shift + D, ldm, out, red, pf, ntok, perm, sat, (int)(mr_a >> 29), mr);
 }
 
 template <class T, int LPQ, bool TOUCH, bool WT>
@@ -924,10 +929,12 @@
 
 template <class T>
 __global__ void fmt_silu_c_kernel(u16* __restrict__ out, const float* __restrict__ temb, const float* __restrict__ ccond,
-                                  int M, int D, size_t step_stride, int dense_rows, unsigned long long* sat) {
-  const int idx = (blockIdx.x * blockDim.x + threadIdx.x) * 8;
+                                  int M, int D, size_t step_stride, int dense_rows, unsigned long long* sat, const ModSegs segs) {
+  int idx = (blockIdx.x * blockDim.x + threadIdx.x) * 8;
   if (idx >= M * D) return;
-  const int c = idx % D, row = idx / D + (int)blockIdx.y * dense_rows;
+  const int c = idx % D, r = idx / D, row = r + (int)blockIdx.y * dense_rows;
+  for (int k = 0; k < segs.n; ++k)
+    if (r >= segs.dst[k] && r < segs.dst[k] + segs.len[k]) idx = (segs.src[k] + r - segs.dst[k]) * D + c;
   typename T::elem* const o = reinterpret_cast<typename T::elem*>(out) + (dense_rows ? (size_t)0 : (size_t)blockIdx.y * step_stride);
   temb += (size_t)blockIdx.y * D;
   typename T::pack8 u;
diff --git a/comfyui-float_optimized_amd/csrc/fmt_launch.hpp b/comfyui-float_optimized_amd/csrc/fmt_launch.hpp
--- a/comfyui-float_optimized_amd/csrc/fmt_launch.hpp
+++ b/comfyui-float_optimized_amd/csrc/fmt_launch.hpp
@@ -29,6 +29,7 @@
   float *xres, *slab;
   u16 *h16, *qkv16, *att16;
   int D, ntok, Ntot, Mpad, heads, attn_window;
+  ModRows mr = fmt_mod_identity();
 };
 
 
@@ -295,6 +296,7 @@
   memset(&g, 0, sizeof(g));
   g.A = A, g.W = L.W, g.bias = L.b;
   g.K = L.K, g.N = L.N, g.M = M;
+  g.mr = fmt_mod_identity();
   return g;
 }
 
@@ -412,8 +414,10 @@
   });
   FH_REQUIRE(kern, "dim_h %d unsupported (must be 256*{1,2,4,8})", cx.D);
   FH_REQUIRE(red.slab_stride <= 0xffffffffull, "split-K slab of %zu elements is beyond the LayerNorm kernel's 32-bit stride", red.slab_stride);
-  hipLaunchKernelGGL(kern, grid, block, 0, cx.s, cx.xres, shift, scale, red.slab, red.gate, M, cx.Ntot, rpw, (unsigned)red.slab_stride,
-                     out ? out : cx.h16, red.bias, pf, cx.ntok, perm, cx.sat);
+  FH_REQUIRE(scale == shift + cx.D && (!ks || red.gate == shift - cx.D), "LayerNorm: scale / gate are not the column blocks around shift");
+  hipLaunchKernelGGL(kern, grid, block, 0, cx.s, cx.xres, shift, red.slab, M, cx.Ntot, (unsigned)red.slab_stride,
+                     cx.mr.a | ((unsigned)rpw << 29), cx.mr.br[0], cx.mr.br[1], cx.mr.br[2], cx.mr.br[3], out ? out : cx.h16, red.bias, pf,
+                     cx.ntok, perm, cx.sat);
   if (pend) pend->ks = 0;
   FH_CHECK_HIP(hipGetLastError());
   return FLOAT_OK;
diff --git a/comfyui-float_optimized_amd/csrc/fmt_pack.hpp b/comfyui-float_optimized_amd/csrc/fmt_pack.hpp
--- a/comfyui-float_optimized_amd/csrc/fmt_pack.hpp
+++ b/comfyui-float_optimized_amd/csrc/fmt_pack.hpp
@@ -101,6 +101,7 @@
   int ldo16;
   const float* gate;
   int ldg;
+  ModRows mr;
   const float* pos;
   int bc, ntok, n_prev;
   int nclip;
diff --git a/comfyui-float_optimized_amd/csrc/tuning.hpp b/comfyui-float_optimized_amd/csrc/tuning.hpp
--- a/comfyui-float_optimized_amd/csrc/tuning.hpp
+++ b/comfyui-float_optimized_amd/csrc/tuning.hpp
@@ -57,6 +57,7 @@
   int proj_split = 0;
   int touch = 230;
   bool hoist = true;
+  bool mod_rows = true;
   int zgroup = 0;
   int ln_rows = 1;
   int attn_qpw = 8, attn_lpq = 16;
@@ -85,6 +86,7 @@
     t.proj_split = env_atoi("FLOAT_FMT_PROJ_SPLIT", t.proj_split);
     t.touch = env_atoi("FLOAT_FMT_TOUCH", t.touch);
     t.hoist = env_atoi("FLOAT_FMT_HOIST", 1) != 0;
+    t.mod_rows = env_atoi("FLOAT_FMT_MOD_ROWS", 1) != 0;
     t.zgroup = std::max(0, env_atoi("FLOAT_FMT_ZGROUP", 0));
     t.ln_rows = std::max(1, std::min(4, env_atoi("FLOAT_FMT_LN_ROWS", 1)));
     int attn[2] = {t.attn_qpw, t.attn_lpq};
diff --git a/comfyui-float_optimized_amd/fmt.py b/comfyui-float_optimized_amd/fmt.py
--- a/comfyui-float_optimized_amd/fmt.py
+++ b/comfyui-float_optimized_amd/fmt.py
@@ -79,6 +79,12 @@
                 native.check(native.lib().float_fmt_debug(self._h, 5, native.dev_ptr(buf[i:i + per]), native.dev_ptr(out[i:i + per]),
                                                           native.stream_ptr(self.device)))
         return out[:n]
+
+    def mod_rows_state(self):
+        out = torch.zeros(4, device=self.device)
+        with torch.cuda.device(self.device):
+            native.check(native.lib().float_fmt_debug(self._h, 6, None, native.dev_ptr(out), native.stream_ptr(self.device)))
+        return tuple(int(v) for v in out.tolist())
 
     def saturation(self, reset=False):
         with torch.cuda.device(self.device):
diff --git a/comfyui-float_optimized_amd/native.py b/comfyui-float_optimized_amd/native.py
--- a/comfyui-float_optimized_amd/native.py
+++ b/comfyui-float_optimized_amd/native.py
@@ -137,6 +137,7 @@
     "float_aud_expand_rows": (C.c_int, [C.c_void_p, C.c_int32, C.c_int32, C.c_void_p, C.c_int32, C.c_float, C.c_void_p]),
     "float_enc_feats16": (C.c_int, [C.c_void_p, C.POINTER(C.c_void_p), C.POINTER(C.c_int32), C.c_int32, C.POINTER(C.c_int32)]),
     "float_enc_export_feats16": (C.c_int, [C.c_void_p, C.POINTER(C.c_void_p), C.c_int32, C.c_void_p]),
+    "float_fmt_mod_rows": (C.c_int, [C.c_float] * 3 + [C.c_int32] * 6 + [C.POINTER(C.c_int32)] * 3),
     "float_fmt_saturation": (C.c_int, [C.c_void_p, C.POINTER(C.c_uint64), C.c_int32, C.c_void_p]),
     "float_enc_saturation": (C.c_int, [C.c_void_p, C.POINTER(C.c_uint64), C.c_int32, C.c_void_p]),
     "float_aud_saturation": (C.c_int, [C.c_void_p, C.POINTER(C.c_uint64), C.c_int32, C.c_void_p]),
diff --git a/include/float_hip.h b/include/float_hip.h
--- a/include/float_hip.h
+++ b/include/float_hip.h
@@ -208,6 +208,9 @@
                                 float scale, void* stream);
 int float_aud_expand_rows(const float* rows, int32_t n, int32_t c, float* frames, int32_t T, float scale, void* stream);
 
+int float_fmt_mod_rows(float a_cfg, float r_cfg, float e_cfg, int32_t include_r_cfg, int32_t ntok, int32_t n_prev, int32_t first,
+                       int32_t prev_first, int32_t other, int32_t* n_rows, int32_t* src, int32_t* map);
+
 int float_hip_abi_version(void);
 const char* float_last_error(void);
 int float_yuv_matrix(int32_t matrix, int32_t table[15]);
```

After: 2592 frames/s. 1.7% lower.
